# pasqualedem/LabelAnything

Measured on AMD Instinct MI355X. Metric: episodes/sec (query+support fwd) ViT-B 1024px 1-shot, higher is better.
Workload: dtype f16; 1 GPU; BASELINE cfg2: SAM ViT-B 1024px encoder + LabelAnything decoder, 1-way 1-shot episodes (2 images each), random-init weights, full-resolution logits; parallelism=episode-sharded x1, no collective, launch=hipGraph replay

## Files before the change

include/la_hip.h:

```cpp
#ifndef LA_HIP_H
#define LA_HIP_H
#ifdef __cplusplus
extern "C" {
#endif

enum { LA_F16 = 0, LA_BF16 = 1, LA_F32 = 2, LA_F16X2 = 3 };
enum { LA_ACT_NONE = 0, LA_ACT_GELU = 1, LA_ACT_RELU = 2, LA_ACT_GELU_BWD = 3  };
enum { LA_MAP_NONE = 0, LA_MAP_GROUP = 1, LA_MAP_WINDOW_MERGE = 2, LA_MAP_CONVT2X2 = 3, LA_MAP_WINDOW_PART = 4, LA_MAP_CONV3X3 = 5  };
enum { LA_ATTN_PLAIN = 0, LA_ATTN_RELPOS = 1, LA_ATTN_RELPOS_WIN16 = 2 };

const char* la_last_error(void);
int la_version(void);

int la_gemm_variant(int v);

typedef struct LaGemmEpilogue {
  const float* bias;
  const float* res;
  int ldr;
  int res_mod;
  float* out32;
  int ld32;
  void* out16;
  int ld16;
  int act;
  int map;
  int p0, p1, p2, p3, p4;
  void* vt;
  int vt_col0, vt_T, vt_Tpad, vt_hd, vt_heads;
  int vt_ws;
  int amap;
  int a_kmod;
  int ksplit;
  void* aux16;
  int ldaux;
  float* nstat_out;
  const float* rvec;
  int rvec_rpg;
  const float* nstat_in;
  const float* ncol;
} LaGemmEpilogue;

int la_gemm_fused_act_ok(int M, int N, int K);

int la_gemm(const void* A, int lda, const void* W, int ldw, int M, int N, int K,
            const LaGemmEpilogue* epi, int dt, void* stream);

enum { LA_GEMM_NT = 0, LA_GEMM_DMA128, LA_GEMM_DMA256x128, LA_GEMM_T256, LA_GEMM_T256P, LA_GEMM_T256Q, LA_GEMM_T256W,
       LA_GEMM_F32_N32, LA_GEMM_F32_N128, LA_GEMM_F32_SMALL, LA_GEMM_SKINNY };
typedef struct LaGemmPlan {
  int kernel, epi, planes, direct, ragged, gm, ksplit, kchunk, grid, block, lds_bytes;
} LaGemmPlan;

int la_gemm_plan(const void* A, int lda, const void* W, int ldw, int M, int N, int K,
                 const LaGemmEpilogue* epi, int dt, int ncu, LaGemmPlan* out);

int la_conv3x3_f32(const float* in, int B, int H, int W, int Cin, const float* wt, const float* bias, int Cout, float* out32,
                   void* stream);

int la_conv3x3_split_ok(int Cin, int Cout);
int la_conv3x3_split(const float* in, int B, int H, int W, int Cin, const float* wt, const float* bias, int Cout, float* out32, void* stream);

int la_layernorm(const float* x, const float* x2, int ldx, int rows, int E, const float* gamma, const float* beta,
                 float eps, int gelu, float* out32, void* out16, void* out16_pe, const float* pe, int pe_mod,
                 int window, int H, int W, int dt, void* stream);

int la_im2col_patch(const float* img, int Bn, int S, int patch, void* out16, int dt, void* stream);

int la_im2col_3x3(const void* in16, int B, int H, int W, int C, void* out16, int dt, void* stream);

int la_relpos_terms(const void* qkv, int B, int heads, int G, int E, const void* tabh, const void* tabw,
                    float* relh, float* relw, int dt, void* stream);

int la_attn_fwd(const void* qkv, const void* vt, void* out16, const float* relh, const float* relw,
                const void* tabh, const void* tabw, int B, int heads, int T, int Tpad, int G, int E, float scale, int mode,
                int dt, void* stream);


int la_dense_pe(const float* gauss, int g, int D, float* out, void* stream);

int la_point_embed(const float* xy, const int* kind, const int* shift, int n, int D, int image_size, const float* gauss,
                   const float* type_emb, const float* not_a_point, const float* no_sparse, float* out32, void* stream);

int la_mask_embed(const float* masks, const int* flags, int P, int C, int Hm, int g, int D, const float* const* w,
                  const float* support, const float* class_enc, const float* pe, float* src32, void* src16, void* srcpe16,
                  int dt, void* stream);

int la_attn_small(const float* q, int ldq, const float* k, int ldk, const float* v, int ldv, int B, int Nq, int Nk, int heads,
                  int hd, void* out16, float* out32, int ldo, int dt, void* stream);

int la_colmean(const float* x, int P, int hw, int D, float* out, float* scratch, void* stream);

int la_class_mean(const float* emb, const unsigned char* flags, int B, int M, int C, int D, float* out, void* stream);

int la_region_mean(const float* x, int B, int M, int C, int g, int k, int D, float* out, void* stream);

int la_classify_max(const float* feat, const float* protos, const unsigned char* flags, int B, int Npix, int N, int C, int Cf, float* seg,
                    int* win, void* stream);

int la_classify(const float* feat, const float* protos, int B, int Npix, int C, int Cf, float* seg, void* stream);

int la_add_cast(const float* x, const float* y, int ymod, long rows, int D, float* out32, void* out16, int dt, void* stream);

int la_nchw_to_nhwc(const float* in, int N, int C, int HW, float* out32, void* out16, int dt, void* stream);
int la_nhwc_to_nchw(const float* in, int N, int C, int HW, float* out, void* stream);

int la_transpose_many(const long long* tile_table, int ntiles, void* stream);

int la_bilinear(const float* in, int N, int h, int w, int H, int W, float* out, void* stream);

int la_post_final(const float* big, int B, int C, int S, const int* sizes, const unsigned char* flag_gts, int Hmax, int Wmax,
                  float* logits, long long* argmax, void* stream);

int la_confmat_update(const long long* pred, const long long* gt, int B, long HW, const int* lut, int L, int K,
                      long long ignore_index, unsigned long long* confmat, unsigned long long* confbin,
                      unsigned long long* counters, void* stream);

int la_resample_u8(const unsigned char* in, long n_outer, int in_size, int inner, int out_size, const int* bounds, const int* kk,
                   int ksize, unsigned char* out, void* stream);
int la_u8_to_chw_norm(const unsigned char* in, int h, int w, int SH, int SW, const float* mean3, const float* std3, float* out,
                      void* stream);

int la_prompt_masks(const unsigned char* masks, const int* first, const int* count, const int* index, int P, int H, int W, int nh,
                    int nw, int S, int Mo, float* out, unsigned char* flags, void* stream);

int la_focal_loss(const float* logits, const long long* target, int B, int C, long HW, float gamma, int class_weighting, float scale,
                  long long ignore_index, float* loss, float* dlogits, float* class_weights, void* scratch, long scratch_bytes,
                  void* stream);

int la_logits_objective_workspace_bytes(int B, int C, long HW, long* bytes);
int la_logits_objective(const float* logits, const long long* target, int B, int C, long HW, long long ignore_index, int mask,
                        float w_focal, float gamma, float w_dice, float w_fp, int class_weighting, float* value, float* components,
                        float* dlogits, float* class_weights, void* workspace, long workspace_bytes, void* stream);

int la_prompt_contrastive_workspace_bytes(int B, int n, int D, long* bytes);
int la_prompt_contrastive(const float* emb, const unsigned char* flags, int B, int n, int C, int D, const float* t_prime, const float* bias,
                          float* loss, float* demb, float* dt_prime, float* dbias, void* workspace, long workspace_bytes, void* stream);

// ... 155 lines not shown
```

labelanything_amd/_lib.py:

```python
from __future__ import annotations

import ctypes as C
import os
from typing import Optional

import torch

_HERE = os.path.dirname(os.path.abspath(__file__))
LIB_PATH = os.path.join(_HERE, "libla_hip.so")

LA_F16, LA_BF16, LA_F32, LA_F16X2 = 0, 1, 2, 3
ACT_NONE, ACT_GELU, ACT_RELU, ACT_GELU_BWD = 0, 1, 2, 3
MAP_NONE, MAP_GROUP, MAP_WINDOW_MERGE, MAP_CONVT2X2, MAP_WINDOW_PART, MAP_CONV3X3 = 0, 1, 2, 3, 4, 5
ATTN_PLAIN, ATTN_RELPOS, ATTN_RELPOS_WIN16 = 0, 1, 2

_DT = {torch.float16: LA_F16, torch.bfloat16: LA_BF16, torch.float32: LA_F32}


class LaGemmEpilogue(C.Structure):
    _fields_ = [
        ("bias", C.c_void_p), ("res", C.c_void_p), ("ldr", C.c_int), ("res_mod", C.c_int),
        ("out32", C.c_void_p), ("ld32", C.c_int), ("out16", C.c_void_p), ("ld16", C.c_int),
        ("act", C.c_int), ("map", C.c_int),
        ("p0", C.c_int), ("p1", C.c_int), ("p2", C.c_int), ("p3", C.c_int), ("p4", C.c_int),
        ("vt", C.c_void_p), ("vt_col0", C.c_int), ("vt_T", C.c_int), ("vt_Tpad", C.c_int),
        ("vt_hd", C.c_int), ("vt_heads", C.c_int), ("vt_ws", C.c_int), ("amap", C.c_int), ("a_kmod", C.c_int), ("ksplit", C.c_int),
        ("aux16", C.c_void_p), ("ldaux", C.c_int),
        ("nstat_out", C.c_void_p), ("rvec", C.c_void_p), ("rvec_rpg", C.c_int), ("nstat_in", C.c_void_p), ("ncol", C.c_void_p),
    ]


_lib: Optional[C.CDLL] = None


def lib() -> C.CDLL:
    global _lib
    if _lib is None:
        if not os.path.exists(LIB_PATH):
            raise RuntimeError(
                f"labelanything_amd: HIP extension {LIB_PATH} is missing - build it with "
                "`python -c 'import __graft_entry__ as g; g.build()'` (there is no CPU/eager fallback)")
        l = C.CDLL(LIB_PATH)
        l.la_last_error.restype = C.c_char_p
        l.la_version.restype = C.c_int
        for name in EXPORTS:
            getattr(l, name).restype = C.c_int
        _lib = l
    return _lib


EXPORTS = [
    "la_gemm", "la_layernorm", "la_im2col_patch", "la_im2col_3x3", "la_relpos_terms", "la_attn_fwd",
    "la_dense_pe", "la_point_embed", "la_mask_embed", "la_attn_small", "la_colmean", "la_class_mean",
    "la_classify", "la_add_cast", "la_conv3x3_f32", "la_nchw_to_nhwc", "la_nhwc_to_nchw", "la_bilinear", "la_post_final",
    "la_confmat_update", "la_resample_u8", "la_u8_to_chw_norm", "la_prompt_masks", "la_focal_loss", "la_adamw_step",
    "la_gemm_tn", "la_gemm_tn16", "la_gemm_fused_act_ok", "la_gemm_plan", "la_colsum_acc", "la_layernorm_bwd", "la_layernorm_bwd_res", "la_transpose_many", "la_act_fwd", "la_act_bwd", "la_attn_small_lse", "la_attn_small_bwd", "la_bilinear_bwd", "la_bilinear_bwd_set", "la_bilinear_bwd_set_ok", "la_bilinear_rows", "la_bilinear_rows_bwd_set",
    "la_classify_bwd", "la_row_broadcast", "la_twoway_t2i", "la_twoway_i2t", "la_gemm_variant", "la_attn_fwd_lse", "la_head_transpose", "la_attn_bwd", "la_cast", "la_gelu_bwd16", "la_axpy", "la_transpose16", "la_qk_fp8", "la_attn_fwd_fp8", "la_colmean16", "la_layernorm_g", "la_add_rowvec", "la_add_rowvec_split", "la_attn_fwd_cs", "la_attn_fwd_rows", "la_colsum_fold", "la_gelu_fwd16", "la_gemm_tn_db",
    "la_attn_fwd_relpos_lse", "la_attn_bwd_relpos", "la_relpos_bwd", "la_twoway_pe_layout",
    "la_norm_finalize", "la_norm_stats", "la_conv3x3_split", "la_conv3x3_split_ok",
    "la_error_count", "la_error_points",
    "la_logits_objective_workspace_bytes", "la_logits_objective", "la_prompt_contrastive_workspace_bytes", "la_prompt_contrastive",
    "la_rle_scan", "la_rle_decode", "la_rle_prompt_masks", "la_rle_ground_truth", "la_rle_points",
    "la_region_mean", "la_classify_max", "la_region_mean_bwd", "la_classify_max_bwd",
    "la_classify_wide", "la_classify_wide_bwd", "la_level_reduce", "la_level_reduce_bwd",
    "la_proto_kernels", "la_proto_kernels_bwd", "la_classify_conv", "la_classify_conv_bwd",
    "la_extract_pool_plan", "la_extract_pool", "la_extract_fold", "la_extract_unfold",
]


def gemm_variant(v: int = -1) -> int:
    return int(lib().la_gemm_variant(int(v)))


def _check(rc: int, what: str) -> None:
    if rc != 0:
        msg = lib().la_last_error().decode()
        raise RuntimeError(f"{what} failed ({rc}): {msg}")


def _ptr(t: Optional[torch.Tensor]):
    return None if t is None else C.c_void_p(t.data_ptr())


def _stream() -> C.c_void_p:
    return C.c_void_p(torch.cuda.current_stream().cuda_stream)


def dt_of(t: torch.Tensor) -> int:
    return _DT[t.dtype]


def _dev(t: torch.Tensor) -> None:
    if not t.is_cuda:
        raise RuntimeError("labelanything_amd kernels need device tensors (no CPU fallback)")
    if t.device.index != torch.cuda.current_device():
        raise RuntimeError(f"tensor on {t.device} but the current device is cuda:{torch.cuda.current_device()}: "
                           "wrap the call in `with torch.cuda.device(tensor.device)`")


class LaGemmPlan(C.Structure):
    _fields_ = [(f, C.c_int) for f in ("kernel", "epi", "planes", "direct", "ragged", "gm", "ksplit", "kchunk", "grid", "block", "lds_bytes")]


GEMM_KERNELS = ("NT", "DMA128", "DMA256x128", "T256", "T256P", "T256Q", "T256W", "F32_N32", "F32_N128", "F32_SMALL", "SKINNY")


def _addr(x) -> Optional[int]:
    return x.data_ptr() if isinstance(x, torch.Tensor) else x


def _gemm_epilogue(m: int, n: int, *, bias=None, res=None, res_mod=0, out32=None, out16=None, act=ACT_NONE, map=MAP_NONE, p=(0, 0, 0, 0, 0), vt=None,
                   vt_col0=0, vt_T=0, vt_Tpad=0, vt_hd=64, vt_heads=0, vt_ws=0, amap=MAP_NONE, a_kmod=0, ksplit=0, aux16=None, nstat_out=None, rvec=None,
                   rvec_rpg=0, nstat_in=None, ncol=None, ldr=None, ld32=None, ld16=None, ldaux=None) -> LaGemmEpilogue:
    def ld(x, given):
        if x is None:
            return 0
        if given is not None:
            return given
        return n if not isinstance(x, torch.Tensor) else (x.stride(-2) if x.dim() >= 2 else 0)

    e = LaGemmEpilogue()
    e.bias, e.res, e.out32, e.out16, e.vt, e.aux16 = _addr(bias), _addr(res), _addr(out32), _addr(out16), _addr(vt), _addr(aux16)
    e.ldr, e.ld32, e.ld16, e.ldaux = ld(res, ldr), ld(out32, ld32), ld(out16, ld16), ld(aux16, ldaux)
    e.res_mod = res_mod
    e.act, e.map = act, map
    e.p0, e.p1, e.p2, e.p3, e.p4 = p
    e.vt_col0, e.vt_T, e.vt_Tpad, e.vt_hd, e.vt_heads = vt_col0, vt_T, vt_Tpad, vt_hd, vt_heads
    e.vt_ws = vt_ws
    e.amap = amap
    e.a_kmod = a_kmod
    e.ksplit = ksplit
    mpad = -(-m // 256) * 256
    if isinstance(nstat_out, torch.Tensor) and (nstat_out.dtype != torch.float32 or nstat_out.numel() < m * (n // 64) * 2):
        raise RuntimeError(f"gemm: nstat_out must be fp32 with at least M * (N / 64) * 2 = {m * (n // 64) * 2} entries")
    if isinstance(nstat_in, torch.Tensor) and (nstat_in.dtype != torch.float32 or nstat_in.numel() < mpad * 2 or ncol is None
                                               or ncol.dtype != torch.float32 or ncol.numel() < n):
        raise RuntimeError(f"gemm: nstat_in must be fp32 [ceil(M / 256) * 256, 2] (>= {mpad * 2} entries) and needs ncol fp32 [N]")
    if isinstance(rvec, torch.Tensor) and (rvec.dtype != torch.float32 or rvec_rpg <= 0 or rvec.numel() < -(-m // rvec_rpg) * n):
        raise RuntimeError("gemm: rvec must be fp32 [ceil(M / rvec_rpg), N] with rvec_rpg > 0")
    e.nstat_out, e.rvec, e.nstat_in, e.ncol = _addr(nstat_out), _addr(rvec), _addr(nstat_in), _addr(ncol)
    e.rvec_rpg = rvec_rpg
    return e


def gemm(a: torch.Tensor, w: torch.Tensor, *, M=None, lda=None, **epilogue) -> None:
    _dev(a)
    m = a.shape[0] if M is None else M
    k = w.shape[1]
    n = w.shape[0]
    e = _gemm_epilogue(m, n, **epilogue)
    rc = lib().la_gemm(_ptr(a), C.c_int(a.stride(0) if lda is None else lda), _ptr(w), C.c_int(w.stride(0)),
                       C.c_int(m), C.c_int(n), C.c_int(k), C.byref(e), C.c_int(dt_of(a)), _stream())
    _check(rc, "la_gemm")


def gemm_plan(a, lda: int, w, ldw: int, m: int, n: int, k: int, dt: int, ncu: int = 0, **epilogue) -> LaGemmPlan:
    plan = LaGemmPlan()
    e = _gemm_epilogue(m, n, **epilogue)
    rc = lib().la_gemm_plan(C.c_void_p(_addr(a)), C.c_int(lda), C.c_void_p(_addr(w)), C.c_int(ldw), C.c_int(m), C.c_int(n), C.c_int(k), C.byref(e),
                            C.c_int(dt), C.c_int(ncu), C.byref(plan))
    _check(rc, "la_gemm_plan")
    return plan


def norm_finalize(part: Optional[torch.Tensor], m: int, e: int, eps: float, mr: torch.Tensor, x16: Optional[torch.Tensor] = None, rpg: int = 0,
                  cs_part: Optional[torch.Tensor] = None) -> None:
    _dev(mr)
    mpad = -(-m // 256) * 256
    if mr.dtype != torch.float32 or mr.numel() < mpad * 2 or not mr.is_contiguous():
        raise RuntimeError(f"norm_finalize: mr must be contiguous fp32 with >= {mpad * 2} entries")
    if part is not None and (part.dtype != torch.float32 or part.numel() < m * (e // 64) * 2):
        raise RuntimeError("norm_finalize: part must be fp32 [m, e / 64, 2]")
    if cs_part is not None:
        if x16 is None or rpg <= 0 or m % rpg or x16.shape[0] < m or x16.shape[1] != e or x16.stride(1) != 1:
            raise RuntimeError("norm_finalize: column sums need x16 [m, e] and m % rpg == 0")
        if cs_part.dtype != torch.float32 or cs_part.numel() < (m // rpg) * norm_cs_chunks(rpg) * e:
            raise RuntimeError("norm_finalize: cs_part too small")
    _check(lib().la_norm_finalize(_ptr(part), C.c_int(m), C.c_int(e // 64), C.c_int(e), C.c_float(eps), _ptr(mr), _ptr(x16),
                                  C.c_int(x16.stride(0) if x16 is not None else 0), C.c_int(rpg), _ptr(cs_part),
                                  C.c_int(dt_of(x16) if x16 is not None else LA_F16), _stream()), "la_norm_finalize")


def norm_cs_chunks(rpg: int) -> int:
    return -(-rpg // 128)


def norm_stats(x: torch.Tensor, eps: float, x16: torch.Tensor, mr: torch.Tensor) -> None:
    _dev(x)
    m, e = x.shape
    mpad = -(-m // 256) * 256
    if x.dtype != torch.float32 or x.stride(1) != 1 or x16.shape != x.shape or not x16.is_contiguous() or mr.dtype != torch.float32 \
            or mr.numel() < mpad * 2:
        raise RuntimeError("norm_stats: x fp32 [m, e], x16 contiguous 16-bit [m, e], mr fp32 with >= ceil(m / 256) * 256 * 2 entries")
    _check(lib().la_norm_stats(_ptr(x), C.c_int(x.stride(0)), C.c_int(m), C.c_int(e), C.c_float(eps), _ptr(x16), _ptr(mr),
                               C.c_int(dt_of(x16)), _stream()), "la_norm_stats")


def gemm_fused_act_ok(m: int, n: int, k: int) -> bool:
    return bool(lib().la_gemm_fused_act_ok(C.c_int(m), C.c_int(n), C.c_int(k)))


def layernorm(x: torch.Tensor, gamma, beta, eps: float, *, x2=None, gelu=False, out32=None, out16=None,
              out16_pe=None, pe=None, pe_mod=0, window=0, H=0, W=0, dt=LA_F16) -> None:
    _dev(x)
    rows, e = x.shape[0], x.shape[1]
    if window < 0:
        o = out32 if out32 is not None else out16
        if window == -2:
            rows = o.shape[0]
            if x.shape[0] < (rows // (H * W)) * (H + 2) * (W + 2):
                raise RuntimeError("layernorm(window=-2): x must hold the padded maps [B * (H + 2) * (W + 2), E]")
        elif out16 is None or out16.shape[0] < (rows // (H * W)) * (H + 2) * (W + 2):
            raise RuntimeError("layernorm(window=-1): out16 must hold the padded maps [B * (H + 2) * (W + 2), ...]")
    rc = lib().la_layernorm(_ptr(x), _ptr(x2), C.c_int(x.stride(0)), C.c_int(rows), C.c_int(e), _ptr(gamma), _ptr(beta),
                            C.c_float(eps), C.c_int(int(gelu)), _ptr(out32), _ptr(out16), _ptr(out16_pe), _ptr(pe),
                            C.c_int(pe_mod), C.c_int(window), C.c_int(H), C.c_int(W), C.c_int(dt), _stream())
    _check(rc, "la_layernorm")


def im2col_patch(img: torch.Tensor, patch: int, out16: torch.Tensor, split: bool = False) -> None:
    _dev(img)
    bn, _, s, _ = img.shape
    dt = LA_F16X2 if split else dt_of(out16)
    if split and out16.dtype != torch.float16:
        raise RuntimeError("im2col_patch(split=True) writes fp16 plane pairs")
    _check(lib().la_im2col_patch(_ptr(img), C.c_int(bn), C.c_int(s), C.c_int(patch), _ptr(out16), C.c_int(dt),
                                 _stream()), "la_im2col_patch")


def im2col_3x3(x16: torch.Tensor, b: int, h: int, w: int, c: int, out16: torch.Tensor, split: bool = False) -> None:
    _dev(x16)
    _check(lib().la_im2col_3x3(_ptr(x16), C.c_int(b), C.c_int(h), C.c_int(w), C.c_int(c), _ptr(out16),
                               C.c_int(LA_F16X2 if split else dt_of(x16)), _stream()), "la_im2col_3x3")


def relpos_terms(qkv: torch.Tensor, b: int, heads: int, g: int, e: int, tabh, tabw, relh, relw) -> None:
    _check(lib().la_relpos_terms(_ptr(qkv), C.c_int(b), C.c_int(heads), C.c_int(g), C.c_int(e), _ptr(tabh), _ptr(tabw),
                                 _ptr(relh), _ptr(relw), C.c_int(dt_of(qkv)), _stream()), "la_relpos_terms")


def attn_fwd(qkv, vt, out16, relh, relw, b: int, heads: int, t: int, tpad: int, g: int, e: int, scale: float, mode: int,
             tabh=None, tabw=None) -> None:
    _check(lib().la_attn_fwd(_ptr(qkv), _ptr(vt), _ptr(out16), _ptr(relh), _ptr(relw), _ptr(tabh), _ptr(tabw), C.c_int(b),
                             C.c_int(heads), C.c_int(t),
                             C.c_int(tpad), C.c_int(g), C.c_int(e), C.c_float(scale), C.c_int(mode), C.c_int(dt_of(qkv)),
                             _stream()), "la_attn_fwd")

# ... 728 lines not shown
```

labelanything_amd/csrc/gemm.hip:

```cpp
#include <cstdlib>
#include <cstring>
#include <type_traits>
#include "la_common.h"
#include "../../include/la_hip.h"
#include "gemm_shared.h"
#include "gemm_plan.h"

namespace la {

constexpr int BM = 128, BN = 128, BK = 64;
constexpr int STAGE_BYTES = (BM + BN) * BK * 2;


template <typename T>
__global__ __launch_bounds__(256, 2) void gemm_nt_kernel(const T* __restrict__ A, int lda, const T* __restrict__ Wt, int ldw,
                                                          int M, int N, int K, LaGemmEpilogue e) {
  extern __shared__ __attribute__((aligned(16))) char smem[];
  const int tid = threadIdx.x, lane = tid & 63, wave = tid >> 6;
  const int wm = wave >> 1, wn = wave & 1;
  const int ntn = (N + BN - 1) / BN, ntm = (M + BM - 1) / BM;
  const int tile = xcd_remap(blockIdx.x, ntm * ntn);
  const int m0 = (tile / ntn) * BM, n0 = (tile % ntn) * BN;

  const int lc = tid & 7, lr = tid >> 3;
// ... 1469 lines not shown
        a[u] = *reinterpret_cast<const float4*>(ap + 8 * j);
        b[u] = *reinterpret_cast<const float4*>(wp + 8 * j);
      }
#pragma unroll
      for (int u = 0; u < 8; ++u) {
        if (j0 + u * KS < nchunk) {
          acc = __builtin_amdgcn_mfma_f32_32x32x2f32(a[u].x, b[u].x, acc, 0, 0, 0);
          acc = __builtin_amdgcn_mfma_f32_32x32x2f32(a[u].y, b[u].y, acc, 0, 0, 0);
          acc = __builtin_amdgcn_mfma_f32_32x32x2f32(a[u].z, b[u].z, acc, 0, 0, 0);
          acc = __builtin_amdgcn_mfma_f32_32x32x2f32(a[u].w, b[u].w, acc, 0, 0, 0);
        }
      }
    }
  }
  if (KS == 4) {
#pragma unroll
    for (int r = 0; r < 16; ++r) part[wave][r][lane] = acc[r];
    __syncthreads();
    if (wave != 0) return;
#pragma unroll
    for (int r = 0; r < 16; ++r) acc[r] = (part[0][r][lane] + part[1][r][lane]) + (part[2][r][lane] + part[3][r][lane]);
  }
  if (!active) return;
  const int col = tn * 32 + fr;
  if (col >= N) return;
  float* outT = reinterpret_cast<float*>(e.out16);
  const float bias = e.bias ? e.bias[col] : 0.f;
#pragma unroll
  for (int r = 0; r < 16; ++r) {
    const int m = tm * 32 + (r & 3) + 8 * (r >> 2) + 4 * fh;
    if (m >= M) continue;
    float v = acc[r] + bias;
    if (e.act == LA_ACT_GELU) v = gelu_erf(v);
    else if (e.act == LA_ACT_RELU) v = fmaxf(v, 0.f);
    if (e.res) v += e.res[(size_t)(e.res_mod ? m % e.res_mod : m) * e.ldr + col];
    if (e.out32) e.out32[(size_t)m * e.ld32 + col] = v;
    if (outT) outT[(size_t)m * e.ld16 + col] = v;
  }
}

static void launch_f32_small(const LaGemmPlan& p, const GemmArgs& g) {
  const dim2 d = f32_small_grid(g.M, g.N, g.K);
  with_int<1, 4>(g.K >= 1024 ? 4 : 1, [&](auto ks) { launch<float, gemm_f32_small_kernel<LA_V(ks)>>(dim3(d.x, d.y), p, g); });
}

template <typename T>
static void launch_plan(const LaGemmPlan& p, const GemmArgs& g, int stg) {
  const dim3 grid(p.grid);
  if constexpr (std::is_same<T, float>::value) {
    switch (p.kernel) {
      case LA_GEMM_F32_SMALL: return launch_f32_small(p, g);
      case LA_GEMM_SKINNY: return launch_skinny<float>(p, g);
      default: return launch_f32(p, g, ConvA{0, 0, 0, 0});
    }
  } else {
    switch (p.kernel) {
      case LA_GEMM_SKINNY: return launch_skinny<T>(p, g);
      case LA_GEMM_NT: return launch<T, gemm_nt_kernel<T>>(grid, p, g);
      case LA_GEMM_DMA128: return launch<T, gemm_dma_kernel<T, 128>>(grid, p, g, p.gm);
      case LA_GEMM_DMA256x128: return launch<T, gemm_dma4_kernel<T>>(grid, p, g, p.gm);
      case LA_GEMM_T256:
        return (void)with_int<1, 2>(p.planes, [&](auto npl) {
          with_int<0, 1, 2, 3>(p.epi, [&](auto e) { launch<T, gemm_t256_kernel<T, LA_V(npl), LA_V(e)>>(grid, p, g, p.gm); });
        });
      case LA_GEMM_T256P:
        return (void)with_int<1, 2>(p.planes, [&](auto npl) {
          with_int<1, 2, 3>(p.epi, [&](auto e) { launch<T, gemm_t256p_kernel<T, LA_V(npl), LA_V(e)>>(grid, p, g, p.gm); });
        });
      case LA_GEMM_T256Q:
        return (void)with_int<1, 2, 3, 4>(p.epi, [&](auto e) { launch<T, gemm_t256q_kernel<T, LA_V(e)>>(grid, p, g, p.gm, p.ksplit, p.kchunk); });
      default:
        with_int<1, 2, 3>(p.epi, [&](auto e) { launch_t256w<T, LA_V(e)>(p, g, stg); });
        with_int<5, 6>(p.epi, [&](auto e) { launch_t256w_fused<T, LA_V(e)>(p, g, stg); });
        if constexpr (std::is_same<T, f16_t>::value) with_int<7, 8, 9, 10, 11, 12>(p.epi, [&](auto e) { launch_t256w_fused<T, LA_V(e)>(p, g, stg); });
    }
  }
}

#ifdef LA_DEBUG
static void plan_debug_overrides(LaGemmPlan* p, uintptr_t A, int lda, uintptr_t W, int ldw, int M, int N, int K, const LaGemmEpilogue& e, int ncu,
                                 int variant, int* stg) {
  static const char *path = getenv("LA_GEMM_PATH"), *nop = getenv("LA_GEMM_NO_PERSISTENT"), *nosmall = getenv("LA_NO_F32_SMALL"),
                    *want = getenv("LA_KSPLIT_WANT"), *kgrid = getenv("LA_KSPLIT_GRID"), *gmenv = getenv("LA_GEMM_GROUP_M"),
                    *w4grid = getenv("LA_W4_GRID"), *stagger = getenv("LA_W4_STAGGER");
  const bool tiles16 = p->kernel <= LA_GEMM_T256P || (p->kernel == LA_GEMM_T256Q && p->epi != 4) || (p->kernel == LA_GEMM_T256W && p->epi <= 3);
  const int planes = p->planes;
  if (tiles16 && path && (path[0] == 'v' || p->kernel != LA_GEMM_NT)) {
    *p = plan_default(K);
    if (path[0] == 'v') plan_launch(p, LA_GEMM_NT, M, N, K, ncu, variant);
    else if (path[0] == '7' && (!e.vt || (e.vt_col0 % 256) == 0)) plan_t256(p, planes, M, N, K / planes, e, ncu, variant);
    else plan_launch(p, path[0] == '4' || (path[0] != '2' && K <= 1536 && tiles_of(M, N, 256, 128) >= 512) ? LA_GEMM_DMA256x128 : LA_GEMM_DMA128, M, N, K, ncu, variant);
  }
  if (tiles16 && nop && p->kernel >= LA_GEMM_T256P) {
    *p = plan_default(K);
    plan_t256(p, planes, M, N, K / planes, e, ncu, variant, false);
  }
  if (nosmall && p->kernel == LA_GEMM_F32_SMALL) plan_launch(p, LA_GEMM_SKINNY, M, N, K, ncu, variant);
  if (p->kernel == LA_GEMM_T256Q && p->epi == 4) {
    if (want) ksplit_chunks(K / 64, atoi(want), p), plan_launch(p, LA_GEMM_T256Q, M, N, K, ncu, variant);
    if (kgrid) p->grid = atoi(kgrid) > 0 ? atoi(kgrid) : (int)tiles_of(M, N, 256, 256) * p->ksplit;
  }
  if (gmenv && group_m(p->kernel, N)) p->gm = (p->gm & ~0xff) | atoi(gmenv);
  if (p->kernel == LA_GEMM_T256W) {
    if (w4grid && atoi(w4grid) > 0 && atoi(w4grid) < p->grid) p->grid = atoi(w4grid);
    if (stagger) *stg = (atoi(stagger) << 16) | (strchr(stagger, ',') ? atoi(strchr(stagger, ',') + 1) : 0);
  }
}
#endif

}

extern "C" int la_gemm_variant(int v) {
  const int prev = la::g_gemm_variant;
#ifdef LA_DEBUG
  if (v >= 0) la::g_gemm_variant = v;
#else
  if (v >= 0 && v <= 2) la::g_gemm_variant = v;
#endif
  return prev;
}

#ifdef LA_DEBUG
extern "C" int la_dbg_gemm_stamps(unsigned long long* host_out) {
  (void)hipDeviceSynchronize();
  return (int)hipMemcpyFromSymbol(host_out, HIP_SYMBOL(la::g_dbg_stamps), sizeof(unsigned long long) * 8 * la::LA_DBG_NSTAMP);
}
extern "C" int la_dbg_gemm_stamps_clear() {
  static unsigned long long z[8 * la::LA_DBG_NSTAMP] = {0};
  return (int)hipMemcpyToSymbol(HIP_SYMBOL(la::g_dbg_stamps), z, sizeof(z));
}
#endif

extern "C" int la_gemm_fused_act_ok(int M, int N, int K) { return la::fused_act_ok(M, N, K, la::cu_count(), la::g_gemm_variant); }

static int gemm_plan_checked(const void* A, int lda, const void* W, int ldw, int M, int N, int K, const LaGemmEpilogue* epi, int dt, int ncu,
                             LaGemmPlan* p, int* stg) {
  LA_CHECK_ARG(A && W && epi && p, "la_gemm: null pointer");
  if (ncu <= 0) ncu = la::cu_count();
  const uintptr_t a = reinterpret_cast<uintptr_t>(A), w = reinterpret_cast<uintptr_t>(W);
  char err[640];
  if (la::gemm_plan(a, lda, w, ldw, M, N, K, *epi, dt, ncu, la::g_gemm_variant, p, err, sizeof(err)) != 0) {
    la_set_error("%s", err);
    return -1;
  }
#ifdef LA_DEBUG
  la::plan_debug_overrides(p, a, lda, w, ldw, M, N, K, *epi, ncu, la::g_gemm_variant, stg);
#endif
  return 0;
}

extern "C" int la_gemm_plan(const void* A, int lda, const void* W, int ldw, int M, int N, int K, const LaGemmEpilogue* epi, int dt, int ncu,
                            LaGemmPlan* out) {
  int stg = 0;
  return gemm_plan_checked(A, lda, W, ldw, M, N, K, epi, dt, ncu, out, &stg);
}

extern "C" int la_gemm(const void* A, int lda, const void* W, int ldw, int M, int N, int K, const LaGemmEpilogue* epi, int dt,
                       void* stream) {
  LaGemmPlan p;
  int stg = 0;
  if (gemm_plan_checked(A, lda, W, ldw, M, N, K, epi, dt, 0, &p, &stg) != 0) return -1;
  const la::GemmArgs g{A, W, lda, ldw, M, N, K, *epi, reinterpret_cast<hipStream_t>(stream)};
  if (dt == LA_F32) la::launch_plan<float>(p, g, stg);
  else if (dt == LA_F16) la::launch_plan<la::f16_t>(p, g, stg);
  else la::launch_plan<la::bf16_t>(p, g, stg);
  LA_CHECK_LAUNCH("la_gemm");
  return 0;
}

extern "C" int la_conv3x3_f32(const float* in, int B, int H, int W, int Cin, const float* wt, const float* bias, int Cout, float* out32,
                              void* stream) {
  LA_CHECK_ARG(in && wt && out32, "la_conv3x3_f32: null pointer");
  LA_CHECK_ARG(B > 0 && H > 0 && W > 0 && Cin > 0 && (Cin % 32) == 0 && Cout > 0, "la_conv3x3_f32: Cin=%d must be a multiple of 32", Cin);
  LaGemmEpilogue e{};
  e.bias = bias;
  e.out32 = out32;
  e.ld32 = Cout;
  const int M = B * H * W, K = 9 * Cin;
  LaGemmPlan p = la::plan_default(K);
  la::plan_f32(&p, M, Cout, K, e);
  la::launch_f32(p, la::GemmArgs{in, wt, Cin, K, M, Cout, K, e, reinterpret_cast<hipStream_t>(stream)}, la::ConvA{1, H, W, Cin});
  LA_CHECK_LAUNCH("la_conv3x3_f32");
  return 0;
}
```

labelanything_amd/csrc/gemm_plan.h:

```cpp
#pragma once
#include <cstdint>
#include <cstdio>
#include "../../include/la_hip.h"

namespace la {

#define LA_PLAN_CHECK(cond, ...) \
  do { if (!(cond)) { snprintf(err, errsz, __VA_ARGS__); return -1; } } while (0)

template <typename P> static inline bool al16(P p) { return ((uintptr_t)p & 15) == 0; }
static inline long tiles_of(int M, int N, int bm, int bn) { return (long)((M + bm - 1) / bm) * ((N + bn - 1) / bn); }

static inline bool k64_ok(int K, int a_kmod) { return (K % 64) == 0 && K >= 128 && (a_kmod == 0 || (a_kmod % 64) == 0); }

static inline bool epi_vec_ok(int N, const LaGemmEpilogue& e, int elt_bytes) {
  return (N % 8) == 0 && (!e.bias || al16(e.bias)) && (!e.res || (al16(e.res) && (e.ldr % 4) == 0)) &&
         (!e.out32 || (al16(e.out32) && (e.ld32 % 4) == 0)) && (!e.out16 || (al16(e.out16) && (e.ld16 % (16 / elt_bytes)) == 0)) &&
         (e.map != LA_MAP_CONVT2X2 || (e.p2 % 8) == 0) && (!e.vt || ((e.vt_col0 % 128) == 0 && (e.vt_Tpad % 4) == 0 && al16(e.vt)));
}

static inline bool dma_operands_ok(uintptr_t A, int lda, uintptr_t W, int ldw, int M, int N) {
  return (size_t)M * lda * 2 < (1ull << 32) && (size_t)N * ldw * 2 < (1ull << 32) && al16(A) && al16(W);
}
static inline bool fast_ok(uintptr_t A, int lda, uintptr_t W, int ldw, int M, int N, int K, const LaGemmEpilogue& e) {
  return (K % 64) == 0 && dma_operands_ok(A, lda, W, ldw, M, N) && epi_vec_ok(N, e, 2);
}

static inline bool fused_act_ok(int M, int N, int K, int ncu, int variant) {
  return M > 0 && (N % 256) == 0 && k64_ok(K, 0) && tiles_of(M, N, 256, 256) >= ncu && (variant & 0xff) == 2;
}

static inline int group_m(int kernel, int N) {
  if (kernel == LA_GEMM_DMA128 || kernel == LA_GEMM_DMA256x128) return 8;
  if (kernel == LA_GEMM_T256Q || kernel == LA_GEMM_T256W) return N >= 2560 ? 8 : 2;
  return kernel == LA_GEMM_T256 || kernel == LA_GEMM_T256P ? 2 : 0;
}

static inline int persistent_grid(long ntiles, int ncu) { return ntiles < ncu ? (int)ntiles : ncu; }

static inline void ksplit_chunks(int nkt, int want, LaGemmPlan* p) {
  if (want > nkt / 2) want = nkt / 2;
  if (want < 1) want = 1;
  int c = (nkt + want - 1) / want;
  if (c < 2) c = 2;
  while (c < nkt && (nkt % c) == 1) ++c;
  if (c > nkt) c = nkt;
  p->kchunk = c * 64;
  p->ksplit = (nkt + c - 1) / c;
}

struct dim2 { int x, y; };
static inline dim2 f32_small_grid(int M, int N, int K) {
  return K >= 1024 ? dim2{(N + 31) / 32, (M + 31) / 32} : dim2{(N + 63) / 64, (M + 63) / 64};
}
static inline dim2 skinny_grid(int M, int N, int K) {
  const int groups = (N + 3) / 4;
  return dim2{K >= 1024 ? groups : (groups + 3) / 4, M > 32 ? (M + 31) / 32 : 1};
}

struct KernelShape { int bm, bn, block, lds, lds2; };
constexpr KernelShape KERNEL_SHAPE[] = {
    {128, 128, 256, 65536, 0},
    {128, 128, 256, 128 * 132 * 4, 0},
    {256, 128, 256, 3 * 24576, 0},
    {256, 256, 512, 136 * 1024, 3 * 49152},
    {256, 256, 512, 4 * 32768 + 8 * 512 + 8 * 2048, 3 * 49152 + 8 * 2048},
    {256, 256, 512, 2 * 65536 + 8 * 2048 + 8 * 512, 0},
    {256, 256, 256, 4 * 32768 + 4 * 8192, 0},
    {128, 32, 256, 2 * (128 + 32) * 128, 0},
    {128, 128, 256, 128 * 132 * 4, 0},
};

static inline void plan_launch(LaGemmPlan* p, int kernel, int M, int N, int K, int ncu, int variant) {
  p->kernel = kernel;
  p->gm = group_m(kernel, N);
  if (kernel == LA_GEMM_F32_SMALL || kernel == LA_GEMM_SKINNY) {
    const dim2 g = kernel == LA_GEMM_SKINNY ? skinny_grid(M, N, K) : f32_small_grid(M, N, K);
    p->grid = g.x * g.y, p->block = 256, p->lds_bytes = 0;
    return;
  }
  const KernelShape& s = KERNEL_SHAPE[kernel];
  const long tiles = tiles_of(M, N, s.bm, s.bn) * p->ksplit;
  p->grid = kernel >= LA_GEMM_T256P && kernel <= LA_GEMM_T256W ? persistent_grid(tiles, ncu) : (int)tiles;
  p->block = s.block, p->lds_bytes = p->planes == 2 ? s.lds2 : s.lds;
  if (kernel == LA_GEMM_T256Q) p->gm |= variant & 0x800500;
}

static inline void plan_t256(LaGemmPlan* p, int planes, int M, int N, int K, const LaGemmEpilogue& e, int ncu, int variant, bool persistent = true) {
  const int var = variant & 0xff;
  const bool plain = e.map == LA_MAP_NONE && e.res_mod == 0;
  const bool only16 = !e.res && !e.out32 && e.out16;
  const bool plain16 = plain && only16 && e.act == LA_ACT_NONE, gelu16 = plain && only16 && e.act == LA_ACT_GELU && !e.vt;
  const bool scatter = e.map == LA_MAP_WINDOW_PART && e.res_mod == 0 && e.amap == LA_MAP_NONE && only16 && e.act == LA_ACT_NONE &&
                       (planes == 1 || (e.vt && e.vt_col0 == 0)) &&
                       (!e.vt || (size_t)((M + e.vt_T - 1) / e.vt_T + 4096) * e.vt_heads * e.vt_hd * e.vt_Tpad < (1ull << 32));
  const bool w4_resmod = planes == 1 && e.map == LA_MAP_NONE && e.res_mod > 0 && (e.res_mod % 256) == 0 && (M % 256) == 0 && e.res && var == 2 &&
                         k64_ok(K, e.a_kmod) && !((variant >> 8) & 1);
  const bool f32 = (plain || w4_resmod) && e.act == LA_ACT_NONE && e.out32 && !e.vt && (e.ld32 % 4) == 0 && (!e.res || (e.ldr % 4) == 0);
  const int pepi = (plain16 || scatter) ? 1 : gelu16 ? 2 : f32 ? 3 : 0;
  p->planes = planes, p->epi = pepi;
  if (!(persistent && pepi && (N % 256) == 0 && K / 32 >= 8 && (e.ld16 % 8) == 0)) {
    p->epi = plain16 ? 1 : gelu16 ? 2 : (plain && e.act == LA_ACT_NONE && e.res && e.out32 && !e.vt) ? 3 : 0;
    return plan_launch(p, LA_GEMM_T256, M, N, K, ncu, variant);
  }
  const bool k64 = planes == 1 && k64_ok(K, e.a_kmod);
  plan_launch(p, k64 && var == 2 ? LA_GEMM_T256W : k64 && var >= 1 ? LA_GEMM_T256Q : LA_GEMM_T256P, M, N, K, ncu, variant);
  if (p->kernel == LA_GEMM_T256W) {
    p->gm |= variant & 0xf500;
    p->direct = e.map == LA_MAP_NONE && !e.vt && !((variant >> 8) & 1);
    p->ragged = p->direct && (M & 255) != 0;
  }
}

static inline void plan_w4_fused(LaGemmPlan* p, int epi, int M, int N, int K, int ncu, int variant) {
  p->epi = epi, p->direct = 1, p->ragged = (M & 255) != 0;
  plan_launch(p, LA_GEMM_T256W, M, N, K, ncu, variant);
}

static inline void plan_tiles16(LaGemmPlan* p, uintptr_t A, int lda, uintptr_t W, int ldw, int M, int N, int K, const LaGemmEpilogue& e, int ncu,
                                int variant) {
  if (!fast_ok(A, lda, W, ldw, M, N, K, e)) return plan_launch(p, LA_GEMM_NT, M, N, K, ncu, variant);
  const int planes = (e.a_kmod > 0 && K == 2 * e.a_kmod) ? 2 : 1;
  if (tiles_of(M, N, 256, 256) >= (planes == 2 ? 128 : 512) && (!e.vt || (e.vt_col0 % 256) == 0)) return plan_t256(p, planes, M, N, K / planes, e, ncu, variant);
  plan_launch(p, K <= 1536 && tiles_of(M, N, 256, 128) >= 512 ? LA_GEMM_DMA256x128 : LA_GEMM_DMA128, M, N, K, ncu, variant);
}

static inline void plan_f32(LaGemmPlan* p, int M, int N, int K, const LaGemmEpilogue& e) {
  p->epi = epi_vec_ok(N, e, 4) ? 1 : 0;
  plan_launch(p, N <= 32 ? LA_GEMM_F32_N32 : LA_GEMM_F32_N128, M, N, K, 0, 0);
}

static inline LaGemmPlan plan_default(int K) { return LaGemmPlan{LA_GEMM_NT, 0, 1, 0, 0, 0, 1, K, 0, 256, 0}; }

static inline int gemm_plan(uintptr_t A, int lda, uintptr_t W, int ldw, int M, int N, int K, const LaGemmEpilogue& e, int dt, int ncu, int variant,
                            LaGemmPlan* p, char* err, size_t errsz) {
  *p = plan_default(K);
  LA_PLAN_CHECK(A && W, "la_gemm: null pointer");
  LA_PLAN_CHECK(M > 0 && N > 0 && K > 0, "la_gemm: bad shape M=%d N=%d K=%d", M, N, K);
  LA_PLAN_CHECK(e.ld16 < (1 << 22) && e.ldaux < (1 << 22) && e.ld32 < (1 << 22) && e.ldr < (1 << 22) && N < (1 << 22),
                "la_gemm: output / residual leading dimensions must be below %d elements", 1 << 22);
  const int kq = (dt == LA_F32) ? 4 : 8;
  LA_PLAN_CHECK((K % kq) == 0 && (lda % kq) == 0 && (ldw % kq) == 0, "la_gemm: K, lda, ldw must be multiples of %d (K=%d lda=%d ldw=%d)", kq, K,
                lda, ldw);
  LA_PLAN_CHECK(e.out32 || e.out16 || e.vt, "la_gemm: no output");
  LA_PLAN_CHECK(e.a_kmod == 0 || (dt != LA_F32 && e.a_kmod > 0 && (e.a_kmod % 64) == 0 && e.a_kmod <= K && lda >= e.a_kmod && M > 32),
                "la_gemm: a_kmod=%d must be a multiple of 64, <= K=%d and <= lda=%d (16-bit operands, M > 32)", e.a_kmod, K, lda);
  LA_PLAN_CHECK(dt == LA_F16 || dt == LA_BF16 || dt == LA_F32, "la_gemm: bad dtype %d", dt);
  LA_PLAN_CHECK(e.amap == LA_MAP_NONE || (e.amap == LA_MAP_WINDOW_PART && e.map == LA_MAP_NONE && dt != LA_F32) ||
                    (e.amap == LA_MAP_CONV3X3 && e.map == LA_MAP_NONE && dt == LA_F16 && e.a_kmod == 0 && e.p1 > 0 && (e.p1 % 64) == 0 &&
                     K == 27 * e.p1 && e.p2 == lda && lda == 2 * e.p1 && e.p0 > 2 && (N % 256) == 0 && !e.vt && e.ksplit == 0 && M > 512),
                "la_gemm: amap must be LA_MAP_NONE, LA_MAP_WINDOW_PART (16-bit operands, no output map) or LA_MAP_CONV3X3 (fp16 plane pairs, p0 = padded "
                "width, p1 = C %% 64 == 0, p2 = lda = 2 C, K = 27 C, N %% 256 == 0), got amap=%d map=%d dt=%d", e.amap, e.map, dt);
  LA_PLAN_CHECK(e.act != LA_ACT_GELU_BWD || e.aux16, "la_gemm: LA_ACT_GELU_BWD needs aux16 (the saved pre-activation)");
  const bool rows16 = (e.ld16 % 8) == 0 && e.ld16 >= N && al16(e.out16);
  if (e.aux16 && !e.nstat_out) {
    LA_PLAN_CHECK(e.act == LA_ACT_GELU || e.act == LA_ACT_GELU_BWD, "la_gemm: aux16 goes with LA_ACT_GELU (written) or LA_ACT_GELU_BWD (read)");
    LA_PLAN_CHECK(dt != LA_F32 && fused_act_ok(M, N, K, ncu, variant) && fast_ok(A, lda, W, ldw, M, N, K, e),
                  "la_gemm: aux16 needs 16-bit operands and a shape la_gemm_fused_act_ok() accepts (M=%d N=%d K=%d)", M, N, K);
    LA_PLAN_CHECK(e.out16 && !e.out32 && !e.res && !e.vt && e.map == LA_MAP_NONE && e.amap == LA_MAP_NONE && e.a_kmod == 0 && e.ksplit == 0 && rows16 &&
                      (e.ldaux % 8) == 0 && e.ldaux >= N && al16(e.aux16),
                  "la_gemm: aux16 forms write out16 only (no residual / fp32 output / maps / V^T / planes), rows 16-byte aligned");
    LA_PLAN_CHECK(e.act == LA_ACT_GELU || !e.bias, "la_gemm: LA_ACT_GELU_BWD takes no bias");
    plan_w4_fused(p, e.act == LA_ACT_GELU ? 5 : 6, M, N, K, ncu, variant);
    return 0;
  }
  if (e.nstat_out || e.nstat_in || e.rvec) {
    LA_PLAN_CHECK(dt == LA_F16 && (N % 256) == 0 && k64_ok(K, e.a_kmod) && fast_ok(A, lda, W, ldw, M, N, K, e) && (variant & 0xff) == 2,
                  "la_gemm: nstat_out / nstat_in need fp16 operands, N %% 256 == 0, K %% 64 == 0, K >= 128, 16-byte aligned rows (M=%d N=%d K=%d)", M,
                  N, K);
    LA_PLAN_CHECK(!e.vt && e.map == LA_MAP_NONE && e.amap == LA_MAP_NONE && e.ksplit == 0 && !(e.nstat_out && e.nstat_in) &&
                      (!e.aux16 || (e.nstat_out && (e.ldaux % 8) == 0 && e.ldaux >= N && al16(e.aux16))),
                  "la_gemm: nstat_out / nstat_in take no row maps / V^T / ksplit, not both at once; aux16 only with nstat_out (the lo plane, 16-byte aligned rows)");
    const bool stat8 = (reinterpret_cast<uintptr_t>(e.nstat_out) & 7) == 0;
    const bool rvec_ok = !e.rvec || (e.rvec_rpg > 0 && al16(e.rvec) && ((e.rvec_rpg % 256) == 0 || e.rvec_rpg >= 128));
    const bool rvec_split = e.rvec && (e.rvec_rpg % 256) != 0;
    int epi;
    if (e.nstat_in) {
      LA_PLAN_CHECK(e.ncol && e.out16 && !e.out32 && !e.res && !e.rvec && (e.act == LA_ACT_NONE || e.act == LA_ACT_GELU) && rows16 && al16(e.nstat_in) &&
                        al16(e.ncol) && e.a_kmod == 0,
                    "la_gemm: nstat_in writes out16 only (act NONE / GELU), needs ncol, one weight plane");
      epi = e.act == LA_ACT_GELU ? 9 : 8;
    } else if (e.nstat_out && !e.out32 && e.res && e.aux16) {
      LA_PLAN_CHECK(e.out16 && e.act == LA_ACT_NONE && rows16 && (e.ldr % 4) == 0 && stat8 && !e.rvec,
                    "la_gemm: nstat_out with a residual and no out32 writes plane pairs only (out16 + aux16), no group vector");
      LA_PLAN_CHECK(e.res_mod == 0 || ((e.res_mod % 256) == 0 && (M % 256) == 0),
                    "la_gemm: nstat_out with a periodic residual needs res_mod %% 256 == 0 and M %% 256 == 0 (res_mod=%d M=%d)", e.res_mod, M);
      epi = 7;
    } else if (e.nstat_out && !e.out32 && !e.res) {
      LA_PLAN_CHECK(e.out16 && e.aux16 && e.act == LA_ACT_NONE && rows16 && (e.ldaux % 8) == 0 && e.ldaux >= N && al16(e.aux16) && stat8 && e.res_mod == 0,
                    "la_gemm: nstat_out without out32 / res updates a plane-pair stream in place: out16 (hi) and aux16 (lo), 16-byte aligned rows");
      LA_PLAN_CHECK(rvec_ok, "la_gemm: rvec needs a 16-byte aligned vector and groups of whole 256-row tiles or of at least 128 rows (rvec_rpg=%d)",
                    e.rvec_rpg);
      epi = rvec_split ? 12 : 11;
    } else {
      LA_PLAN_CHECK(e.nstat_out && e.out32 && e.out16 && e.act == LA_ACT_NONE && rows16 && (e.ld32 % 4) == 0 && e.ld32 >= N && al16(e.out32) &&
                        (!e.res || (e.ldr % 4) == 0) && stat8,
                    "la_gemm: nstat_out goes with out32 + out16 (no activation), 16-byte aligned rows");
      LA_PLAN_CHECK(e.res_mod == 0 || ((e.res_mod % 256) == 0 && (M % 256) == 0 && e.res),
// ... 36 lines not shown
```

labelanything_amd/csrc/gemm_w4.hip:

```cpp
#include <cstdlib>
#include <cstring>
#include <type_traits>
#include "gemm_shared.h"

namespace la {

typedef uint32_t u32x4 __attribute__((ext_vector_type(4)));
typedef float f32x4 __attribute__((ext_vector_type(4)));

__device__ __forceinline__ u32x4 lds_read16(unsigned addr) {
  return *reinterpret_cast<const __attribute__((address_space(3))) u32x4*>((uintptr_t)addr);
}

template <int IMM>
__device__ __forceinline__ void dma_piece(const void* gbase_uniform, unsigned voff, unsigned ldsbase_uniform) {
  asm volatile("s_add_u32 m0, %2, %3\n\ts_nop 0\n\tglobal_load_lds_dwordx4 %0, %1"
               :
               : "v"(voff), "s"(gbase_uniform), "s"(ldsbase_uniform), "n"(IMM)
               : "memory", "scc");
}

template <typename T> struct MfmaA;
template <> struct MfmaA<f16_t> {
  static __device__ __forceinline__ void go(f32x16& c, const u32x4& a, const u32x4& b) {
    asm volatile("v_mfma_f32_32x32x16_f16 %0, %1, %2, %0" : "+a"(c) : "v"(a), "v"(b));
  }
};
template <> struct MfmaA<bf16_t> {
  static __device__ __forceinline__ void go(f32x16& c, const u32x4& a, const u32x4& b) {
    asm volatile("v_mfma_f32_32x32x16_bf16 %0, %1, %2, %0" : "+a"(c) : "v"(a), "v"(b));
  }
};

__device__ __forceinline__ void acc_zero(f32x16& c) {
  const u32x4 z = {0u, 0u, 0u, 0u};
  asm volatile("s_nop 1\n\tv_mfma_f32_32x32x16_f16 %0, %1, %1, 0" : "=a"(c) : "v"(z));
}

#ifdef LA_DEBUG
constexpr int LA_W4_NSTAMP = 128;
__device__ unsigned long long g_w4_stamps[4 * LA_W4_NSTAMP];
#endif

template <int BYTES> struct GWords;
template <> struct GWords<16> { typedef unsigned type __attribute__((ext_vector_type(4))); };
template <> struct GWords<8> { typedef unsigned type __attribute__((ext_vector_type(2))); };
template <typename V> __device__ __forceinline__ V gld(uintptr_t a) {
  typedef typename GWords<sizeof(V)>::type W;
  return __builtin_bit_cast(V, *reinterpret_cast<const __attribute__((address_space(1))) W*>(a));
}
template <typename V> __device__ __forceinline__ void gst(uintptr_t a, const V& v) {
  typedef typename GWords<sizeof(V)>::type W;
  *reinterpret_cast<__attribute__((address_space(1))) W*>(a) = __builtin_bit_cast(W, v);
}

template <int N> __device__ __forceinline__ void wait_vm_lgkm0() { asm volatile("s_waitcnt vmcnt(%0) lgkmcnt(0)" ::"n"(N) : "memory"); }

#define LA_W4_SB __builtin_amdgcn_sched_barrier(0);
#define LA_W4_MF(IB, ii, j, PAR, KS)                                                                                            \
  if constexpr (!(ABL & 8)) MfmaA<T>::go(acc[(j) >> 1][(IB) + (ii)][(j) & 1], af[PAR][ii], wf[KS][j]); \
  LA_W4_SB
#define LA_W4_RW(KS, j) if constexpr (!(ABL & 2)) wf[KS][j] = lds_read16(waddr[KS] + (j) * 4096); LA_W4_SB
#define LA_W4_RA(PAR, ii, i, KS) if constexpr (!(ABL & 2)) af[PAR][ii] = lds_read16(aaddr[KS] + (i) * 4096); LA_W4_SB
#define LA_W4_PA0(src, i, bo) if constexpr (!(ABL & 1)) dma_piece<(i) * 1024>(src, soA0[i], dstA + (bo)); LA_W4_SB
#define LA_W4_PA1(src, i, bo) if constexpr (!(ABL & 1)) dma_piece<8192 + (i) * 1024>(src, soA1[i], dstA + (bo)); LA_W4_SB
#define LA_W4_PW(src, i, bo) if constexpr (!(ABL & 1)) dma_piece<(i) * 1024>(src, soW[i], dstW + (bo)); LA_W4_SB
#define LA_W4_QA0(src, i, bo) dma_piece<(i) * 1024>(src, soA0[i], dstA + (bo));
#define LA_W4_QA1(src, i, bo) dma_piece<8192 + (i) * 1024>(src, soA1[i], dstA + (bo));
#define LA_W4_QW(src, i, bo) dma_piece<(i) * 1024>(src, soW[i], dstW + (bo));
#define LA_W4_WAIT(N)                                                             \
  if constexpr (!(ABL & 4)) {                                                     \
    if (seam) wait_vm_lgkm0<((N) + SEAM > 63 ? 63 : (N) + SEAM)>();               \
    else wait_vm_lgkm0<(N)>();                                                    \
  }
#define LA_W4_BAR if constexpr (!(ABL & 4)) { __builtin_amdgcn_s_barrier(); asm volatile("" ::: "memory"); }
#ifndef LA_W4_GROUP
#define LA_W4_GROUP 1
#endif
#include "gemm_w4_ktile.inc"

template <typename T, int EPI, bool RAGGED>
__device__ __forceinline__ void epilogue_w4(char* slab, f32x16 (&acc)[2][4][2], int row0, int col0, const LaGemmEpilogue& e, int lane, int M, int N) {
  row0 = __builtin_amdgcn_readfirstlane(row0);
  col0 = __builtin_amdgcn_readfirstlane(col0);
  asm volatile("" : "+v"(lane));
  const int fr = lane & 31, fh = lane >> 5;
  const int rq = lane >> 3, cg = lane & 7;
  const unsigned sl = lds_addr_of(slab);
  const unsigned waddr = sl + (unsigned)((fh * 64 + (fr & ~7) + ((fr & 7) ^ (((fr >> 3) ^ fh) & 7))) << 4);
  unsigned raddr[8];
#pragma unroll
  for (int t = 0; t < 8; ++t) raddr[t] = sl + (unsigned)((rq * 64 + cg * 8 + (t ^ ((cg ^ rq) & 7))) << 4);
  constexpr bool RESP = EPI == 11 || EPI == 12;
  constexpr bool TWOG = EPI == 10 || EPI == 12;
  constexpr bool PROD = EPI == 7 || EPI == 10 || RESP;
  constexpr bool RES = EPI == 3 || PROD;
  constexpr bool NORM = EPI == 8 || EPI == 9;
  constexpr bool GELU = EPI == 2 || EPI == 5 || EPI == 9;
  float bias[2][8];
  float biasB[2][8];
  float ncol[2][8];
#pragma unroll
  for (int jp = 0; jp < 2; ++jp) {
    if (EPI == 6) continue;
    const float4 b0 = e.bias ? *reinterpret_cast<const float4*>(e.bias + col0 + jp * 64 + cg * 8) : make_float4(0.f, 0.f, 0.f, 0.f);
    const float4 b1 = e.bias ? *reinterpret_cast<const float4*>(e.bias + col0 + jp * 64 + cg * 8 + 4) : make_float4(0.f, 0.f, 0.f, 0.f);
    bias[jp][0] = b0.x; bias[jp][1] = b0.y; bias[jp][2] = b0.z; bias[jp][3] = b0.w;
    bias[jp][4] = b1.x; bias[jp][5] = b1.y; bias[jp][6] = b1.z; bias[jp][7] = b1.w;
    if (TWOG) {
#pragma unroll
      for (int t = 0; t < 8; ++t) biasB[jp][t] = bias[jp][t];
      const int gB = min(row0 / e.rvec_rpg + 1, (M - 1) / e.rvec_rpg);
      const float* rv = e.rvec + (size_t)gB * N + col0 + jp * 64 + cg * 8;
      const float4 r0 = *reinterpret_cast<const float4*>(rv), r1 = *reinterpret_cast<const float4*>(rv + 4);
      biasB[jp][0] += r0.x; biasB[jp][1] += r0.y; biasB[jp][2] += r0.z; biasB[jp][3] += r0.w;
      biasB[jp][4] += r1.x; biasB[jp][5] += r1.y; biasB[jp][6] += r1.z; biasB[jp][7] += r1.w;
    }
    if (PROD && e.rvec) {
      const float* rv = e.rvec + (size_t)min(row0 / e.rvec_rpg, (M - 1) / e.rvec_rpg) * N + col0 + jp * 64 + cg * 8;
      const float4 r0 = *reinterpret_cast<const float4*>(rv), r1 = *reinterpret_cast<const float4*>(rv + 4);
      bias[jp][0] += r0.x; bias[jp][1] += r0.y; bias[jp][2] += r0.z; bias[jp][3] += r0.w;
      bias[jp][4] += r1.x; bias[jp][5] += r1.y; bias[jp][6] += r1.z; bias[jp][7] += r1.w;
    }
    if (NORM) {
      const float4 c0 = *reinterpret_cast<const float4*>(e.ncol + col0 + jp * 64 + cg * 8);
      const float4 c1 = *reinterpret_cast<const float4*>(e.ncol + col0 + jp * 64 + cg * 8 + 4);
      ncol[jp][0] = c0.x; ncol[jp][1] = c0.y; ncol[jp][2] = c0.z; ncol[jp][3] = c0.w;
      ncol[jp][4] = c1.x; ncol[jp][5] = c1.y; ncol[jp][6] = c1.z; ncol[jp][7] = c1.w;
    }
  }
  float4 mrv[2][2];
  auto ldmr = [&](int i) {
#ifdef LA_W4_NO_MRLOAD
    mrv[i & 1][0] = mrv[i & 1][1] = make_float4(0.f, 1.f, 0.f, 1.f);
    return;
#endif
    const uintptr_t mp = reinterpret_cast<uintptr_t>(e.nstat_in + (size_t)(row0 + i * 32) * 2) + (size_t)(unsigned)(rq * 32);
    mrv[i & 1][0] = gld<float4>(mp);
    mrv[i & 1][1] = gld<float4>(mp + 16);
  };
  if (NORM) {
    ldmr(0);
    ldmr(1);
  }
  const int rowB = TWOG ? (row0 / e.rvec_rpg + 1) * e.rvec_rpg : 0;
  const int nslots = N >> 6;
  T* out16 = reinterpret_cast<T*>(e.out16);
  auto wr = [&](auto ic, auto jpc) {
    constexpr int i = decltype(ic)::value, jp = decltype(jpc)::value;
#pragma unroll
    for (int jj = 0; jj < 2; ++jj)
#pragma unroll
      for (int g = 0; g < 4; ++g) {
        const f32x4 v = {acc[jp][i][jj][4 * g], acc[jp][i][jj][4 * g + 1], acc[jp][i][jj][4 * g + 2], acc[jp][i][jj][4 * g + 3]};
        const unsigned a = (waddr ^ (unsigned)((((4 * jj) ^ (2 * g)) & 7) << 4)) + (unsigned)(g * 2048 + jj * 512);
        *reinterpret_cast<__attribute__((address_space(3))) f32x4*>((uintptr_t)a) = v;
      }
  };
  f32x4 rd0[8];
  auto rd = [&](f32x4 (&r)[8]) {
#pragma unroll
    for (int t = 0; t < 8; ++t) r[t] = *reinterpret_cast<const __attribute__((address_space(3))) f32x4*>((uintptr_t)raddr[t]);
  };
  const int rrow0 = e.res_mod > 0 ? row0 % e.res_mod : row0;
  auto tbase = [&](const void* p, int r0, int ld, int es) { return reinterpret_cast<uintptr_t>(p) + ((size_t)r0 * ld + col0) * es; };
  auto loff = [&](int ld, int es) { return (unsigned)((rq * 4 * ld + cg * 8) * es); };
  auto addr = [&](const void* p, uintptr_t base, unsigned lo, int r0, int r, int ld, int es, int cb) {
    if constexpr (RAGGED) return reinterpret_cast<uintptr_t>(p) + ((size_t)(r0 + rq * 4 + r) * ld + col0 + cg * 8) * es + cb;
    else return (base + (size_t)(unsigned)(r * ld * es)) + (size_t)lo + cb;
  };
  const uintptr_t b16 = tbase(e.out16, row0, e.ld16, 2), bax = tbase(e.aux16, row0, e.ldaux, 2), b32 = tbase(e.out32, row0, e.ld32, 4);
  const uintptr_t br16 = tbase(e.out16, rrow0, e.ld16, 2), brax = tbase(e.aux16, rrow0, e.ldaux, 2), brs = tbase(e.res, rrow0, e.ldr, 4);
  const unsigned l16 = loff(e.ld16, 2), lax = loff(e.ldaux, 2), l32 = loff(e.ld32, 4), lrs = loff(e.ldr, 4);
  const float4 zero4 = make_float4(0.f, 0.f, 0.f, 0.f);
  auto ldres = [&](int i, int jp, float4 (&res)[4][2]) {
    if constexpr (RESP) {
#pragma unroll
      for (int s_ = 0; s_ < 4; ++s_) {
        const uintptr_t ph = addr(e.out16, br16, l16, rrow0, i * 32 + s_, e.ld16, 2, jp * 128);
        const uintptr_t pl = addr(e.aux16, brax, lax, rrow0, i * 32 + s_, e.ldaux, 2, jp * 128);
        if constexpr (RAGGED) {
          const bool ok = row0 + i * 32 + rq * 4 + s_ < M;
          res[s_][0] = ok ? gld<float4>(ph) : zero4;
          res[s_][1] = ok ? gld<float4>(pl) : zero4;
        } else {
          res[s_][0] = gld<float4>(ph);
          res[s_][1] = gld<float4>(pl);
        }
      }
      return;
    }
    if (!e.res) {
#pragma unroll
      for (int s_ = 0; s_ < 4; ++s_) res[s_][0] = res[s_][1] = zero4;
      return;
    }
#pragma unroll
    for (int s_ = 0; s_ < 4; ++s_)
#pragma unroll
      for (int h = 0; h < 2; ++h) {
        const uintptr_t pr = addr(e.res, brs, lrs, rrow0, i * 32 + s_, e.ldr, 4, jp * 256 + 16 * h);
        if constexpr (RAGGED) res[s_][h] = row0 + i * 32 + rq * 4 + s_ < M ? gld<float4>(pr) : zero4;
        else res[s_][h] = gld<float4>(pr);
      }
  };
  T* aux16 = reinterpret_cast<T*>(e.aux16);
  auto ldaux = [&](int i, int jp, uint4 (&ax)[4]) {
    const int row = row0 + i * 32 + rq * 4;
#pragma unroll
    for (int s_ = 0; s_ < 4; ++s_) {
      const uintptr_t pa = addr(e.aux16, bax, lax, row0, i * 32 + s_, e.ldaux, 2, jp * 128);
      if constexpr (RAGGED) ax[s_] = row + s_ < M ? gld<uint4>(pa) : make_uint4(0u, 0u, 0u, 0u);
      else ax[s_] = gld<uint4>(pa);
    }
  };
  const uintptr_t bns = PROD ? reinterpret_cast<uintptr_t>(e.nstat_out) + ((size_t)row0 * nslots + (col0 >> 6)) * 8 : 0;
  const unsigned lns = (unsigned)(rq * 4 * nslots * 8);
  auto out = [&](int i, int jp, const f32x4 (&r)[8], const float4 (&res)[4][2], const uint4 (&ax)[4]) {
    const int row = row0 + i * 32 + rq * 4;
    if (RES) {
      if constexpr (RESP && !TWOG && !RAGGED) {
#pragma unroll
        for (int sp = 0; sp < 2; ++sp) {
          const int s0 = 2 * sp, s1 = 2 * sp + 1;
          const uint32_t h0[4] = {__builtin_bit_cast(uint32_t, res[s0][0].x), __builtin_bit_cast(uint32_t, res[s0][0].y),
                                  __builtin_bit_cast(uint32_t, res[s0][0].z), __builtin_bit_cast(uint32_t, res[s0][0].w)};
          const uint32_t h1[4] = {__builtin_bit_cast(uint32_t, res[s1][0].x), __builtin_bit_cast(uint32_t, res[s1][0].y),
                                  __builtin_bit_cast(uint32_t, res[s1][0].z), __builtin_bit_cast(uint32_t, res[s1][0].w)};
          const uint32_t l0[4] = {__builtin_bit_cast(uint32_t, res[s0][1].x), __builtin_bit_cast(uint32_t, res[s0][1].y),
                                  __builtin_bit_cast(uint32_t, res[s0][1].z), __builtin_bit_cast(uint32_t, res[s0][1].w)};
          const uint32_t l1[4] = {__builtin_bit_cast(uint32_t, res[s1][1].x), __builtin_bit_cast(uint32_t, res[s1][1].y),
                                  __builtin_bit_cast(uint32_t, res[s1][1].z), __builtin_bit_cast(uint32_t, res[s1][1].w)};
          f32x2 c[8];
#pragma unroll
          for (int t = 0; t < 8; ++t) {
            const f32x2 hv = (t & 1) ? f32x2{unpack_hi<T>(h0[t >> 1]), unpack_hi<T>(h1[t >> 1])} : f32x2{unpack_lo<T>(h0[t >> 1]), unpack_lo<T>(h1[t >> 1])};
            const f32x2 lv = (t & 1) ? f32x2{unpack_hi<T>(l0[t >> 1]), unpack_hi<T>(l1[t >> 1])} : f32x2{unpack_lo<T>(l0[t >> 1]), unpack_lo<T>(l1[t >> 1])};
            c[t] = f32x2{r[t][s0], r[t][s1]} + f32x2{bias[jp][t], bias[jp][t]} + (hv + lv);
          }
          const f32x2 a2 = ((c[0] + c[1]) + (c[2] + c[3])) + ((c[4] + c[5]) + (c[6] + c[7]));
// ... 197 lines not shown
      }
#pragma unroll
      for (int s_ = 0; s_ < 4; ++s_) {
        uint4 pk;
        pk.x = pack2<T>(v[0][s_ >> 1][s_ & 1], v[1][s_ >> 1][s_ & 1]);
        pk.y = pack2<T>(v[2][s_ >> 1][s_ & 1], v[3][s_ >> 1][s_ & 1]);
        pk.z = pack2<T>(v[4][s_ >> 1][s_ & 1], v[5][s_ >> 1][s_ & 1]);
        pk.w = pack2<T>(v[6][s_ >> 1][s_ & 1], v[7][s_ >> 1][s_ & 1]);
        if (!RAGGED || row + s_ < M) gst(addr(e.out16, b16, l16, row0, i * 32 + s_, e.ld16, 2, jp * 128), pk);
      }
    }
  };
  using I0 = std::integral_constant<int, 0>;
  using I1 = std::integral_constant<int, 1>;
  using I2 = std::integral_constant<int, 2>;
  using I3 = std::integral_constant<int, 3>;
  float4 res0[4][2], res1[4][2];
  uint4 aux0[4], aux1[4];
  if (RES) {
    ldres(0, 0, res0);
    ldres(0, 1, res1);
  }

  if (EPI == 6) {
    ldaux(0, 0, aux0);
    ldaux(0, 1, aux1);
  }
  wr(I0{}, I0{});
  rd(rd0);
  wr(I0{}, I1{});
  __builtin_amdgcn_sched_barrier(0);
  out(0, 0, rd0, res0, aux0);
  if (RES) ldres(1, 0, res0);
  if (EPI == 6) ldaux(1, 0, aux0);
  __builtin_amdgcn_sched_barrier(0);
  rd(rd0);
  wr(I1{}, I0{});
  __builtin_amdgcn_sched_barrier(0);
  out(0, 1, rd0, res1, aux1);
  if (NORM) ldmr(2);
  if (RES) ldres(1, 1, res1);
  if (EPI == 6) ldaux(1, 1, aux1);
  __builtin_amdgcn_sched_barrier(0);
  rd(rd0);
  wr(I1{}, I1{});
  __builtin_amdgcn_sched_barrier(0);
  out(1, 0, rd0, res0, aux0);
  if (RES) ldres(2, 0, res0);
  if (EPI == 6) ldaux(2, 0, aux0);
  __builtin_amdgcn_sched_barrier(0);
  rd(rd0);
  wr(I2{}, I0{});
  __builtin_amdgcn_sched_barrier(0);
  out(1, 1, rd0, res1, aux1);
  if (NORM) ldmr(3);
  if (RES) ldres(2, 1, res1);
  if (EPI == 6) ldaux(2, 1, aux1);
  __builtin_amdgcn_sched_barrier(0);
  rd(rd0);
  wr(I2{}, I1{});
  __builtin_amdgcn_sched_barrier(0);
  out(2, 0, rd0, res0, aux0);
  if (RES) ldres(3, 0, res0);
  if (EPI == 6) ldaux(3, 0, aux0);
  __builtin_amdgcn_sched_barrier(0);
  rd(rd0);
  wr(I3{}, I0{});
  __builtin_amdgcn_sched_barrier(0);
  out(2, 1, rd0, res1, aux1);
  if (RES) ldres(3, 1, res1);
  if (EPI == 6) ldaux(3, 1, aux1);
  __builtin_amdgcn_sched_barrier(0);
  rd(rd0);
  wr(I3{}, I1{});
  __builtin_amdgcn_sched_barrier(0);
  out(3, 0, rd0, res0, aux0);
  __builtin_amdgcn_sched_barrier(0);
  rd(rd0);
  __builtin_amdgcn_sched_barrier(0);
  out(3, 1, rd0, res1, aux1);
  __builtin_amdgcn_sched_barrier(0);
}

template <typename T, int EPI, int ABL, bool DIRECT, bool RAGGED = false>
__global__ __launch_bounds__(256, 1) void gemm_t256w_kernel(const T* __restrict__ A, int lda, const T* __restrict__ Wt, int ldw, int M, int N,
                                                             int K, LaGemmEpilogue e, int gm, int stg) {
  constexpr int BK_ = 64;
  constexpr unsigned REG = 32768;
  constexpr int SEAM = (EPI == 3 || EPI == 5 || EPI == 7 || EPI >= 10) ? 47 : 32;
  extern __shared__ __attribute__((aligned(16))) char smem[];
  const int tid = threadIdx.x, lane = tid & 63, wave = __builtin_amdgcn_readfirstlane(tid >> 6);
#ifdef LA_DEBUG
  const bool stamps = ((gm >> 10) & 1) && blockIdx.x == 0;
  int stamp_i = 0;
  auto stamp = [&](int tag) {
    if (stamps && stamp_i < LA_W4_NSTAMP) {
      unsigned long long t_;
      asm volatile("s_memtime %0\n\ts_waitcnt lgkmcnt(0)" : "=s"(t_)::"memory");
      if (lane == 0) g_w4_stamps[wave * LA_W4_NSTAMP + stamp_i] = (t_ << 8) | (unsigned)tag;
      ++stamp_i;
    }
  };
#else
  auto stamp = [](int) {};
#endif
#ifdef LA_DEBUG
  const bool nostore = (gm >> 8) & 1;
#else
  constexpr bool nostore = false;
#endif
  gm &= 0xff;
  if ((stg >> 16) > 1) {
    const int cls = (blockIdx.x >> 3) % (stg >> 16);
    for (int i = 0; i < cls * (stg & 0xffff); ++i) __builtin_amdgcn_s_sleep(16);
  }
  const int wr = wave >> 1, wc = wave & 1;
  const int fr = lane & 31, fh = lane >> 5;
  const int ntn = N / 256, ntm = (M + 255) / 256, ntiles = ntm * ntn;
  const unsigned lds0 = lds_addr_of(smem);
  char* slab = smem + 4 * REG + wave * 8192;
  unsigned* rtab = nullptr;
  if (EPI == 1 && e.map != LA_MAP_NONE) rtab = reinterpret_cast<unsigned*>(slab + 2048);

  unsigned aaddr[4], waddr[4];
#pragma unroll
  for (int ks = 0; ks < 4; ++ks) {
    const unsigned coff = (unsigned)(((ks * 2 + fh) ^ ((fr >> 1) & 7)) << 4);
    aaddr[ks] = lds0 + (wr * 128 + fr) * 128 + coff;
    waddr[ks] = lds0 + 2 * REG + (wc * 128 + fr) * 128 + coff;
  }
  const unsigned dstA = lds0 + (wave >> 1) * 16384 + (wave & 1) * 4096;
  const unsigned dstW = lds0 + 2 * REG + wave * 8192;
  unsigned soA0[4], soA1[4], soA1n[4], soW[8];
  int m0 = 0, n0 = 0, m0n = 0, n0n = 0;
  auto plan = [&](int tile, int& pm0, int& pn0, unsigned (&a0)[4], unsigned (&a1)[4], unsigned (&w)[8]) {
    int tm_, tn_;
    tile_coords(xcd_remap(tile, ntiles), ntm, ntn, gm, tm_, tn_);
    pm0 = tm_ * 256;
    pn0 = tn_ * 256;
    int lane_ = lane;
    if constexpr (EPI >= 7) asm volatile("" : "+v"(lane_));
    const int lane = lane_;
    const int lr = lane >> 3;
#pragma unroll
    for (int i = 0; i < 4; ++i) {
      const int r = (wave >> 1) * 128 + ((wave & 1) * 4 + i) * 8 + lr;
      const int ch = ((lane & 7) ^ ((r >> 1) & 7)) << 3;
      a0[i] = (unsigned)(((size_t)a_row(e, min(pm0 + r, M - 1)) * lda + ch) * sizeof(T));
      a1[i] = (unsigned)(((size_t)a_row(e, min(pm0 + r + 64, M - 1)) * lda + ch) * sizeof(T));
    }
#pragma unroll
    for (int i = 0; i < 8; ++i) {
      const int r = (wave * 8 + i) * 8 + lr;
      const int ch = ((lane & 7) ^ ((r >> 1) & 7)) << 3;
      w[i] = (unsigned)(((size_t)(pn0 + r) * ldw + ch) * sizeof(T));
    }
  };

  f32x16 acc[2][4][2];
#pragma unroll
  for (int h = 0; h < 2; ++h)
#pragma unroll
    for (int i = 0; i < 4; ++i)
#pragma unroll
      for (int j = 0; j < 2; ++j)
        acc_zero(acc[h][i][j]);
  u32x4 wf[4][4], af[2][2];

  int tile = blockIdx.x;
  plan(tile, m0, n0, soA0, soA1, soW);
  const int nk = K / BK_;
  unsigned bofs = 0;
  {
    const T* sa = A + a_koff(e, 0);
    const T* sw = Wt;
    LA_W4_QA0(sa, 0, 0) LA_W4_QA0(sa, 1, 0) LA_W4_QA0(sa, 2, 0) LA_W4_QA0(sa, 3, 0)
    LA_W4_QW(sw, 0, 0) LA_W4_QW(sw, 1, 0) LA_W4_QW(sw, 2, 0) LA_W4_QW(sw, 3, 0)
    LA_W4_QW(sw, 4, 0) LA_W4_QW(sw, 5, 0) LA_W4_QW(sw, 6, 0) LA_W4_QW(sw, 7, 0)
    LA_W4_QA1(sa, 0, 0) LA_W4_QA1(sa, 1, 0) LA_W4_QA1(sa, 2, 0) LA_W4_QA1(sa, 3, 0)
    sa = A + a_koff(e, BK_);
    sw = Wt + BK_;
    LA_W4_QA0(sa, 0, REG) LA_W4_QA0(sa, 1, REG) LA_W4_QA0(sa, 2, REG) LA_W4_QA0(sa, 3, REG)
    LA_W4_QW(sw, 0, REG) LA_W4_QW(sw, 1, REG) LA_W4_QW(sw, 2, REG) LA_W4_QW(sw, 3, REG)
    LA_W4_QW(sw, 4, REG) LA_W4_QW(sw, 5, REG) LA_W4_QW(sw, 6, REG) LA_W4_QW(sw, 7, REG)
  }
  wait_vm_lgkm0<16>();
  __builtin_amdgcn_s_barrier();
  asm volatile("" ::: "memory");
#pragma unroll
  for (int j = 0; j < 4; ++j) wf[0][j] = lds_read16(waddr[0] + j * 4096);
#pragma unroll
  for (int ii = 0; ii < 2; ++ii) af[0][ii] = lds_read16(aaddr[0] + ii * 4096);
  waddr[0] ^= REG;

  int kt = 0;
  stamp(1);
  bool seam = false;
  for (;;) {
    const int next = tile + gridDim.x;
    const bool more = next < ntiles;
    const bool last = kt + 1 == nk, prelast = kt + 2 == nk;
    const int kA1 = last ? 0 : kt + 1;
    const int kAW = kt + 2 < nk ? kt + 2 : kt + 2 - nk;
    if (last && more) {
#pragma unroll
      for (int i = 0; i < 4; ++i) soA1[i] = soA1n[i];
    }
    const T* sa1 = A + a_koff(e, kA1 * BK_);
    const unsigned bo1 = bofs ^ REG;
    LA_W4_BLOCK_0
    LA_W4_BLOCK_1
    LA_W4_BLOCK_2
    if (prelast && more) plan(next, m0n, n0n, soA0, soA1n, soW);
    const T* saw = A + a_koff(e, kAW * BK_);
    const T* sww = Wt + kAW * BK_;
#pragma unroll
    for (int ks = 1; ks < 4; ++ks) waddr[ks] ^= REG;
    LA_W4_BLOCK_3
    aaddr[0] ^= REG;
    LA_W4_BLOCK_4
    LA_W4_BLOCK_5
    LA_W4_BLOCK_6
#pragma unroll
    for (int ks = 1; ks < 4; ++ks) aaddr[ks] ^= REG;
    LA_W4_BLOCK_7
    waddr[0] ^= REG;
    bofs ^= REG;
    seam = false;
    ++kt;
    if (!last) continue;
    stamp(2);
    asm volatile("s_nop 15" ::: "memory");
    const bool vtile = !DIRECT && EPI == 1 && e.vt != nullptr && n0 >= e.vt_col0;
#pragma unroll
    for (int i = 0; i < 4; ++i)
#pragma unroll
      for (int j = 0; j < 2; ++j) asm volatile("" : "+a"(acc[0][i][j]));
    constexpr bool STASH = DIRECT && EPI >= 7;
    const unsigned stash = dstA + 8192 + (bofs ^ REG) + (unsigned)lane * 64;
    if constexpr (STASH) {
      const u32x4 q0 = {soA0[0], soA0[1], soA0[2], soA0[3]}, q1 = {soA1[0], soA1[1], soA1[2], soA1[3]};
      const u32x4 q2 = {soW[0], soW[1], soW[2], soW[3]}, q3 = {soW[4], soW[5], soW[6], soW[7]};
      asm volatile("ds_write_b128 %0, %1\n\tds_write_b128 %0, %2 offset:16\n\tds_write_b128 %0, %3 offset:32\n\tds_write_b128 %0, %4 offset:48"
                   :
                   : "v"(stash), "v"(q0), "v"(q1), "v"(q2), "v"(q3)
                   : "memory");
    }
    if constexpr (DIRECT) {
#pragma unroll
      for (int i = 0; i < 4; ++i)
#pragma unroll
        for (int j = 0; j < 2; ++j) asm volatile("" : "+a"(acc[1][i][j]));
      epilogue_w4<T, EPI, RAGGED>(slab, acc, m0 + wr * 128, n0 + wc * 128, e, lane, M, N);
    } else {
      epilogue_wave<T, EPI>(slab, rtab, acc[0], m0 + wr * 128, n0 + wc * 128, n0, M, e, lane, nostore);
#pragma unroll
      for (int i = 0; i < 4; ++i)
#pragma unroll
        for (int j = 0; j < 2; ++j) asm volatile("" : "+a"(acc[1][i][j]));
      epilogue_wave<T, EPI>(slab, rtab, acc[1], m0 + wr * 128, n0 + wc * 128 + 64, n0, M, e, lane, nostore);
    }
    seam = (m0 + 256 <= M) && !vtile;
    stamp(3);
    if (!more) break;
    if constexpr (STASH) {
      u32x4 q0, q1, q2, q3;
      asm volatile("ds_read_b128 %0, %4\n\tds_read_b128 %1, %4 offset:16\n\tds_read_b128 %2, %4 offset:32\n\tds_read_b128 %3, %4 offset:48\n\t"
                   "s_waitcnt lgkmcnt(0)"
                   : "=&v"(q0), "=&v"(q1), "=&v"(q2), "=&v"(q3)
                   : "v"(stash)
                   : "memory");
#pragma unroll
      for (int i = 0; i < 4; ++i) {
        soA0[i] = q0[i];
        soA1[i] = q1[i];
        soW[i] = q2[i];
        soW[4 + i] = q3[i];
      }
    }
#pragma unroll
    for (int h = 0; h < 2; ++h)
#pragma unroll
      for (int i = 0; i < 4; ++i)
#pragma unroll
        for (int j = 0; j < 2; ++j)
          acc_zero(acc[h][i][j]);
    m0 = m0n;
    n0 = n0n;
    tile = next;
    kt = 0;
    if constexpr (DIRECT) {
#pragma unroll
      for (int j = 0; j < 4; ++j) wf[0][j] = lds_read16((waddr[0] ^ REG) + j * 4096);
#pragma unroll
      for (int ii = 0; ii < 2; ++ii) af[0][ii] = lds_read16((aaddr[0]) + ii * 4096);
    }
    stamp(1);
  }
  asm volatile("s_waitcnt vmcnt(0)" ::: "memory");
}

template <typename T, int EPI, int ABL, bool DIRECT, bool RAGGED = false>
static void launch_t256w_abl(const LaGemmPlan& p, const GemmArgs& g, int stg) {
  launch<T, gemm_t256w_kernel<T, EPI, ABL, DIRECT, RAGGED>>(dim3(p.grid), p, g, p.gm & 0x5ff, stg);
}

template <typename T, int EPI>
void launch_t256w(const LaGemmPlan& p, const GemmArgs& g, int stg) {
#ifdef LA_DEBUG
  if (EPI == 1 && with_int<1, 2, 3, 4, 5, 7, 8, 14>((p.gm >> 12) & 15, [&](auto abl) { launch_t256w_abl<T, 1, LA_V(abl), false>(p, g, stg); })) return;
#endif
  if (p.direct && !p.ragged) launch_t256w_abl<T, EPI, 0, true>(p, g, stg);
  else if (p.direct) launch_t256w_abl<T, EPI, 0, true, true>(p, g, stg);
  else launch_t256w_abl<T, EPI, 0, false>(p, g, stg);
}

template <typename T, int EPI>
void launch_t256w_fused(const LaGemmPlan& p, const GemmArgs& g, int stg) {
  if (!p.ragged) launch_t256w_abl<T, EPI, 0, true>(p, g, stg);
  else launch_t256w_abl<T, EPI, 0, true, true>(p, g, stg);
}
#define LA_W4_FUSED(T, EPI) template void launch_t256w_fused<T, EPI>(const LaGemmPlan&, const GemmArgs&, int);
LA_W4_FUSED(f16_t, 5) LA_W4_FUSED(f16_t, 6) LA_W4_FUSED(bf16_t, 5) LA_W4_FUSED(bf16_t, 6)
LA_W4_FUSED(f16_t, 7) LA_W4_FUSED(f16_t, 10) LA_W4_FUSED(f16_t, 8) LA_W4_FUSED(f16_t, 9) LA_W4_FUSED(f16_t, 11) LA_W4_FUSED(f16_t, 12)

#define LA_W4_INST(T, EPI) template void launch_t256w<T, EPI>(const LaGemmPlan&, const GemmArgs&, int);
LA_W4_INST(f16_t, 1) LA_W4_INST(f16_t, 2) LA_W4_INST(f16_t, 3)
LA_W4_INST(bf16_t, 1) LA_W4_INST(bf16_t, 2) LA_W4_INST(bf16_t, 3)

}

#ifdef LA_DEBUG
extern "C" int la_dbg_w4_stamps(unsigned long long* host_out) {
  (void)hipDeviceSynchronize();
  return (int)hipMemcpyFromSymbol(host_out, HIP_SYMBOL(la::g_w4_stamps), sizeof(unsigned long long) * 4 * la::LA_W4_NSTAMP);
}
extern "C" int la_dbg_w4_stamps_clear() {
  static unsigned long long z[4 * la::LA_W4_NSTAMP] = {0};
  return (int)hipMemcpyToSymbol(HIP_SYMBOL(la::g_w4_stamps), z, sizeof(z));
}
#endif
```

labelanything_amd/csrc/gemm_w4_ktile.inc:

```
#if LA_W4_GROUP == 1
#define LA_W4_BLOCK_0 LA_W4_MF(0, 0, 0, 0, 0) LA_W4_RA(1, 0, 0, 1) LA_W4_MF(0, 0, 1, 0, 0) LA_W4_RW(1, 0) LA_W4_MF(0, 0, 2, 0, 0) LA_W4_RW(1, 1) LA_W4_MF(0, 0, 3, 0, 0) LA_W4_RW(1, 2) LA_W4_MF(0, 1, 0, 0, 0) LA_W4_RW(1, 3) LA_W4_MF(0, 1, 1, 0, 0) LA_W4_RA(1, 1, 1, 1) LA_W4_MF(0, 1, 2, 0, 0) LA_W4_PA1(sa1, 0, bo1) LA_W4_MF(0, 1, 3, 0, 0) LA_W4_PA1(sa1, 1, bo1)
#define LA_W4_BLOCK_1 LA_W4_MF(0, 0, 0, 1, 1) LA_W4_RA(0, 0, 0, 2) LA_W4_MF(0, 0, 1, 1, 1) LA_W4_RW(2, 0) LA_W4_MF(0, 0, 2, 1, 1) LA_W4_RW(2, 1) LA_W4_MF(0, 0, 3, 1, 1) LA_W4_RW(2, 2) LA_W4_MF(0, 1, 0, 1, 1) LA_W4_RW(2, 3) LA_W4_MF(0, 1, 1, 1, 1) LA_W4_RA(0, 1, 1, 2) LA_W4_MF(0, 1, 2, 1, 1) LA_W4_PA1(sa1, 2, bo1) LA_W4_MF(0, 1, 3, 1, 1)
#define LA_W4_BLOCK_2 LA_W4_MF(0, 0, 0, 0, 2) LA_W4_RA(1, 0, 0, 3) LA_W4_MF(0, 0, 1, 0, 2) LA_W4_RW(3, 0) LA_W4_MF(0, 0, 2, 0, 2) LA_W4_RW(3, 1) LA_W4_MF(0, 0, 3, 0, 2) LA_W4_RW(3, 2) LA_W4_MF(0, 1, 0, 0, 2) LA_W4_RW(3, 3) LA_W4_MF(0, 1, 1, 0, 2) LA_W4_RA(1, 1, 1, 3) LA_W4_MF(0, 1, 2, 0, 2) LA_W4_PA1(sa1, 3, bo1) LA_W4_WAIT(16) LA_W4_SB LA_W4_MF(0, 1, 3, 0, 2) LA_W4_BAR LA_W4_SB
#define LA_W4_BLOCK_3 LA_W4_MF(0, 0, 0, 1, 3) LA_W4_RA(0, 0, 2, 0) LA_W4_MF(0, 0, 1, 1, 3) LA_W4_RA(0, 1, 3, 0) LA_W4_MF(0, 0, 2, 1, 3) LA_W4_PA0(saw, 0, bofs) LA_W4_MF(0, 0, 3, 1, 3) LA_W4_PA0(saw, 1, bofs) LA_W4_MF(0, 1, 0, 1, 3) LA_W4_MF(0, 1, 1, 1, 3) LA_W4_MF(0, 1, 2, 1, 3) LA_W4_MF(0, 1, 3, 1, 3)
#define LA_W4_BLOCK_4 LA_W4_MF(2, 0, 0, 0, 0) LA_W4_RA(1, 0, 2, 1) LA_W4_MF(2, 0, 1, 0, 0) LA_W4_RA(1, 1, 3, 1) LA_W4_MF(2, 0, 2, 0, 0) LA_W4_PA0(saw, 2, bofs) LA_W4_MF(2, 0, 3, 0, 0) LA_W4_PA0(saw, 3, bofs) LA_W4_MF(2, 1, 0, 0, 0) LA_W4_PW(sww, 0, bofs) LA_W4_MF(2, 1, 1, 0, 0) LA_W4_MF(2, 1, 2, 0, 0) LA_W4_MF(2, 1, 3, 0, 0)
#define LA_W4_BLOCK_5 LA_W4_MF(2, 0, 0, 1, 1) LA_W4_RA(0, 0, 2, 2) LA_W4_MF(2, 0, 1, 1, 1) LA_W4_RA(0, 1, 3, 2) LA_W4_MF(2, 0, 2, 1, 1) LA_W4_PW(sww, 1, bofs) LA_W4_MF(2, 0, 3, 1, 1) LA_W4_PW(sww, 2, bofs) LA_W4_MF(2, 1, 0, 1, 1) LA_W4_PW(sww, 3, bofs) LA_W4_MF(2, 1, 1, 1, 1) LA_W4_MF(2, 1, 2, 1, 1) LA_W4_MF(2, 1, 3, 1, 1)
#define LA_W4_BLOCK_6 LA_W4_MF(2, 0, 0, 0, 2) LA_W4_RA(1, 0, 2, 3) LA_W4_MF(2, 0, 1, 0, 2) LA_W4_RA(1, 1, 3, 3) LA_W4_MF(2, 0, 2, 0, 2) LA_W4_PW(sww, 4, bofs) LA_W4_MF(2, 0, 3, 0, 2) LA_W4_PW(sww, 5, bofs) LA_W4_MF(2, 1, 0, 0, 2) LA_W4_PW(sww, 6, bofs) LA_W4_MF(2, 1, 1, 0, 2) LA_W4_MF(2, 1, 2, 0, 2) LA_W4_WAIT(15) LA_W4_SB LA_W4_MF(2, 1, 3, 0, 2) LA_W4_BAR LA_W4_SB
#define LA_W4_BLOCK_7 LA_W4_MF(2, 0, 0, 1, 3) LA_W4_RA(0, 0, 0, 0) LA_W4_MF(2, 0, 1, 1, 3) LA_W4_RW(0, 0) LA_W4_MF(2, 0, 2, 1, 3) LA_W4_RW(0, 1) LA_W4_MF(2, 0, 3, 1, 3) LA_W4_RW(0, 2) LA_W4_MF(2, 1, 0, 1, 3) LA_W4_RW(0, 3) LA_W4_MF(2, 1, 1, 1, 3) LA_W4_RA(0, 1, 1, 0) LA_W4_MF(2, 1, 2, 1, 3) LA_W4_PW(sww, 7, bofs) LA_W4_MF(2, 1, 3, 1, 3)
#elif LA_W4_GROUP == 2
#define LA_W4_BLOCK_0 LA_W4_MF(0, 0, 0, 0, 0) LA_W4_RA(1, 0, 0, 1) LA_W4_RW(1, 0) LA_W4_MF(0, 0, 1, 0, 0) LA_W4_MF(0, 0, 2, 0, 0) LA_W4_RW(1, 1) LA_W4_RW(1, 2) LA_W4_MF(0, 0, 3, 0, 0) LA_W4_MF(0, 1, 0, 0, 0) LA_W4_RW(1, 3) LA_W4_RA(1, 1, 1, 1) LA_W4_MF(0, 1, 1, 0, 0) LA_W4_MF(0, 1, 2, 0, 0) LA_W4_PA1(sa1, 0, bo1) LA_W4_PA1(sa1, 1, bo1) LA_W4_MF(0, 1, 3, 0, 0)
#define LA_W4_BLOCK_1 LA_W4_MF(0, 0, 0, 1, 1) LA_W4_RA(0, 0, 0, 2) LA_W4_RW(2, 0) LA_W4_MF(0, 0, 1, 1, 1) LA_W4_MF(0, 0, 2, 1, 1) LA_W4_RW(2, 1) LA_W4_RW(2, 2) LA_W4_MF(0, 0, 3, 1, 1) LA_W4_MF(0, 1, 0, 1, 1) LA_W4_RW(2, 3) LA_W4_RA(0, 1, 1, 2) LA_W4_MF(0, 1, 1, 1, 1) LA_W4_MF(0, 1, 2, 1, 1) LA_W4_PA1(sa1, 2, bo1) LA_W4_MF(0, 1, 3, 1, 1)
#define LA_W4_BLOCK_2 LA_W4_MF(0, 0, 0, 0, 2) LA_W4_RA(1, 0, 0, 3) LA_W4_RW(3, 0) LA_W4_MF(0, 0, 1, 0, 2) LA_W4_MF(0, 0, 2, 0, 2) LA_W4_RW(3, 1) LA_W4_RW(3, 2) LA_W4_MF(0, 0, 3, 0, 2) LA_W4_MF(0, 1, 0, 0, 2) LA_W4_RW(3, 3) LA_W4_RA(1, 1, 1, 3) LA_W4_MF(0, 1, 1, 0, 2) LA_W4_MF(0, 1, 2, 0, 2) LA_W4_PA1(sa1, 3, bo1) LA_W4_WAIT(16) LA_W4_SB LA_W4_MF(0, 1, 3, 0, 2) LA_W4_BAR LA_W4_SB
#define LA_W4_BLOCK_3 LA_W4_MF(0, 0, 0, 1, 3) LA_W4_RA(0, 0, 2, 0) LA_W4_RA(0, 1, 3, 0) LA_W4_MF(0, 0, 1, 1, 3) LA_W4_MF(0, 0, 2, 1, 3) LA_W4_MF(0, 0, 3, 1, 3) LA_W4_MF(0, 1, 0, 1, 3) LA_W4_MF(0, 1, 1, 1, 3) LA_W4_MF(0, 1, 2, 1, 3) LA_W4_PA0(saw, 0, bofs) LA_W4_PA0(saw, 1, bofs) LA_W4_MF(0, 1, 3, 1, 3)
#define LA_W4_BLOCK_4 LA_W4_MF(2, 0, 0, 0, 0) LA_W4_RA(1, 0, 2, 1) LA_W4_RA(1, 1, 3, 1) LA_W4_MF(2, 0, 1, 0, 0) LA_W4_MF(2, 0, 2, 0, 0) LA_W4_MF(2, 0, 3, 0, 0) LA_W4_PA0(saw, 2, bofs) LA_W4_PA0(saw, 3, bofs) LA_W4_MF(2, 1, 0, 0, 0) LA_W4_MF(2, 1, 1, 0, 0) LA_W4_MF(2, 1, 2, 0, 0) LA_W4_PW(sww, 0, bofs) LA_W4_MF(2, 1, 3, 0, 0)
#define LA_W4_BLOCK_5 LA_W4_MF(2, 0, 0, 1, 1) LA_W4_RA(0, 0, 2, 2) LA_W4_RA(0, 1, 3, 2) LA_W4_MF(2, 0, 1, 1, 1) LA_W4_MF(2, 0, 2, 1, 1) LA_W4_MF(2, 0, 3, 1, 1) LA_W4_PW(sww, 1, bofs) LA_W4_PW(sww, 2, bofs) LA_W4_MF(2, 1, 0, 1, 1) LA_W4_MF(2, 1, 1, 1, 1) LA_W4_MF(2, 1, 2, 1, 1) LA_W4_PW(sww, 3, bofs) LA_W4_MF(2, 1, 3, 1, 1)
#define LA_W4_BLOCK_6 LA_W4_MF(2, 0, 0, 0, 2) LA_W4_RA(1, 0, 2, 3) LA_W4_RA(1, 1, 3, 3) LA_W4_MF(2, 0, 1, 0, 2) LA_W4_MF(2, 0, 2, 0, 2) LA_W4_MF(2, 0, 3, 0, 2) LA_W4_PW(sww, 4, bofs) LA_W4_PW(sww, 5, bofs) LA_W4_MF(2, 1, 0, 0, 2) LA_W4_MF(2, 1, 1, 0, 2) LA_W4_MF(2, 1, 2, 0, 2) LA_W4_PW(sww, 6, bofs) LA_W4_WAIT(15) LA_W4_SB LA_W4_MF(2, 1, 3, 0, 2) LA_W4_BAR LA_W4_SB
#define LA_W4_BLOCK_7 LA_W4_MF(2, 0, 0, 1, 3) LA_W4_RA(0, 0, 0, 0) LA_W4_RW(0, 0) LA_W4_MF(2, 0, 1, 1, 3) LA_W4_MF(2, 0, 2, 1, 3) LA_W4_RW(0, 1) LA_W4_RW(0, 2) LA_W4_MF(2, 0, 3, 1, 3) LA_W4_MF(2, 1, 0, 1, 3) LA_W4_RW(0, 3) LA_W4_RA(0, 1, 1, 0) LA_W4_MF(2, 1, 1, 1, 3) LA_W4_MF(2, 1, 2, 1, 3) LA_W4_PW(sww, 7, bofs) LA_W4_MF(2, 1, 3, 1, 3)
#elif LA_W4_GROUP == 3
#define LA_W4_BLOCK_0 LA_W4_MF(0, 0, 0, 0, 0) LA_W4_RA(1, 0, 0, 1) LA_W4_RW(1, 0) LA_W4_RW(1, 1) LA_W4_MF(0, 0, 1, 0, 0) LA_W4_MF(0, 0, 2, 0, 0) LA_W4_MF(0, 0, 3, 0, 0) LA_W4_RW(1, 2) LA_W4_RW(1, 3) LA_W4_RA(1, 1, 1, 1) LA_W4_MF(0, 1, 0, 0, 0) LA_W4_MF(0, 1, 1, 0, 0) LA_W4_MF(0, 1, 2, 0, 0) LA_W4_PA1(sa1, 0, bo1) LA_W4_PA1(sa1, 1, bo1) LA_W4_MF(0, 1, 3, 0, 0)
#define LA_W4_BLOCK_1 LA_W4_MF(0, 0, 0, 1, 1) LA_W4_RA(0, 0, 0, 2) LA_W4_RW(2, 0) LA_W4_RW(2, 1) LA_W4_MF(0, 0, 1, 1, 1) LA_W4_MF(0, 0, 2, 1, 1) LA_W4_MF(0, 0, 3, 1, 1) LA_W4_RW(2, 2) LA_W4_RW(2, 3) LA_W4_RA(0, 1, 1, 2) LA_W4_MF(0, 1, 0, 1, 1) LA_W4_MF(0, 1, 1, 1, 1) LA_W4_MF(0, 1, 2, 1, 1) LA_W4_PA1(sa1, 2, bo1) LA_W4_MF(0, 1, 3, 1, 1)
#define LA_W4_BLOCK_2 LA_W4_MF(0, 0, 0, 0, 2) LA_W4_RA(1, 0, 0, 3) LA_W4_RW(3, 0) LA_W4_RW(3, 1) LA_W4_MF(0, 0, 1, 0, 2) LA_W4_MF(0, 0, 2, 0, 2) LA_W4_MF(0, 0, 3, 0, 2) LA_W4_RW(3, 2) LA_W4_RW(3, 3) LA_W4_RA(1, 1, 1, 3) LA_W4_MF(0, 1, 0, 0, 2) LA_W4_MF(0, 1, 1, 0, 2) LA_W4_MF(0, 1, 2, 0, 2) LA_W4_PA1(sa1, 3, bo1) LA_W4_WAIT(16) LA_W4_SB LA_W4_MF(0, 1, 3, 0, 2) LA_W4_BAR LA_W4_SB
#define LA_W4_BLOCK_3 LA_W4_MF(0, 0, 0, 1, 3) LA_W4_RA(0, 0, 2, 0) LA_W4_RA(0, 1, 3, 0) LA_W4_PA0(saw, 0, bofs) LA_W4_MF(0, 0, 1, 1, 3) LA_W4_MF(0, 0, 2, 1, 3) LA_W4_MF(0, 0, 3, 1, 3) LA_W4_MF(0, 1, 0, 1, 3) LA_W4_MF(0, 1, 1, 1, 3) LA_W4_MF(0, 1, 2, 1, 3) LA_W4_PA0(saw, 1, bofs) LA_W4_MF(0, 1, 3, 1, 3)
#define LA_W4_BLOCK_4 LA_W4_MF(2, 0, 0, 0, 0) LA_W4_RA(1, 0, 2, 1) LA_W4_RA(1, 1, 3, 1) LA_W4_PA0(saw, 2, bofs) LA_W4_MF(2, 0, 1, 0, 0) LA_W4_MF(2, 0, 2, 0, 0) LA_W4_MF(2, 0, 3, 0, 0) LA_W4_MF(2, 1, 0, 0, 0) LA_W4_MF(2, 1, 1, 0, 0) LA_W4_MF(2, 1, 2, 0, 0) LA_W4_PA0(saw, 3, bofs) LA_W4_PW(sww, 0, bofs) LA_W4_MF(2, 1, 3, 0, 0)
#define LA_W4_BLOCK_5 LA_W4_MF(2, 0, 0, 1, 1) LA_W4_RA(0, 0, 2, 2) LA_W4_RA(0, 1, 3, 2) LA_W4_PW(sww, 1, bofs) LA_W4_MF(2, 0, 1, 1, 1) LA_W4_MF(2, 0, 2, 1, 1) LA_W4_MF(2, 0, 3, 1, 1) LA_W4_MF(2, 1, 0, 1, 1) LA_W4_MF(2, 1, 1, 1, 1) LA_W4_MF(2, 1, 2, 1, 1) LA_W4_PW(sww, 2, bofs) LA_W4_PW(sww, 3, bofs) LA_W4_MF(2, 1, 3, 1, 1)
#define LA_W4_BLOCK_6 LA_W4_MF(2, 0, 0, 0, 2) LA_W4_RA(1, 0, 2, 3) LA_W4_RA(1, 1, 3, 3) LA_W4_PW(sww, 4, bofs) LA_W4_MF(2, 0, 1, 0, 2) LA_W4_MF(2, 0, 2, 0, 2) LA_W4_MF(2, 0, 3, 0, 2) LA_W4_MF(2, 1, 0, 0, 2) LA_W4_MF(2, 1, 1, 0, 2) LA_W4_MF(2, 1, 2, 0, 2) LA_W4_PW(sww, 5, bofs) LA_W4_PW(sww, 6, bofs) LA_W4_WAIT(15) LA_W4_SB LA_W4_MF(2, 1, 3, 0, 2) LA_W4_BAR LA_W4_SB
#define LA_W4_BLOCK_7 LA_W4_MF(2, 0, 0, 1, 3) LA_W4_RA(0, 0, 0, 0) LA_W4_RW(0, 0) LA_W4_RW(0, 1) LA_W4_MF(2, 0, 1, 1, 3) LA_W4_MF(2, 0, 2, 1, 3) LA_W4_MF(2, 0, 3, 1, 3) LA_W4_RW(0, 2) LA_W4_RW(0, 3) LA_W4_RA(0, 1, 1, 0) LA_W4_MF(2, 1, 0, 1, 3) LA_W4_MF(2, 1, 1, 1, 3) LA_W4_MF(2, 1, 2, 1, 3) LA_W4_PW(sww, 7, bofs) LA_W4_MF(2, 1, 3, 1, 3)
#elif LA_W4_GROUP == 4
#define LA_W4_BLOCK_0 LA_W4_MF(0, 0, 0, 0, 0) LA_W4_RA(1, 0, 0, 1) LA_W4_RW(1, 0) LA_W4_RW(1, 1) LA_W4_RW(1, 2) LA_W4_MF(0, 0, 1, 0, 0) LA_W4_MF(0, 0, 2, 0, 0) LA_W4_MF(0, 0, 3, 0, 0) LA_W4_MF(0, 1, 0, 0, 0) LA_W4_MF(0, 1, 1, 0, 0) LA_W4_MF(0, 1, 2, 0, 0) LA_W4_RW(1, 3) LA_W4_RA(1, 1, 1, 1) LA_W4_PA1(sa1, 0, bo1) LA_W4_PA1(sa1, 1, bo1) LA_W4_MF(0, 1, 3, 0, 0)
#define LA_W4_BLOCK_1 LA_W4_MF(0, 0, 0, 1, 1) LA_W4_RA(0, 0, 0, 2) LA_W4_RW(2, 0) LA_W4_RW(2, 1) LA_W4_RW(2, 2) LA_W4_MF(0, 0, 1, 1, 1) LA_W4_MF(0, 0, 2, 1, 1) LA_W4_MF(0, 0, 3, 1, 1) LA_W4_MF(0, 1, 0, 1, 1) LA_W4_MF(0, 1, 1, 1, 1) LA_W4_MF(0, 1, 2, 1, 1) LA_W4_RW(2, 3) LA_W4_RA(0, 1, 1, 2) LA_W4_PA1(sa1, 2, bo1) LA_W4_MF(0, 1, 3, 1, 1)
#define LA_W4_BLOCK_2 LA_W4_MF(0, 0, 0, 0, 2) LA_W4_RA(1, 0, 0, 3) LA_W4_RW(3, 0) LA_W4_RW(3, 1) LA_W4_RW(3, 2) LA_W4_MF(0, 0, 1, 0, 2) LA_W4_MF(0, 0, 2, 0, 2) LA_W4_MF(0, 0, 3, 0, 2) LA_W4_MF(0, 1, 0, 0, 2) LA_W4_MF(0, 1, 1, 0, 2) LA_W4_MF(0, 1, 2, 0, 2) LA_W4_RW(3, 3) LA_W4_RA(1, 1, 1, 3) LA_W4_PA1(sa1, 3, bo1) LA_W4_WAIT(16) LA_W4_SB LA_W4_MF(0, 1, 3, 0, 2) LA_W4_BAR LA_W4_SB
#define LA_W4_BLOCK_3 LA_W4_MF(0, 0, 0, 1, 3) LA_W4_RA(0, 0, 2, 0) LA_W4_RA(0, 1, 3, 0) LA_W4_PA0(saw, 0, bofs) LA_W4_PA0(saw, 1, bofs) LA_W4_MF(0, 0, 1, 1, 3) LA_W4_MF(0, 0, 2, 1, 3) LA_W4_MF(0, 0, 3, 1, 3) LA_W4_MF(0, 1, 0, 1, 3) LA_W4_MF(0, 1, 1, 1, 3) LA_W4_MF(0, 1, 2, 1, 3) LA_W4_MF(0, 1, 3, 1, 3)
#define LA_W4_BLOCK_4 LA_W4_MF(2, 0, 0, 0, 0) LA_W4_RA(1, 0, 2, 1) LA_W4_RA(1, 1, 3, 1) LA_W4_PA0(saw, 2, bofs) LA_W4_PA0(saw, 3, bofs) LA_W4_MF(2, 0, 1, 0, 0) LA_W4_MF(2, 0, 2, 0, 0) LA_W4_MF(2, 0, 3, 0, 0) LA_W4_MF(2, 1, 0, 0, 0) LA_W4_MF(2, 1, 1, 0, 0) LA_W4_MF(2, 1, 2, 0, 0) LA_W4_PW(sww, 0, bofs) LA_W4_MF(2, 1, 3, 0, 0)
#define LA_W4_BLOCK_5 LA_W4_MF(2, 0, 0, 1, 1) LA_W4_RA(0, 0, 2, 2) LA_W4_RA(0, 1, 3, 2) LA_W4_PW(sww, 1, bofs) LA_W4_PW(sww, 2, bofs) LA_W4_MF(2, 0, 1, 1, 1) LA_W4_MF(2, 0, 2, 1, 1) LA_W4_MF(2, 0, 3, 1, 1) LA_W4_MF(2, 1, 0, 1, 1) LA_W4_MF(2, 1, 1, 1, 1) LA_W4_MF(2, 1, 2, 1, 1) LA_W4_PW(sww, 3, bofs) LA_W4_MF(2, 1, 3, 1, 1)
#define LA_W4_BLOCK_6 LA_W4_MF(2, 0, 0, 0, 2) LA_W4_RA(1, 0, 2, 3) LA_W4_RA(1, 1, 3, 3) LA_W4_PW(sww, 4, bofs) LA_W4_PW(sww, 5, bofs) LA_W4_MF(2, 0, 1, 0, 2) LA_W4_MF(2, 0, 2, 0, 2) LA_W4_MF(2, 0, 3, 0, 2) LA_W4_MF(2, 1, 0, 0, 2) LA_W4_MF(2, 1, 1, 0, 2) LA_W4_MF(2, 1, 2, 0, 2) LA_W4_PW(sww, 6, bofs) LA_W4_WAIT(15) LA_W4_SB LA_W4_MF(2, 1, 3, 0, 2) LA_W4_BAR LA_W4_SB
#define LA_W4_BLOCK_7 LA_W4_MF(2, 0, 0, 1, 3) LA_W4_RA(0, 0, 0, 0) LA_W4_RW(0, 0) LA_W4_RW(0, 1) LA_W4_RW(0, 2) LA_W4_MF(2, 0, 1, 1, 3) LA_W4_MF(2, 0, 2, 1, 3) LA_W4_MF(2, 0, 3, 1, 3) LA_W4_MF(2, 1, 0, 1, 3) LA_W4_MF(2, 1, 1, 1, 3) LA_W4_MF(2, 1, 2, 1, 3) LA_W4_RW(0, 3) LA_W4_RA(0, 1, 1, 0) LA_W4_PW(sww, 7, bofs) LA_W4_MF(2, 1, 3, 1, 3)
#elif LA_W4_GROUP == 8
#define LA_W4_BLOCK_0 LA_W4_MF(0, 0, 0, 0, 0) LA_W4_RA(1, 0, 0, 1) LA_W4_RW(1, 0) LA_W4_RW(1, 1) LA_W4_RW(1, 2) LA_W4_RW(1, 3) LA_W4_RA(1, 1, 1, 1) LA_W4_PA1(sa1, 0, bo1) LA_W4_PA1(sa1, 1, bo1) LA_W4_MF(0, 0, 1, 0, 0) LA_W4_MF(0, 0, 2, 0, 0) LA_W4_MF(0, 0, 3, 0, 0) LA_W4_MF(0, 1, 0, 0, 0) LA_W4_MF(0, 1, 1, 0, 0) LA_W4_MF(0, 1, 2, 0, 0) LA_W4_MF(0, 1, 3, 0, 0)
#define LA_W4_BLOCK_1 LA_W4_MF(0, 0, 0, 1, 1) LA_W4_RA(0, 0, 0, 2) LA_W4_RW(2, 0) LA_W4_RW(2, 1) LA_W4_RW(2, 2) LA_W4_RW(2, 3) LA_W4_RA(0, 1, 1, 2) LA_W4_PA1(sa1, 2, bo1) LA_W4_MF(0, 0, 1, 1, 1) LA_W4_MF(0, 0, 2, 1, 1) LA_W4_MF(0, 0, 3, 1, 1) LA_W4_MF(0, 1, 0, 1, 1) LA_W4_MF(0, 1, 1, 1, 1) LA_W4_MF(0, 1, 2, 1, 1) LA_W4_MF(0, 1, 3, 1, 1)
#define LA_W4_BLOCK_2 LA_W4_MF(0, 0, 0, 0, 2) LA_W4_RA(1, 0, 0, 3) LA_W4_RW(3, 0) LA_W4_RW(3, 1) LA_W4_RW(3, 2) LA_W4_RW(3, 3) LA_W4_RA(1, 1, 1, 3) LA_W4_PA1(sa1, 3, bo1) LA_W4_MF(0, 0, 1, 0, 2) LA_W4_MF(0, 0, 2, 0, 2) LA_W4_MF(0, 0, 3, 0, 2) LA_W4_MF(0, 1, 0, 0, 2) LA_W4_MF(0, 1, 1, 0, 2) LA_W4_MF(0, 1, 2, 0, 2) LA_W4_WAIT(16) LA_W4_SB LA_W4_MF(0, 1, 3, 0, 2) LA_W4_BAR LA_W4_SB
#define LA_W4_BLOCK_3 LA_W4_MF(0, 0, 0, 1, 3) LA_W4_RA(0, 0, 2, 0) LA_W4_RA(0, 1, 3, 0) LA_W4_PA0(saw, 0, bofs) LA_W4_PA0(saw, 1, bofs) LA_W4_MF(0, 0, 1, 1, 3) LA_W4_MF(0, 0, 2, 1, 3) LA_W4_MF(0, 0, 3, 1, 3) LA_W4_MF(0, 1, 0, 1, 3) LA_W4_MF(0, 1, 1, 1, 3) LA_W4_MF(0, 1, 2, 1, 3) LA_W4_MF(0, 1, 3, 1, 3)
#define LA_W4_BLOCK_4 LA_W4_MF(2, 0, 0, 0, 0) LA_W4_RA(1, 0, 2, 1) LA_W4_RA(1, 1, 3, 1) LA_W4_PA0(saw, 2, bofs) LA_W4_PA0(saw, 3, bofs) LA_W4_PW(sww, 0, bofs) LA_W4_MF(2, 0, 1, 0, 0) LA_W4_MF(2, 0, 2, 0, 0) LA_W4_MF(2, 0, 3, 0, 0) LA_W4_MF(2, 1, 0, 0, 0) LA_W4_MF(2, 1, 1, 0, 0) LA_W4_MF(2, 1, 2, 0, 0) LA_W4_MF(2, 1, 3, 0, 0)
#define LA_W4_BLOCK_5 LA_W4_MF(2, 0, 0, 1, 1) LA_W4_RA(0, 0, 2, 2) LA_W4_RA(0, 1, 3, 2) LA_W4_PW(sww, 1, bofs) LA_W4_PW(sww, 2, bofs) LA_W4_PW(sww, 3, bofs) LA_W4_MF(2, 0, 1, 1, 1) LA_W4_MF(2, 0, 2, 1, 1) LA_W4_MF(2, 0, 3, 1, 1) LA_W4_MF(2, 1, 0, 1, 1) LA_W4_MF(2, 1, 1, 1, 1) LA_W4_MF(2, 1, 2, 1, 1) LA_W4_MF(2, 1, 3, 1, 1)
#define LA_W4_BLOCK_6 LA_W4_MF(2, 0, 0, 0, 2) LA_W4_RA(1, 0, 2, 3) LA_W4_RA(1, 1, 3, 3) LA_W4_PW(sww, 4, bofs) LA_W4_PW(sww, 5, bofs) LA_W4_PW(sww, 6, bofs) LA_W4_MF(2, 0, 1, 0, 2) LA_W4_MF(2, 0, 2, 0, 2) LA_W4_MF(2, 0, 3, 0, 2) LA_W4_MF(2, 1, 0, 0, 2) LA_W4_MF(2, 1, 1, 0, 2) LA_W4_MF(2, 1, 2, 0, 2) LA_W4_WAIT(15) LA_W4_SB LA_W4_MF(2, 1, 3, 0, 2) LA_W4_BAR LA_W4_SB
#define LA_W4_BLOCK_7 LA_W4_MF(2, 0, 0, 1, 3) LA_W4_RA(0, 0, 0, 0) LA_W4_RW(0, 0) LA_W4_RW(0, 1) LA_W4_RW(0, 2) LA_W4_RW(0, 3) LA_W4_RA(0, 1, 1, 0) LA_W4_PW(sww, 7, bofs) LA_W4_MF(2, 0, 1, 1, 3) LA_W4_MF(2, 0, 2, 1, 3) LA_W4_MF(2, 0, 3, 1, 3) LA_W4_MF(2, 1, 0, 1, 3) LA_W4_MF(2, 1, 1, 1, 3) LA_W4_MF(2, 1, 2, 1, 3) LA_W4_MF(2, 1, 3, 1, 3)
#else
#error "LA_W4_GROUP must be 1, 2, 3, 4 or 8"
#endif
```

Before: 391.2 episodes/s.

## Add 16x16x32 MFMA main loop variant for the T256W direct GEMM kernel

Adds a second main-loop variant of the T256W GEMM kernel that uses v_mfma_f32_16x16x32 instructions instead of 32x32x16, with a matching LDS fragment layout, accumulator arrays, k-tile schedule and epilogue write-out. The planner enables it by default for direct-epilogue tiles, except some residual, ragged and special epilogues, and a variant bit can force the 32x32 path back. The aim is better MFMA throughput or issue and latency characteristics on MI355X. It raises the number of accumulator registers and instructions per tile, and adds a small standalone probe kernel for checking layout correctness.

```diff
diff --git a/include/la_hip.h b/include/la_hip.h
--- a/include/la_hip.h
+++ b/include/la_hip.h
@@ -12,6 +12,7 @@
 const char* la_last_error(void);
 int la_version(void);
 
+enum { LA_GEMM_VARIANT_MFMA32 = 0x10000 };
 int la_gemm_variant(int v);
 
 typedef struct LaGemmEpilogue {
@@ -49,11 +50,13 @@
 enum { LA_GEMM_NT = 0, LA_GEMM_DMA128, LA_GEMM_DMA256x128, LA_GEMM_T256, LA_GEMM_T256P, LA_GEMM_T256Q, LA_GEMM_T256W,
        LA_GEMM_F32_N32, LA_GEMM_F32_N128, LA_GEMM_F32_SMALL, LA_GEMM_SKINNY };
 typedef struct LaGemmPlan {
-  int kernel, epi, planes, direct, ragged, gm, ksplit, kchunk, grid, block, lds_bytes;
+  int kernel, epi, planes, direct, ragged, gm, ksplit, kchunk, grid, block, lds_bytes, mfma;
 } LaGemmPlan;
 
 int la_gemm_plan(const void* A, int lda, const void* W, int ldw, int M, int N, int K,
                  const LaGemmEpilogue* epi, int dt, int ncu, LaGemmPlan* out);
+
+int la_mfma_shape_probe(const void* A, const void* W, float* out, int K, int dt, int shape, void* stream);
 
 int la_conv3x3_f32(const float* in, int B, int H, int W, int Cin, const float* wt, const float* bias, int Cout, float* out32,
                    void* stream);
diff --git a/labelanything_amd/_lib.py b/labelanything_amd/_lib.py
--- a/labelanything_amd/_lib.py
+++ b/labelanything_amd/_lib.py
@@ -65,7 +65,11 @@
     "la_classify_wide", "la_classify_wide_bwd", "la_level_reduce", "la_level_reduce_bwd",
     "la_proto_kernels", "la_proto_kernels_bwd", "la_classify_conv", "la_classify_conv_bwd",
     "la_extract_pool_plan", "la_extract_pool", "la_extract_fold", "la_extract_unfold",
+    "la_mfma_shape_probe",
 ]
+
+
+GEMM_VARIANT_MFMA32 = 0x10000
 
 
 def gemm_variant(v: int = -1) -> int:
@@ -99,7 +103,7 @@
 
 
 class LaGemmPlan(C.Structure):
-    _fields_ = [(f, C.c_int) for f in ("kernel", "epi", "planes", "direct", "ragged", "gm", "ksplit", "kchunk", "grid", "block", "lds_bytes")]
+    _fields_ = [(f, C.c_int) for f in ("kernel", "epi", "planes", "direct", "ragged", "gm", "ksplit", "kchunk", "grid", "block", "lds_bytes", "mfma")]
 
 
 GEMM_KERNELS = ("NT", "DMA128", "DMA256x128", "T256", "T256P", "T256Q", "T256W", "F32_N32", "F32_N128", "F32_SMALL", "SKINNY")
@@ -163,6 +167,16 @@
     return plan
 
 
+def mfma_shape_probe(a: torch.Tensor, w: torch.Tensor, shape: int) -> torch.Tensor:
+    _dev(a)
+    if a.dtype != w.dtype or a.shape != w.shape or a.shape[0] != 32 or not (a.is_contiguous() and w.is_contiguous()):
+        raise RuntimeError("mfma_shape_probe: a and w must be contiguous [32, K] of one 16-bit type")
+    out = torch.empty(32, 32, device=a.device, dtype=torch.float32)
+    rc = lib().la_mfma_shape_probe(_ptr(a), _ptr(w), _ptr(out), C.c_int(a.shape[1]), C.c_int(dt_of(a)), C.c_int(shape), _stream())
+    _check(rc, "la_mfma_shape_probe")
+    return out
+
+
 def norm_finalize(part: Optional[torch.Tensor], m: int, e: int, eps: float, mr: torch.Tensor, x16: Optional[torch.Tensor] = None, rpg: int = 0,
                   cs_part: Optional[torch.Tensor] = None) -> None:
     _dev(mr)
diff --git a/labelanything_amd/csrc/gemm.hip b/labelanything_amd/csrc/gemm.hip
--- a/labelanything_amd/csrc/gemm.hip
+++ b/labelanything_amd/csrc/gemm.hip
@@ -1575,7 +1575,7 @@
                                  int variant, int* stg) {
   static const char *path = getenv("LA_GEMM_PATH"), *nop = getenv("LA_GEMM_NO_PERSISTENT"), *nosmall = getenv("LA_NO_F32_SMALL"),
                     *want = getenv("LA_KSPLIT_WANT"), *kgrid = getenv("LA_KSPLIT_GRID"), *gmenv = getenv("LA_GEMM_GROUP_M"),
-                    *w4grid = getenv("LA_W4_GRID"), *stagger = getenv("LA_W4_STAGGER");
+                    *w4grid = getenv("LA_W4_GRID"), *stagger = getenv("LA_W4_STAGGER"), *w4mfma = getenv("LA_W4_MFMA");
   const bool tiles16 = p->kernel <= LA_GEMM_T256P || (p->kernel == LA_GEMM_T256Q && p->epi != 4) || (p->kernel == LA_GEMM_T256W && p->epi <= 3);
   const int planes = p->planes;
   if (tiles16 && path && (path[0] == 'v' || p->kernel != LA_GEMM_NT)) {
@@ -1597,6 +1597,7 @@
   if (p->kernel == LA_GEMM_T256W) {
     if (w4grid && atoi(w4grid) > 0 && atoi(w4grid) < p->grid) p->grid = atoi(w4grid);
     if (stagger) *stg = (atoi(stagger) << 16) | (strchr(stagger, ',') ? atoi(strchr(stagger, ',') + 1) : 0);
+    if (w4mfma && p->direct) p->mfma = atoi(w4mfma) == 16 ? w4_mfma_shape(1, p->epi, p->ragged, 1 << 20, 0) : 0;
   }
 }
 #endif
@@ -1608,7 +1609,7 @@
 #ifdef LA_DEBUG
   if (v >= 0) la::g_gemm_variant = v;
 #else
-  if (v >= 0 && v <= 2) la::g_gemm_variant = v;
+  if (v >= 0 && (v & ~LA_GEMM_VARIANT_MFMA32) <= 2) la::g_gemm_variant = v;
 #endif
   return prev;
 }
diff --git a/labelanything_amd/csrc/gemm_plan.h b/labelanything_amd/csrc/gemm_plan.h
--- a/labelanything_amd/csrc/gemm_plan.h
+++ b/labelanything_amd/csrc/gemm_plan.h
@@ -34,6 +34,11 @@
   if (kernel == LA_GEMM_DMA128 || kernel == LA_GEMM_DMA256x128) return 8;
   if (kernel == LA_GEMM_T256Q || kernel == LA_GEMM_T256W) return N >= 2560 ? 8 : 2;
   return kernel == LA_GEMM_T256 || kernel == LA_GEMM_T256P ? 2 : 0;
+}
+
+static inline int w4_mfma_shape(int direct, int epi, int ragged, int K, int variant) {
+  const bool res_epi = epi == 3 || epi == 7 || epi == 10 || epi == 11;
+  return direct && epi != 12 && !(epi == 9 && ragged) && !(res_epi && K < 1536) && !(variant & LA_GEMM_VARIANT_MFMA32) ? 1 : 0;
 }
 
 static inline int persistent_grid(long ntiles, int ncu) { return ntiles < ncu ? (int)ntiles : ncu; }
@@ -109,11 +114,13 @@
     p->gm |= variant & 0xf500;
     p->direct = e.map == LA_MAP_NONE && !e.vt && !((variant >> 8) & 1);
     p->ragged = p->direct && (M & 255) != 0;
+    p->mfma = w4_mfma_shape(p->direct, p->epi, p->ragged, K, variant);
   }
 }
 
 static inline void plan_w4_fused(LaGemmPlan* p, int epi, int M, int N, int K, int ncu, int variant) {
   p->epi = epi, p->direct = 1, p->ragged = (M & 255) != 0;
+  p->mfma = w4_mfma_shape(1, epi, p->ragged, K, variant);
   plan_launch(p, LA_GEMM_T256W, M, N, K, ncu, variant);
 }
 
diff --git a/labelanything_amd/csrc/gemm_w4.hip b/labelanything_amd/csrc/gemm_w4.hip
--- a/labelanything_amd/csrc/gemm_w4.hip
+++ b/labelanything_amd/csrc/gemm_w4.hip
@@ -32,14 +32,33 @@
   }
 };
 
+template <typename T> struct MfmaA16;
+template <> struct MfmaA16<f16_t> {
+  static __device__ __forceinline__ void go(f32x4& c, const u32x4& a, const u32x4& b) {
+    asm volatile("v_mfma_f32_16x16x32_f16 %0, %1, %2, %0" : "+a"(c) : "v"(a), "v"(b));
+  }
+};
+template <> struct MfmaA16<bf16_t> {
+  static __device__ __forceinline__ void go(f32x4& c, const u32x4& a, const u32x4& b) {
+    asm volatile("v_mfma_f32_16x16x32_bf16 %0, %1, %2, %0" : "+a"(c) : "v"(a), "v"(b));
+  }
+};
+
 __device__ __forceinline__ void acc_zero(f32x16& c) {
   const u32x4 z = {0u, 0u, 0u, 0u};
   asm volatile("s_nop 1\n\tv_mfma_f32_32x32x16_f16 %0, %1, %1, 0" : "=a"(c) : "v"(z));
 }
+__device__ __forceinline__ void acc_zero(f32x4& c) {
+  const u32x4 z = {0u, 0u, 0u, 0u};
+  asm volatile("s_nop 1\n\tv_mfma_f32_16x16x32_f16 %0, %1, %1, 0" : "=a"(c) : "v"(z));
+}
+template <int MS> struct W4Acc { typedef f32x16 type[2][4][2]; };
+template <> struct W4Acc<1> { typedef f32x4 type[8][8]; };
 
 #ifdef LA_DEBUG
 constexpr int LA_W4_NSTAMP = 128;
 __device__ unsigned long long g_w4_stamps[4 * LA_W4_NSTAMP];
+__device__ unsigned long long g_w4_rstamps[4 * LA_W4_NSTAMP];
 #endif
 
 template <int BYTES> struct GWords;
@@ -62,6 +81,11 @@
   LA_W4_SB
 #define LA_W4_RW(KS, j) if constexpr (!(ABL & 2)) wf[KS][j] = lds_read16(waddr[KS] + (j) * 4096); LA_W4_SB
 #define LA_W4_RA(PAR, ii, i, KS) if constexpr (!(ABL & 2)) af[PAR][ii] = lds_read16(aaddr[KS] + (i) * 4096); LA_W4_SB
+#define LA_W4_MF16(bi, bj, PAR, ii, KS)                                                      \
+  if constexpr (!(ABL & 8)) MfmaA16<T>::go(acc[bi][bj], af[PAR][ii], wf[KS][bj]); \
+  LA_W4_SB
+#define LA_W4_RW16(KS, j) if constexpr (!(ABL & 2)) wf[KS][j] = lds_read16(waddr[KS] + (j) * 2048); LA_W4_SB
+#define LA_W4_RA16(PAR, ii, bi, KS) if constexpr (!(ABL & 2)) af[PAR][ii] = lds_read16(aaddr[KS] + (bi) * 2048); LA_W4_SB
 #define LA_W4_PA0(src, i, bo) if constexpr (!(ABL & 1)) dma_piece<(i) * 1024>(src, soA0[i], dstA + (bo)); LA_W4_SB
 #define LA_W4_PA1(src, i, bo) if constexpr (!(ABL & 1)) dma_piece<8192 + (i) * 1024>(src, soA1[i], dstA + (bo)); LA_W4_SB
 #define LA_W4_PW(src, i, bo) if constexpr (!(ABL & 1)) dma_piece<(i) * 1024>(src, soW[i], dstW + (bo)); LA_W4_SB
@@ -79,15 +103,16 @@
 #endif
 #include "gemm_w4_ktile.inc"
 
-template <typename T, int EPI, bool RAGGED>
-__device__ __forceinline__ void epilogue_w4(char* slab, f32x16 (&acc)[2][4][2], int row0, int col0, const LaGemmEpilogue& e, int lane, int M, int N) {
+template <typename T, int EPI, bool RAGGED, int MS = 0>
+__device__ __forceinline__ void epilogue_w4(char* slab, typename W4Acc<MS>::type& acc, int row0, int col0, const LaGemmEpilogue& e, int lane, int M, int N) {
   row0 = __builtin_amdgcn_readfirstlane(row0);
   col0 = __builtin_amdgcn_readfirstlane(col0);
   asm volatile("" : "+v"(lane));
   const int fr = lane & 31, fh = lane >> 5;
   const int rq = lane >> 3, cg = lane & 7;
   const unsigned sl = lds_addr_of(slab);
-  const unsigned waddr = sl + (unsigned)((fh * 64 + (fr & ~7) + ((fr & 7) ^ (((fr >> 3) ^ fh) & 7))) << 4);
+  const unsigned waddr = MS ? sl + (unsigned)(((lane >> 4) * 64 + (lane & 8) + ((lane & 7) ^ ((((lane >> 3) & 1) ^ (lane >> 4)) & 7))) << 4)
+                            : sl + (unsigned)((fh * 64 + (fr & ~7) + ((fr & 7) ^ (((fr >> 3) ^ fh) & 7))) << 4);
   unsigned raddr[8];
 #pragma unroll
   for (int t = 0; t < 8; ++t) raddr[t] = sl + (unsigned)((rq * 64 + cg * 8 + (t ^ ((cg ^ rq) & 7))) << 4);
@@ -148,14 +173,24 @@
   T* out16 = reinterpret_cast<T*>(e.out16);
   auto wr = [&](auto ic, auto jpc) {
     constexpr int i = decltype(ic)::value, jp = decltype(jpc)::value;
-#pragma unroll
-    for (int jj = 0; jj < 2; ++jj)
-#pragma unroll
-      for (int g = 0; g < 4; ++g) {
-        const f32x4 v = {acc[jp][i][jj][4 * g], acc[jp][i][jj][4 * g + 1], acc[jp][i][jj][4 * g + 2], acc[jp][i][jj][4 * g + 3]};
-        const unsigned a = (waddr ^ (unsigned)((((4 * jj) ^ (2 * g)) & 7) << 4)) + (unsigned)(g * 2048 + jj * 512);
-        *reinterpret_cast<__attribute__((address_space(3))) f32x4*>((uintptr_t)a) = v;
-      }
+    if constexpr (MS == 1) {
+#pragma unroll
+      for (int bil = 0; bil < 2; ++bil)
+#pragma unroll
+        for (int bjl = 0; bjl < 4; ++bjl) {
+          const unsigned a = (waddr ^ (unsigned)((((2 * bjl) ^ (4 * bil)) & 7) << 4)) + (unsigned)(bil * 4096 + bjl * 256);
+          *reinterpret_cast<__attribute__((address_space(3))) f32x4*>((uintptr_t)a) = acc[2 * i + bil][4 * jp + bjl];
+        }
+    } else {
+#pragma unroll
+      for (int jj = 0; jj < 2; ++jj)
+#pragma unroll
+        for (int g = 0; g < 4; ++g) {
+          const f32x4 v = {acc[jp][i][jj][4 * g], acc[jp][i][jj][4 * g + 1], acc[jp][i][jj][4 * g + 2], acc[jp][i][jj][4 * g + 3]};
+          const unsigned a = (waddr ^ (unsigned)((((4 * jj) ^ (2 * g)) & 7) << 4)) + (unsigned)(g * 2048 + jj * 512);
+          *reinterpret_cast<__attribute__((address_space(3))) f32x4*>((uintptr_t)a) = v;
+        }
+    }
   };
   f32x4 rd0[8];
   auto rd = [&](f32x4 (&r)[8]) {
@@ -519,11 +554,14 @@
   __builtin_amdgcn_sched_barrier(0);
 }
 
-template <typename T, int EPI, int ABL, bool DIRECT, bool RAGGED = false>
+template <typename T, int EPI, int ABL, bool DIRECT, bool RAGGED = false, int MS = 0>
 __global__ __launch_bounds__(256, 1) void gemm_t256w_kernel(const T* __restrict__ A, int lda, const T* __restrict__ Wt, int ldw, int M, int N,
                                                              int K, LaGemmEpilogue e, int gm, int stg) {
+  static_assert(MS == 0 || (MS == 1 && DIRECT), "the 16x16x32 main loop exists with the direct epilogue only");
   constexpr int BK_ = 64;
   constexpr unsigned REG = 32768;
+  constexpr int NKS = MS ? 2 : 4, NWF = MS ? 8 : 4;
+  constexpr unsigned FRAG = MS ? 2048 : 4096;
   constexpr int SEAM = (EPI == 3 || EPI == 5 || EPI == 7 || EPI >= 10) ? 47 : 32;
   extern __shared__ __attribute__((aligned(16))) char smem[];
   const int tid = threadIdx.x, lane = tid & 63, wave = __builtin_amdgcn_readfirstlane(tid >> 6);
@@ -532,9 +570,10 @@
   int stamp_i = 0;
   auto stamp = [&](int tag) {
     if (stamps && stamp_i < LA_W4_NSTAMP) {
-      unsigned long long t_;
-      asm volatile("s_memtime %0\n\ts_waitcnt lgkmcnt(0)" : "=s"(t_)::"memory");
+      unsigned long long t_, r_;
+      asm volatile("s_memtime %0\n\ts_memrealtime %1\n\ts_waitcnt lgkmcnt(0)" : "=s"(t_), "=s"(r_)::"memory");
       if (lane == 0) g_w4_stamps[wave * LA_W4_NSTAMP + stamp_i] = (t_ << 8) | (unsigned)tag;
+      if (lane == 0) g_w4_rstamps[wave * LA_W4_NSTAMP + stamp_i] = r_;
       ++stamp_i;
     }
   };
@@ -559,12 +598,13 @@
   unsigned* rtab = nullptr;
   if (EPI == 1 && e.map != LA_MAP_NONE) rtab = reinterpret_cast<unsigned*>(slab + 2048);
 
-  unsigned aaddr[4], waddr[4];
-#pragma unroll
-  for (int ks = 0; ks < 4; ++ks) {
-    const unsigned coff = (unsigned)(((ks * 2 + fh) ^ ((fr >> 1) & 7)) << 4);
-    aaddr[ks] = lds0 + (wr * 128 + fr) * 128 + coff;
-    waddr[ks] = lds0 + 2 * REG + (wc * 128 + fr) * 128 + coff;
+  unsigned aaddr[NKS], waddr[NKS];
+#pragma unroll
+  for (int ks = 0; ks < NKS; ++ks) {
+    const int r_ = MS ? (lane & 15) : fr;
+    const unsigned coff = (unsigned)(((MS ? ks * 4 + (lane >> 4) : ks * 2 + fh) ^ ((r_ >> 1) & 7)) << 4);
+    aaddr[ks] = lds0 + (wr * 128 + r_) * 128 + coff;
+    waddr[ks] = lds0 + 2 * REG + (wc * 128 + r_) * 128 + coff;
   }
   const unsigned dstA = lds0 + (wave >> 1) * 16384 + (wave & 1) * 4096;
   const unsigned dstW = lds0 + 2 * REG + wave * 8192;
@@ -594,15 +634,26 @@
     }
   };
 
-  f32x16 acc[2][4][2];
-#pragma unroll
-  for (int h = 0; h < 2; ++h)
-#pragma unroll
-    for (int i = 0; i < 4; ++i)
-#pragma unroll
-      for (int j = 0; j < 2; ++j)
-        acc_zero(acc[h][i][j]);
-  u32x4 wf[4][4], af[2][2];
+  typename W4Acc<MS>::type acc;
+  auto acc_clear = [&]() {
+    if constexpr (MS == 1) {
+#pragma unroll
+      for (int i = 0; i < 8; ++i)
+#pragma unroll
+        for (int j = 0; j < 8; ++j)
+          acc_zero(acc[i][j]);
+    } else {
+#pragma unroll
+      for (int h = 0; h < 2; ++h)
+#pragma unroll
+        for (int i = 0; i < 4; ++i)
+#pragma unroll
+          for (int j = 0; j < 2; ++j)
+            acc_zero(acc[h][i][j]);
+    }
+  };
+  acc_clear();
+  u32x4 wf[NKS][NWF], af[2][2];
 
   int tile = blockIdx.x;
   plan(tile, m0, n0, soA0, soA1, soW);
@@ -625,9 +676,9 @@
   __builtin_amdgcn_s_barrier();
   asm volatile("" ::: "memory");
 #pragma unroll
-  for (int j = 0; j < 4; ++j) wf[0][j] = lds_read16(waddr[0] + j * 4096);
-#pragma unroll
-  for (int ii = 0; ii < 2; ++ii) af[0][ii] = lds_read16(aaddr[0] + ii * 4096);
+  for (int j = 0; j < NWF; ++j) wf[0][j] = lds_read16(waddr[0] + j * FRAG);
+#pragma unroll
+  for (int ii = 0; ii < 2; ++ii) af[0][ii] = lds_read16(aaddr[0] + ii * FRAG);
   waddr[0] ^= REG;
 
   int kt = 0;
@@ -645,22 +696,40 @@
     }
     const T* sa1 = A + a_koff(e, kA1 * BK_);
     const unsigned bo1 = bofs ^ REG;
-    LA_W4_BLOCK_0
-    LA_W4_BLOCK_1
-    LA_W4_BLOCK_2
+    if constexpr (MS == 1) {
+      LA_W4_BLOCK16_0
+      LA_W4_BLOCK16_1
+      LA_W4_BLOCK16_2
+    } else {
+      LA_W4_BLOCK_0
+      LA_W4_BLOCK_1
+      LA_W4_BLOCK_2
+    }
     if (prelast && more) plan(next, m0n, n0n, soA0, soA1n, soW);
     const T* saw = A + a_koff(e, kAW * BK_);
     const T* sww = Wt + kAW * BK_;
 #pragma unroll
-    for (int ks = 1; ks < 4; ++ks) waddr[ks] ^= REG;
-    LA_W4_BLOCK_3
-    aaddr[0] ^= REG;
-    LA_W4_BLOCK_4
-    LA_W4_BLOCK_5
-    LA_W4_BLOCK_6
-#pragma unroll
-    for (int ks = 1; ks < 4; ++ks) aaddr[ks] ^= REG;
-    LA_W4_BLOCK_7
+    for (int ks = 1; ks < NKS; ++ks) waddr[ks] ^= REG;
+    if constexpr (MS == 1) {
+      LA_W4_BLOCK16_3
+      LA_W4_BLOCK16_4
+      aaddr[0] ^= REG;
+      LA_W4_BLOCK16_5
+      LA_W4_BLOCK16_6
+    } else {
+      LA_W4_BLOCK_3
+      aaddr[0] ^= REG;
+      LA_W4_BLOCK_4
+      LA_W4_BLOCK_5
+      LA_W4_BLOCK_6
+    }
+#pragma unroll
+    for (int ks = 1; ks < NKS; ++ks) aaddr[ks] ^= REG;
+    if constexpr (MS == 1) {
+      LA_W4_BLOCK16_7
+    } else {
+      LA_W4_BLOCK_7
+    }
     waddr[0] ^= REG;
     bofs ^= REG;
     seam = false;
@@ -669,10 +738,17 @@
     stamp(2);
     asm volatile("s_nop 15" ::: "memory");
     const bool vtile = !DIRECT && EPI == 1 && e.vt != nullptr && n0 >= e.vt_col0;
-#pragma unroll
-    for (int i = 0; i < 4; ++i)
-#pragma unroll
-      for (int j = 0; j < 2; ++j) asm volatile("" : "+a"(acc[0][i][j]));
+    if constexpr (MS == 1) {
+#pragma unroll
+      for (int i = 0; i < 8; ++i)
+#pragma unroll
+        for (int j = 0; j < 8; ++j) asm volatile("" : "+a"(acc[i][j]));
+    } else {
+#pragma unroll
+      for (int i = 0; i < 4; ++i)
+#pragma unroll
+        for (int j = 0; j < 2; ++j) asm volatile("" : "+a"(acc[0][i][j]));
+    }
     constexpr bool STASH = DIRECT && EPI >= 7;
     const unsigned stash = dstA + 8192 + (bofs ^ REG) + (unsigned)lane * 64;
     if constexpr (STASH) {
@@ -683,7 +759,9 @@
                    : "v"(stash), "v"(q0), "v"(q1), "v"(q2), "v"(q3)
                    : "memory");
     }
-    if constexpr (DIRECT) {
+    if constexpr (MS == 1) {
+      epilogue_w4<T, EPI, RAGGED, 1>(slab, acc, m0 + wr * 128, n0 + wc * 128, e, lane, M, N);
+    } else if constexpr (DIRECT) {
 #pragma unroll
       for (int i = 0; i < 4; ++i)
 #pragma unroll
@@ -715,31 +793,36 @@
         soW[4 + i] = q3[i];
       }
     }
-#pragma unroll
-    for (int h = 0; h < 2; ++h)
-#pragma unroll
-      for (int i = 0; i < 4; ++i)
-#pragma unroll
-        for (int j = 0; j < 2; ++j)
-          acc_zero(acc[h][i][j]);
+    acc_clear();
     m0 = m0n;
     n0 = n0n;
     tile = next;
     kt = 0;
     if constexpr (DIRECT) {
 #pragma unroll
-      for (int j = 0; j < 4; ++j) wf[0][j] = lds_read16((waddr[0] ^ REG) + j * 4096);
-#pragma unroll
-      for (int ii = 0; ii < 2; ++ii) af[0][ii] = lds_read16((aaddr[0]) + ii * 4096);
+      for (int j = 0; j < NWF; ++j) wf[0][j] = lds_read16((waddr[0] ^ REG) + j * FRAG);
+#pragma unroll
+      for (int ii = 0; ii < 2; ++ii) af[0][ii] = lds_read16((aaddr[0]) + ii * FRAG);
     }
     stamp(1);
   }
   asm volatile("s_waitcnt vmcnt(0)" ::: "memory");
 }
 
-template <typename T, int EPI, int ABL, bool DIRECT, bool RAGGED = false>
+template <typename T, int EPI, int ABL, bool DIRECT, bool RAGGED = false, int MS = 0>
 static void launch_t256w_abl(const LaGemmPlan& p, const GemmArgs& g, int stg) {
-  launch<T, gemm_t256w_kernel<T, EPI, ABL, DIRECT, RAGGED>>(dim3(p.grid), p, g, p.gm & 0x5ff, stg);
+  launch<T, gemm_t256w_kernel<T, EPI, ABL, DIRECT, RAGGED, MS>>(dim3(p.grid), p, g, p.gm & 0x5ff, stg);
+}
+
+template <typename T, int EPI>
+static void launch_t256w_direct(const LaGemmPlan& p, const GemmArgs& g, int stg) {
+  if constexpr (EPI != 12) {
+    if (p.mfma == 1 && !p.ragged) return launch_t256w_abl<T, EPI, 0, true, false, 1>(p, g, stg);
+    if constexpr (EPI != 9)
+      if (p.mfma == 1) return launch_t256w_abl<T, EPI, 0, true, true, 1>(p, g, stg);
+  }
+  if (!p.ragged) launch_t256w_abl<T, EPI, 0, true>(p, g, stg);
+  else launch_t256w_abl<T, EPI, 0, true, true>(p, g, stg);
 }
 
 template <typename T, int EPI>
@@ -747,15 +830,13 @@
 #ifdef LA_DEBUG
   if (EPI == 1 && with_int<1, 2, 3, 4, 5, 7, 8, 14>((p.gm >> 12) & 15, [&](auto abl) { launch_t256w_abl<T, 1, LA_V(abl), false>(p, g, stg); })) return;
 #endif
-  if (p.direct && !p.ragged) launch_t256w_abl<T, EPI, 0, true>(p, g, stg);
-  else if (p.direct) launch_t256w_abl<T, EPI, 0, true, true>(p, g, stg);
+  if (p.direct) launch_t256w_direct<T, EPI>(p, g, stg);
   else launch_t256w_abl<T, EPI, 0, false>(p, g, stg);
 }
 
 template <typename T, int EPI>
 void launch_t256w_fused(const LaGemmPlan& p, const GemmArgs& g, int stg) {
-  if (!p.ragged) launch_t256w_abl<T, EPI, 0, true>(p, g, stg);
-  else launch_t256w_abl<T, EPI, 0, true, true>(p, g, stg);
+  launch_t256w_direct<T, EPI>(p, g, stg);
 }
 #define LA_W4_FUSED(T, EPI) template void launch_t256w_fused<T, EPI>(const LaGemmPlan&, const GemmArgs&, int);
 LA_W4_FUSED(f16_t, 5) LA_W4_FUSED(f16_t, 6) LA_W4_FUSED(bf16_t, 5) LA_W4_FUSED(bf16_t, 6)
@@ -772,8 +853,13 @@
   (void)hipDeviceSynchronize();
   return (int)hipMemcpyFromSymbol(host_out, HIP_SYMBOL(la::g_w4_stamps), sizeof(unsigned long long) * 4 * la::LA_W4_NSTAMP);
 }
+extern "C" int la_dbg_w4_rstamps(unsigned long long* host_out) {
+  (void)hipDeviceSynchronize();
+  return (int)hipMemcpyFromSymbol(host_out, HIP_SYMBOL(la::g_w4_rstamps), sizeof(unsigned long long) * 4 * la::LA_W4_NSTAMP);
+}
 extern "C" int la_dbg_w4_stamps_clear() {
   static unsigned long long z[4 * la::LA_W4_NSTAMP] = {0};
-  return (int)hipMemcpyToSymbol(HIP_SYMBOL(la::g_w4_stamps), z, sizeof(z));
+  const int rc = (int)hipMemcpyToSymbol(HIP_SYMBOL(la::g_w4_stamps), z, sizeof(z));
+  return rc ? rc : (int)hipMemcpyToSymbol(HIP_SYMBOL(la::g_w4_rstamps), z, sizeof(z));
 }
 #endif
diff --git a/labelanything_amd/csrc/gemm_w4_ktile.inc b/labelanything_amd/csrc/gemm_w4_ktile.inc
--- a/labelanything_amd/csrc/gemm_w4_ktile.inc
+++ b/labelanything_amd/csrc/gemm_w4_ktile.inc
@@ -46,3 +46,49 @@
 #else
 #error "LA_W4_GROUP must be 1, 2, 3, 4 or 8"
 #endif
+#if LA_W4_GROUP == 1
+#define LA_W4_BLOCK16_0 LA_W4_MF16(0, 0, 0, 0, 0) LA_W4_RA16(1, 0, 2, 0) LA_W4_MF16(0, 1, 0, 0, 0) LA_W4_RA16(1, 1, 3, 0) LA_W4_MF16(0, 2, 0, 0, 0) LA_W4_RW16(1, 0) LA_W4_MF16(0, 3, 0, 0, 0) LA_W4_RW16(1, 1) LA_W4_MF16(0, 4, 0, 0, 0) LA_W4_RW16(1, 2) LA_W4_MF16(0, 5, 0, 0, 0) LA_W4_RW16(1, 3) LA_W4_MF16(0, 6, 0, 0, 0) LA_W4_PA1(sa1, 0, bo1) LA_W4_MF16(0, 7, 0, 0, 0) LA_W4_PA1(sa1, 1, bo1) LA_W4_MF16(1, 0, 0, 1, 0) LA_W4_MF16(1, 1, 0, 1, 0) LA_W4_MF16(1, 2, 0, 1, 0) LA_W4_MF16(1, 3, 0, 1, 0) LA_W4_MF16(1, 4, 0, 1, 0) LA_W4_MF16(1, 5, 0, 1, 0) LA_W4_MF16(1, 6, 0, 1, 0) LA_W4_MF16(1, 7, 0, 1, 0)
+#define LA_W4_BLOCK16_1 LA_W4_MF16(2, 0, 1, 0, 0) LA_W4_RA16(0, 0, 0, 1) LA_W4_MF16(2, 1, 1, 0, 0) LA_W4_RW16(1, 4) LA_W4_MF16(2, 2, 1, 0, 0) LA_W4_RW16(1, 5) LA_W4_MF16(2, 3, 1, 0, 0) LA_W4_RW16(1, 6) LA_W4_MF16(2, 4, 1, 0, 0) LA_W4_RW16(1, 7) LA_W4_MF16(2, 5, 1, 0, 0) LA_W4_RA16(0, 1, 1, 1) LA_W4_MF16(2, 6, 1, 0, 0) LA_W4_PA1(sa1, 2, bo1) LA_W4_MF16(2, 7, 1, 0, 0) LA_W4_MF16(3, 0, 1, 1, 0) LA_W4_MF16(3, 1, 1, 1, 0) LA_W4_MF16(3, 2, 1, 1, 0) LA_W4_MF16(3, 3, 1, 1, 0) LA_W4_MF16(3, 4, 1, 1, 0) LA_W4_MF16(3, 5, 1, 1, 0) LA_W4_MF16(3, 6, 1, 1, 0) LA_W4_MF16(3, 7, 1, 1, 0)
+#define LA_W4_BLOCK16_2 LA_W4_MF16(0, 0, 0, 0, 1) LA_W4_RA16(1, 0, 2, 1) LA_W4_MF16(0, 1, 0, 0, 1) LA_W4_RA16(1, 1, 3, 1) LA_W4_MF16(0, 2, 0, 0, 1) LA_W4_PA1(sa1, 3, bo1) LA_W4_MF16(0, 3, 0, 0, 1) LA_W4_MF16(0, 4, 0, 0, 1) LA_W4_MF16(0, 5, 0, 0, 1) LA_W4_MF16(0, 6, 0, 0, 1) LA_W4_MF16(0, 7, 0, 0, 1) LA_W4_MF16(1, 0, 0, 1, 1) LA_W4_MF16(1, 1, 0, 1, 1) LA_W4_MF16(1, 2, 0, 1, 1) LA_W4_MF16(1, 3, 0, 1, 1) LA_W4_MF16(1, 4, 0, 1, 1) LA_W4_MF16(1, 5, 0, 1, 1) LA_W4_MF16(1, 6, 0, 1, 1) LA_W4_WAIT(16) LA_W4_SB LA_W4_MF16(1, 7, 0, 1, 1) LA_W4_BAR LA_W4_SB
+#define LA_W4_BLOCK16_3 LA_W4_MF16(2, 0, 1, 0, 1) LA_W4_RA16(0, 0, 4, 0) LA_W4_MF16(2, 1, 1, 0, 1) LA_W4_RA16(0, 1, 5, 0) LA_W4_MF16(2, 2, 1, 0, 1) LA_W4_PA0(saw, 0, bofs) LA_W4_MF16(2, 3, 1, 0, 1) LA_W4_PA0(saw, 1, bofs) LA_W4_MF16(2, 4, 1, 0, 1) LA_W4_MF16(2, 5, 1, 0, 1) LA_W4_MF16(2, 6, 1, 0, 1) LA_W4_MF16(2, 7, 1, 0, 1) LA_W4_MF16(3, 0, 1, 1, 1) LA_W4_MF16(3, 1, 1, 1, 1) LA_W4_MF16(3, 2, 1, 1, 1) LA_W4_MF16(3, 3, 1, 1, 1) LA_W4_MF16(3, 4, 1, 1, 1) LA_W4_MF16(3, 5, 1, 1, 1) LA_W4_MF16(3, 6, 1, 1, 1) LA_W4_MF16(3, 7, 1, 1, 1)
+#define LA_W4_BLOCK16_4 LA_W4_MF16(4, 0, 0, 0, 0) LA_W4_RA16(1, 0, 6, 0) LA_W4_MF16(4, 1, 0, 0, 0) LA_W4_RA16(1, 1, 7, 0) LA_W4_MF16(4, 2, 0, 0, 0) LA_W4_PA0(saw, 2, bofs) LA_W4_MF16(4, 3, 0, 0, 0) LA_W4_PA0(saw, 3, bofs) LA_W4_MF16(4, 4, 0, 0, 0) LA_W4_PW(sww, 0, bofs) LA_W4_MF16(4, 5, 0, 0, 0) LA_W4_MF16(4, 6, 0, 0, 0) LA_W4_MF16(4, 7, 0, 0, 0) LA_W4_MF16(5, 0, 0, 1, 0) LA_W4_MF16(5, 1, 0, 1, 0) LA_W4_MF16(5, 2, 0, 1, 0) LA_W4_MF16(5, 3, 0, 1, 0) LA_W4_MF16(5, 4, 0, 1, 0) LA_W4_MF16(5, 5, 0, 1, 0) LA_W4_MF16(5, 6, 0, 1, 0) LA_W4_MF16(5, 7, 0, 1, 0)
+#define LA_W4_BLOCK16_5 LA_W4_MF16(6, 0, 1, 0, 0) LA_W4_RA16(0, 0, 4, 1) LA_W4_MF16(6, 1, 1, 0, 0) LA_W4_RA16(0, 1, 5, 1) LA_W4_MF16(6, 2, 1, 0, 0) LA_W4_PW(sww, 1, bofs) LA_W4_MF16(6, 3, 1, 0, 0) LA_W4_PW(sww, 2, bofs) LA_W4_MF16(6, 4, 1, 0, 0) LA_W4_PW(sww, 3, bofs) LA_W4_MF16(6, 5, 1, 0, 0) LA_W4_MF16(6, 6, 1, 0, 0) LA_W4_MF16(6, 7, 1, 0, 0) LA_W4_MF16(7, 0, 1, 1, 0) LA_W4_MF16(7, 1, 1, 1, 0) LA_W4_MF16(7, 2, 1, 1, 0) LA_W4_MF16(7, 3, 1, 1, 0) LA_W4_MF16(7, 4, 1, 1, 0) LA_W4_MF16(7, 5, 1, 1, 0) LA_W4_MF16(7, 6, 1, 1, 0) LA_W4_MF16(7, 7, 1, 1, 0)
+#define LA_W4_BLOCK16_6 LA_W4_MF16(4, 0, 0, 0, 1) LA_W4_RA16(1, 0, 6, 1) LA_W4_MF16(4, 1, 0, 0, 1) LA_W4_RA16(1, 1, 7, 1) LA_W4_MF16(4, 2, 0, 0, 1) LA_W4_PW(sww, 4, bofs) LA_W4_MF16(4, 3, 0, 0, 1) LA_W4_PW(sww, 5, bofs) LA_W4_MF16(4, 4, 0, 0, 1) LA_W4_PW(sww, 6, bofs) LA_W4_MF16(4, 5, 0, 0, 1) LA_W4_MF16(4, 6, 0, 0, 1) LA_W4_MF16(4, 7, 0, 0, 1) LA_W4_MF16(5, 0, 0, 1, 1) LA_W4_MF16(5, 1, 0, 1, 1) LA_W4_MF16(5, 2, 0, 1, 1) LA_W4_MF16(5, 3, 0, 1, 1) LA_W4_MF16(5, 4, 0, 1, 1) LA_W4_MF16(5, 5, 0, 1, 1) LA_W4_MF16(5, 6, 0, 1, 1) LA_W4_WAIT(15) LA_W4_SB LA_W4_MF16(5, 7, 0, 1, 1) LA_W4_BAR LA_W4_SB
+#define LA_W4_BLOCK16_7 LA_W4_MF16(6, 0, 1, 0, 1) LA_W4_RA16(0, 0, 0, 0) LA_W4_MF16(6, 1, 1, 0, 1) LA_W4_RW16(0, 0) LA_W4_MF16(6, 2, 1, 0, 1) LA_W4_RW16(0, 1) LA_W4_MF16(6, 3, 1, 0, 1) LA_W4_RW16(0, 2) LA_W4_MF16(6, 4, 1, 0, 1) LA_W4_RW16(0, 3) LA_W4_MF16(6, 5, 1, 0, 1) LA_W4_RW16(0, 4) LA_W4_MF16(6, 6, 1, 0, 1) LA_W4_RW16(0, 5) LA_W4_MF16(6, 7, 1, 0, 1) LA_W4_RW16(0, 6) LA_W4_MF16(7, 0, 1, 1, 1) LA_W4_RW16(0, 7) LA_W4_MF16(7, 1, 1, 1, 1) LA_W4_RA16(0, 1, 1, 0) LA_W4_MF16(7, 2, 1, 1, 1) LA_W4_PW(sww, 7, bofs) LA_W4_MF16(7, 3, 1, 1, 1) LA_W4_MF16(7, 4, 1, 1, 1) LA_W4_MF16(7, 5, 1, 1, 1) LA_W4_MF16(7, 6, 1, 1, 1) LA_W4_MF16(7, 7, 1, 1, 1)
+#elif LA_W4_GROUP == 2
+#define LA_W4_BLOCK16_0 LA_W4_MF16(0, 0, 0, 0, 0) LA_W4_RA16(1, 0, 2, 0) LA_W4_RA16(1, 1, 3, 0) LA_W4_MF16(0, 1, 0, 0, 0) LA_W4_MF16(0, 2, 0, 0, 0) LA_W4_MF16(0, 3, 0, 0, 0) LA_W4_MF16(0, 4, 0, 0, 0) LA_W4_RW16(1, 0) LA_W4_RW16(1, 1) LA_W4_MF16(0, 5, 0, 0, 0) LA_W4_MF16(0, 6, 0, 0, 0) LA_W4_MF16(0, 7, 0, 0, 0) LA_W4_MF16(1, 0, 0, 1, 0) LA_W4_MF16(1, 1, 0, 1, 0) LA_W4_RW16(1, 2) LA_W4_RW16(1, 3) LA_W4_MF16(1, 2, 0, 1, 0) LA_W4_MF16(1, 3, 0, 1, 0) LA_W4_MF16(1, 4, 0, 1, 0) LA_W4_MF16(1, 5, 0, 1, 0) LA_W4_MF16(1, 6, 0, 1, 0) LA_W4_PA1(sa1, 0, bo1) LA_W4_PA1(sa1, 1, bo1) LA_W4_MF16(1, 7, 0, 1, 0)
+#define LA_W4_BLOCK16_1 LA_W4_MF16(2, 0, 1, 0, 0) LA_W4_RA16(0, 0, 0, 1) LA_W4_RW16(1, 4) LA_W4_MF16(2, 1, 1, 0, 0) LA_W4_MF16(2, 2, 1, 0, 0) LA_W4_MF16(2, 3, 1, 0, 0) LA_W4_MF16(2, 4, 1, 0, 0) LA_W4_RW16(1, 5) LA_W4_RW16(1, 6) LA_W4_MF16(2, 5, 1, 0, 0) LA_W4_MF16(2, 6, 1, 0, 0) LA_W4_MF16(2, 7, 1, 0, 0) LA_W4_MF16(3, 0, 1, 1, 0) LA_W4_MF16(3, 1, 1, 1, 0) LA_W4_RW16(1, 7) LA_W4_RA16(0, 1, 1, 1) LA_W4_MF16(3, 2, 1, 1, 0) LA_W4_MF16(3, 3, 1, 1, 0) LA_W4_MF16(3, 4, 1, 1, 0) LA_W4_MF16(3, 5, 1, 1, 0) LA_W4_MF16(3, 6, 1, 1, 0) LA_W4_PA1(sa1, 2, bo1) LA_W4_MF16(3, 7, 1, 1, 0)
+#define LA_W4_BLOCK16_2 LA_W4_MF16(0, 0, 0, 0, 1) LA_W4_RA16(1, 0, 2, 1) LA_W4_RA16(1, 1, 3, 1) LA_W4_MF16(0, 1, 0, 0, 1) LA_W4_MF16(0, 2, 0, 0, 1) LA_W4_MF16(0, 3, 0, 0, 1) LA_W4_MF16(0, 4, 0, 0, 1) LA_W4_MF16(0, 5, 0, 0, 1) LA_W4_MF16(0, 6, 0, 0, 1) LA_W4_MF16(0, 7, 0, 0, 1) LA_W4_MF16(1, 0, 0, 1, 1) LA_W4_MF16(1, 1, 0, 1, 1) LA_W4_MF16(1, 2, 0, 1, 1) LA_W4_MF16(1, 3, 0, 1, 1) LA_W4_MF16(1, 4, 0, 1, 1) LA_W4_MF16(1, 5, 0, 1, 1) LA_W4_MF16(1, 6, 0, 1, 1) LA_W4_PA1(sa1, 3, bo1) LA_W4_WAIT(16) LA_W4_SB LA_W4_MF16(1, 7, 0, 1, 1) LA_W4_BAR LA_W4_SB
+#define LA_W4_BLOCK16_3 LA_W4_MF16(2, 0, 1, 0, 1) LA_W4_RA16(0, 0, 4, 0) LA_W4_RA16(0, 1, 5, 0) LA_W4_MF16(2, 1, 1, 0, 1) LA_W4_MF16(2, 2, 1, 0, 1) LA_W4_MF16(2, 3, 1, 0, 1) LA_W4_MF16(2, 4, 1, 0, 1) LA_W4_MF16(2, 5, 1, 0, 1) LA_W4_MF16(2, 6, 1, 0, 1) LA_W4_MF16(2, 7, 1, 0, 1) LA_W4_MF16(3, 0, 1, 1, 1) LA_W4_MF16(3, 1, 1, 1, 1) LA_W4_MF16(3, 2, 1, 1, 1) LA_W4_MF16(3, 3, 1, 1, 1) LA_W4_MF16(3, 4, 1, 1, 1) LA_W4_MF16(3, 5, 1, 1, 1) LA_W4_MF16(3, 6, 1, 1, 1) LA_W4_PA0(saw, 0, bofs) LA_W4_PA0(saw, 1, bofs) LA_W4_MF16(3, 7, 1, 1, 1)
+#define LA_W4_BLOCK16_4 LA_W4_MF16(4, 0, 0, 0, 0) LA_W4_RA16(1, 0, 6, 0) LA_W4_RA16(1, 1, 7, 0) LA_W4_MF16(4, 1, 0, 0, 0) LA_W4_MF16(4, 2, 0, 0, 0) LA_W4_MF16(4, 3, 0, 0, 0) LA_W4_MF16(4, 4, 0, 0, 0) LA_W4_MF16(4, 5, 0, 0, 0) LA_W4_MF16(4, 6, 0, 0, 0) LA_W4_MF16(4, 7, 0, 0, 0) LA_W4_PA0(saw, 2, bofs) LA_W4_PA0(saw, 3, bofs) LA_W4_MF16(5, 0, 0, 1, 0) LA_W4_MF16(5, 1, 0, 1, 0) LA_W4_MF16(5, 2, 0, 1, 0) LA_W4_MF16(5, 3, 0, 1, 0) LA_W4_MF16(5, 4, 0, 1, 0) LA_W4_MF16(5, 5, 0, 1, 0) LA_W4_MF16(5, 6, 0, 1, 0) LA_W4_PW(sww, 0, bofs) LA_W4_MF16(5, 7, 0, 1, 0)
+#define LA_W4_BLOCK16_5 LA_W4_MF16(6, 0, 1, 0, 0) LA_W4_RA16(0, 0, 4, 1) LA_W4_RA16(0, 1, 5, 1) LA_W4_MF16(6, 1, 1, 0, 0) LA_W4_MF16(6, 2, 1, 0, 0) LA_W4_MF16(6, 3, 1, 0, 0) LA_W4_MF16(6, 4, 1, 0, 0) LA_W4_MF16(6, 5, 1, 0, 0) LA_W4_MF16(6, 6, 1, 0, 0) LA_W4_MF16(6, 7, 1, 0, 0) LA_W4_PW(sww, 1, bofs) LA_W4_PW(sww, 2, bofs) LA_W4_MF16(7, 0, 1, 1, 0) LA_W4_MF16(7, 1, 1, 1, 0) LA_W4_MF16(7, 2, 1, 1, 0) LA_W4_MF16(7, 3, 1, 1, 0) LA_W4_MF16(7, 4, 1, 1, 0) LA_W4_MF16(7, 5, 1, 1, 0) LA_W4_MF16(7, 6, 1, 1, 0) LA_W4_PW(sww, 3, bofs) LA_W4_MF16(7, 7, 1, 1, 0)
+#define LA_W4_BLOCK16_6 LA_W4_MF16(4, 0, 0, 0, 1) LA_W4_RA16(1, 0, 6, 1) LA_W4_RA16(1, 1, 7, 1) LA_W4_MF16(4, 1, 0, 0, 1) LA_W4_MF16(4, 2, 0, 0, 1) LA_W4_MF16(4, 3, 0, 0, 1) LA_W4_MF16(4, 4, 0, 0, 1) LA_W4_MF16(4, 5, 0, 0, 1) LA_W4_MF16(4, 6, 0, 0, 1) LA_W4_MF16(4, 7, 0, 0, 1) LA_W4_PW(sww, 4, bofs) LA_W4_PW(sww, 5, bofs) LA_W4_MF16(5, 0, 0, 1, 1) LA_W4_MF16(5, 1, 0, 1, 1) LA_W4_MF16(5, 2, 0, 1, 1) LA_W4_MF16(5, 3, 0, 1, 1) LA_W4_MF16(5, 4, 0, 1, 1) LA_W4_MF16(5, 5, 0, 1, 1) LA_W4_MF16(5, 6, 0, 1, 1) LA_W4_PW(sww, 6, bofs) LA_W4_WAIT(15) LA_W4_SB LA_W4_MF16(5, 7, 0, 1, 1) LA_W4_BAR LA_W4_SB
+#define LA_W4_BLOCK16_7 LA_W4_MF16(6, 0, 1, 0, 1) LA_W4_RA16(0, 0, 0, 0) LA_W4_RW16(0, 0) LA_W4_MF16(6, 1, 1, 0, 1) LA_W4_MF16(6, 2, 1, 0, 1) LA_W4_RW16(0, 1) LA_W4_RW16(0, 2) LA_W4_MF16(6, 3, 1, 0, 1) LA_W4_MF16(6, 4, 1, 0, 1) LA_W4_MF16(6, 5, 1, 0, 1) LA_W4_RW16(0, 3) LA_W4_RW16(0, 4) LA_W4_MF16(6, 6, 1, 0, 1) LA_W4_MF16(6, 7, 1, 0, 1) LA_W4_MF16(7, 0, 1, 1, 1) LA_W4_RW16(0, 5) LA_W4_RW16(0, 6) LA_W4_MF16(7, 1, 1, 1, 1) LA_W4_MF16(7, 2, 1, 1, 1) LA_W4_MF16(7, 3, 1, 1, 1) LA_W4_RW16(0, 7) LA_W4_RA16(0, 1, 1, 0) LA_W4_MF16(7, 4, 1, 1, 1) LA_W4_MF16(7, 5, 1, 1, 1) LA_W4_MF16(7, 6, 1, 1, 1) LA_W4_PW(sww, 7, bofs) LA_W4_MF16(7, 7, 1, 1, 1)
+#elif LA_W4_GROUP == 3
+#define LA_W4_BLOCK16_0 LA_W4_MF16(0, 0, 0, 0, 0) LA_W4_RA16(1, 0, 2, 0) LA_W4_RA16(1, 1, 3, 0) LA_W4_RW16(1, 0) LA_W4_MF16(0, 1, 0, 0, 0) LA_W4_MF16(0, 2, 0, 0, 0) LA_W4_MF16(0, 3, 0, 0, 0) LA_W4_MF16(0, 4, 0, 0, 0) LA_W4_MF16(0, 5, 0, 0, 0) LA_W4_MF16(0, 6, 0, 0, 0) LA_W4_MF16(0, 7, 0, 0, 0) LA_W4_RW16(1, 1) LA_W4_RW16(1, 2) LA_W4_RW16(1, 3) LA_W4_MF16(1, 0, 0, 1, 0) LA_W4_MF16(1, 1, 0, 1, 0) LA_W4_MF16(1, 2, 0, 1, 0) LA_W4_MF16(1, 3, 0, 1, 0) LA_W4_MF16(1, 4, 0, 1, 0) LA_W4_MF16(1, 5, 0, 1, 0) LA_W4_MF16(1, 6, 0, 1, 0) LA_W4_PA1(sa1, 0, bo1) LA_W4_PA1(sa1, 1, bo1) LA_W4_MF16(1, 7, 0, 1, 0)
+#define LA_W4_BLOCK16_1 LA_W4_MF16(2, 0, 1, 0, 0) LA_W4_RA16(0, 0, 0, 1) LA_W4_RW16(1, 4) LA_W4_RW16(1, 5) LA_W4_MF16(2, 1, 1, 0, 0) LA_W4_MF16(2, 2, 1, 0, 0) LA_W4_MF16(2, 3, 1, 0, 0) LA_W4_MF16(2, 4, 1, 0, 0) LA_W4_MF16(2, 5, 1, 0, 0) LA_W4_MF16(2, 6, 1, 0, 0) LA_W4_MF16(2, 7, 1, 0, 0) LA_W4_RW16(1, 6) LA_W4_RW16(1, 7) LA_W4_RA16(0, 1, 1, 1) LA_W4_MF16(3, 0, 1, 1, 0) LA_W4_MF16(3, 1, 1, 1, 0) LA_W4_MF16(3, 2, 1, 1, 0) LA_W4_MF16(3, 3, 1, 1, 0) LA_W4_MF16(3, 4, 1, 1, 0) LA_W4_MF16(3, 5, 1, 1, 0) LA_W4_MF16(3, 6, 1, 1, 0) LA_W4_PA1(sa1, 2, bo1) LA_W4_MF16(3, 7, 1, 1, 0)
+#define LA_W4_BLOCK16_2 LA_W4_MF16(0, 0, 0, 0, 1) LA_W4_RA16(1, 0, 2, 1) LA_W4_RA16(1, 1, 3, 1) LA_W4_PA1(sa1, 3, bo1) LA_W4_MF16(0, 1, 0, 0, 1) LA_W4_MF16(0, 2, 0, 0, 1) LA_W4_MF16(0, 3, 0, 0, 1) LA_W4_MF16(0, 4, 0, 0, 1) LA_W4_MF16(0, 5, 0, 0, 1) LA_W4_MF16(0, 6, 0, 0, 1) LA_W4_MF16(0, 7, 0, 0, 1) LA_W4_MF16(1, 0, 0, 1, 1) LA_W4_MF16(1, 1, 0, 1, 1) LA_W4_MF16(1, 2, 0, 1, 1) LA_W4_MF16(1, 3, 0, 1, 1) LA_W4_MF16(1, 4, 0, 1, 1) LA_W4_MF16(1, 5, 0, 1, 1) LA_W4_MF16(1, 6, 0, 1, 1) LA_W4_WAIT(16) LA_W4_SB LA_W4_MF16(1, 7, 0, 1, 1) LA_W4_BAR LA_W4_SB
+#define LA_W4_BLOCK16_3 LA_W4_MF16(2, 0, 1, 0, 1) LA_W4_RA16(0, 0, 4, 0) LA_W4_RA16(0, 1, 5, 0) LA_W4_PA0(saw, 0, bofs) LA_W4_MF16(2, 1, 1, 0, 1) LA_W4_MF16(2, 2, 1, 0, 1) LA_W4_MF16(2, 3, 1, 0, 1) LA_W4_MF16(2, 4, 1, 0, 1) LA_W4_MF16(2, 5, 1, 0, 1) LA_W4_MF16(2, 6, 1, 0, 1) LA_W4_MF16(2, 7, 1, 0, 1) LA_W4_MF16(3, 0, 1, 1, 1) LA_W4_MF16(3, 1, 1, 1, 1) LA_W4_MF16(3, 2, 1, 1, 1) LA_W4_MF16(3, 3, 1, 1, 1) LA_W4_MF16(3, 4, 1, 1, 1) LA_W4_MF16(3, 5, 1, 1, 1) LA_W4_MF16(3, 6, 1, 1, 1) LA_W4_PA0(saw, 1, bofs) LA_W4_MF16(3, 7, 1, 1, 1)
+#define LA_W4_BLOCK16_4 LA_W4_MF16(4, 0, 0, 0, 0) LA_W4_RA16(1, 0, 6, 0) LA_W4_RA16(1, 1, 7, 0) LA_W4_PA0(saw, 2, bofs) LA_W4_MF16(4, 1, 0, 0, 0) LA_W4_MF16(4, 2, 0, 0, 0) LA_W4_MF16(4, 3, 0, 0, 0) LA_W4_MF16(4, 4, 0, 0, 0) LA_W4_MF16(4, 5, 0, 0, 0) LA_W4_MF16(4, 6, 0, 0, 0) LA_W4_MF16(4, 7, 0, 0, 0) LA_W4_MF16(5, 0, 0, 1, 0) LA_W4_MF16(5, 1, 0, 1, 0) LA_W4_MF16(5, 2, 0, 1, 0) LA_W4_MF16(5, 3, 0, 1, 0) LA_W4_MF16(5, 4, 0, 1, 0) LA_W4_MF16(5, 5, 0, 1, 0) LA_W4_MF16(5, 6, 0, 1, 0) LA_W4_PA0(saw, 3, bofs) LA_W4_PW(sww, 0, bofs) LA_W4_MF16(5, 7, 0, 1, 0)
+#define LA_W4_BLOCK16_5 LA_W4_MF16(6, 0, 1, 0, 0) LA_W4_RA16(0, 0, 4, 1) LA_W4_RA16(0, 1, 5, 1) LA_W4_PW(sww, 1, bofs) LA_W4_MF16(6, 1, 1, 0, 0) LA_W4_MF16(6, 2, 1, 0, 0) LA_W4_MF16(6, 3, 1, 0, 0) LA_W4_MF16(6, 4, 1, 0, 0) LA_W4_MF16(6, 5, 1, 0, 0) LA_W4_MF16(6, 6, 1, 0, 0) LA_W4_MF16(6, 7, 1, 0, 0) LA_W4_MF16(7, 0, 1, 1, 0) LA_W4_MF16(7, 1, 1, 1, 0) LA_W4_MF16(7, 2, 1, 1, 0) LA_W4_MF16(7, 3, 1, 1, 0) LA_W4_MF16(7, 4, 1, 1, 0) LA_W4_MF16(7, 5, 1, 1, 0) LA_W4_MF16(7, 6, 1, 1, 0) LA_W4_PW(sww, 2, bofs) LA_W4_PW(sww, 3, bofs) LA_W4_MF16(7, 7, 1, 1, 0)
+#define LA_W4_BLOCK16_6 LA_W4_MF16(4, 0, 0, 0, 1) LA_W4_RA16(1, 0, 6, 1) LA_W4_RA16(1, 1, 7, 1) LA_W4_PW(sww, 4, bofs) LA_W4_MF16(4, 1, 0, 0, 1) LA_W4_MF16(4, 2, 0, 0, 1) LA_W4_MF16(4, 3, 0, 0, 1) LA_W4_MF16(4, 4, 0, 0, 1) LA_W4_MF16(4, 5, 0, 0, 1) LA_W4_MF16(4, 6, 0, 0, 1) LA_W4_MF16(4, 7, 0, 0, 1) LA_W4_MF16(5, 0, 0, 1, 1) LA_W4_MF16(5, 1, 0, 1, 1) LA_W4_MF16(5, 2, 0, 1, 1) LA_W4_MF16(5, 3, 0, 1, 1) LA_W4_MF16(5, 4, 0, 1, 1) LA_W4_MF16(5, 5, 0, 1, 1) LA_W4_MF16(5, 6, 0, 1, 1) LA_W4_PW(sww, 5, bofs) LA_W4_PW(sww, 6, bofs) LA_W4_WAIT(15) LA_W4_SB LA_W4_MF16(5, 7, 0, 1, 1) LA_W4_BAR LA_W4_SB
+#define LA_W4_BLOCK16_7 LA_W4_MF16(6, 0, 1, 0, 1) LA_W4_RA16(0, 0, 0, 0) LA_W4_RW16(0, 0) LA_W4_RW16(0, 1) LA_W4_MF16(6, 1, 1, 0, 1) LA_W4_MF16(6, 2, 1, 0, 1) LA_W4_MF16(6, 3, 1, 0, 1) LA_W4_MF16(6, 4, 1, 0, 1) LA_W4_RW16(0, 2) LA_W4_RW16(0, 3) LA_W4_RW16(0, 4) LA_W4_MF16(6, 5, 1, 0, 1) LA_W4_MF16(6, 6, 1, 0, 1) LA_W4_MF16(6, 7, 1, 0, 1) LA_W4_MF16(7, 0, 1, 1, 1) LA_W4_MF16(7, 1, 1, 1, 1) LA_W4_RW16(0, 5) LA_W4_RW16(0, 6) LA_W4_RW16(0, 7) LA_W4_MF16(7, 2, 1, 1, 1) LA_W4_MF16(7, 3, 1, 1, 1) LA_W4_MF16(7, 4, 1, 1, 1) LA_W4_MF16(7, 5, 1, 1, 1) LA_W4_MF16(7, 6, 1, 1, 1) LA_W4_RA16(0, 1, 1, 0) LA_W4_PW(sww, 7, bofs) LA_W4_MF16(7, 7, 1, 1, 1)
+#elif LA_W4_GROUP == 4
+#define LA_W4_BLOCK16_0 LA_W4_MF16(0, 0, 0, 0, 0) LA_W4_RA16(1, 0, 2, 0) LA_W4_RA16(1, 1, 3, 0) LA_W4_RW16(1, 0) LA_W4_RW16(1, 1) LA_W4_MF16(0, 1, 0, 0, 0) LA_W4_MF16(0, 2, 0, 0, 0) LA_W4_MF16(0, 3, 0, 0, 0) LA_W4_MF16(0, 4, 0, 0, 0) LA_W4_MF16(0, 5, 0, 0, 0) LA_W4_MF16(0, 6, 0, 0, 0) LA_W4_MF16(0, 7, 0, 0, 0) LA_W4_MF16(1, 0, 0, 1, 0) LA_W4_MF16(1, 1, 0, 1, 0) LA_W4_MF16(1, 2, 0, 1, 0) LA_W4_MF16(1, 3, 0, 1, 0) LA_W4_MF16(1, 4, 0, 1, 0) LA_W4_MF16(1, 5, 0, 1, 0) LA_W4_MF16(1, 6, 0, 1, 0) LA_W4_RW16(1, 2) LA_W4_RW16(1, 3) LA_W4_PA1(sa1, 0, bo1) LA_W4_PA1(sa1, 1, bo1) LA_W4_MF16(1, 7, 0, 1, 0)
+#define LA_W4_BLOCK16_1 LA_W4_MF16(2, 0, 1, 0, 0) LA_W4_RA16(0, 0, 0, 1) LA_W4_RW16(1, 4) LA_W4_RW16(1, 5) LA_W4_RW16(1, 6) LA_W4_MF16(2, 1, 1, 0, 0) LA_W4_MF16(2, 2, 1, 0, 0) LA_W4_MF16(2, 3, 1, 0, 0) LA_W4_MF16(2, 4, 1, 0, 0) LA_W4_MF16(2, 5, 1, 0, 0) LA_W4_MF16(2, 6, 1, 0, 0) LA_W4_MF16(2, 7, 1, 0, 0) LA_W4_MF16(3, 0, 1, 1, 0) LA_W4_MF16(3, 1, 1, 1, 0) LA_W4_MF16(3, 2, 1, 1, 0) LA_W4_MF16(3, 3, 1, 1, 0) LA_W4_MF16(3, 4, 1, 1, 0) LA_W4_MF16(3, 5, 1, 1, 0) LA_W4_MF16(3, 6, 1, 1, 0) LA_W4_RW16(1, 7) LA_W4_RA16(0, 1, 1, 1) LA_W4_PA1(sa1, 2, bo1) LA_W4_MF16(3, 7, 1, 1, 0)
+#define LA_W4_BLOCK16_2 LA_W4_MF16(0, 0, 0, 0, 1) LA_W4_RA16(1, 0, 2, 1) LA_W4_RA16(1, 1, 3, 1) LA_W4_PA1(sa1, 3, bo1) LA_W4_MF16(0, 1, 0, 0, 1) LA_W4_MF16(0, 2, 0, 0, 1) LA_W4_MF16(0, 3, 0, 0, 1) LA_W4_MF16(0, 4, 0, 0, 1) LA_W4_MF16(0, 5, 0, 0, 1) LA_W4_MF16(0, 6, 0, 0, 1) LA_W4_MF16(0, 7, 0, 0, 1) LA_W4_MF16(1, 0, 0, 1, 1) LA_W4_MF16(1, 1, 0, 1, 1) LA_W4_MF16(1, 2, 0, 1, 1) LA_W4_MF16(1, 3, 0, 1, 1) LA_W4_MF16(1, 4, 0, 1, 1) LA_W4_MF16(1, 5, 0, 1, 1) LA_W4_MF16(1, 6, 0, 1, 1) LA_W4_WAIT(16) LA_W4_SB LA_W4_MF16(1, 7, 0, 1, 1) LA_W4_BAR LA_W4_SB
+#define LA_W4_BLOCK16_3 LA_W4_MF16(2, 0, 1, 0, 1) LA_W4_RA16(0, 0, 4, 0) LA_W4_RA16(0, 1, 5, 0) LA_W4_PA0(saw, 0, bofs) LA_W4_PA0(saw, 1, bofs) LA_W4_MF16(2, 1, 1, 0, 1) LA_W4_MF16(2, 2, 1, 0, 1) LA_W4_MF16(2, 3, 1, 0, 1) LA_W4_MF16(2, 4, 1, 0, 1) LA_W4_MF16(2, 5, 1, 0, 1) LA_W4_MF16(2, 6, 1, 0, 1) LA_W4_MF16(2, 7, 1, 0, 1) LA_W4_MF16(3, 0, 1, 1, 1) LA_W4_MF16(3, 1, 1, 1, 1) LA_W4_MF16(3, 2, 1, 1, 1) LA_W4_MF16(3, 3, 1, 1, 1) LA_W4_MF16(3, 4, 1, 1, 1) LA_W4_MF16(3, 5, 1, 1, 1) LA_W4_MF16(3, 6, 1, 1, 1) LA_W4_MF16(3, 7, 1, 1, 1)
+#define LA_W4_BLOCK16_4 LA_W4_MF16(4, 0, 0, 0, 0) LA_W4_RA16(1, 0, 6, 0) LA_W4_RA16(1, 1, 7, 0) LA_W4_PA0(saw, 2, bofs) LA_W4_PA0(saw, 3, bofs) LA_W4_MF16(4, 1, 0, 0, 0) LA_W4_MF16(4, 2, 0, 0, 0) LA_W4_MF16(4, 3, 0, 0, 0) LA_W4_MF16(4, 4, 0, 0, 0) LA_W4_MF16(4, 5, 0, 0, 0) LA_W4_MF16(4, 6, 0, 0, 0) LA_W4_MF16(4, 7, 0, 0, 0) LA_W4_MF16(5, 0, 0, 1, 0) LA_W4_MF16(5, 1, 0, 1, 0) LA_W4_MF16(5, 2, 0, 1, 0) LA_W4_MF16(5, 3, 0, 1, 0) LA_W4_MF16(5, 4, 0, 1, 0) LA_W4_MF16(5, 5, 0, 1, 0) LA_W4_MF16(5, 6, 0, 1, 0) LA_W4_PW(sww, 0, bofs) LA_W4_MF16(5, 7, 0, 1, 0)
+#define LA_W4_BLOCK16_5 LA_W4_MF16(6, 0, 1, 0, 0) LA_W4_RA16(0, 0, 4, 1) LA_W4_RA16(0, 1, 5, 1) LA_W4_PW(sww, 1, bofs) LA_W4_PW(sww, 2, bofs) LA_W4_MF16(6, 1, 1, 0, 0) LA_W4_MF16(6, 2, 1, 0, 0) LA_W4_MF16(6, 3, 1, 0, 0) LA_W4_MF16(6, 4, 1, 0, 0) LA_W4_MF16(6, 5, 1, 0, 0) LA_W4_MF16(6, 6, 1, 0, 0) LA_W4_MF16(6, 7, 1, 0, 0) LA_W4_MF16(7, 0, 1, 1, 0) LA_W4_MF16(7, 1, 1, 1, 0) LA_W4_MF16(7, 2, 1, 1, 0) LA_W4_MF16(7, 3, 1, 1, 0) LA_W4_MF16(7, 4, 1, 1, 0) LA_W4_MF16(7, 5, 1, 1, 0) LA_W4_MF16(7, 6, 1, 1, 0) LA_W4_PW(sww, 3, bofs) LA_W4_MF16(7, 7, 1, 1, 0)
+#define LA_W4_BLOCK16_6 LA_W4_MF16(4, 0, 0, 0, 1) LA_W4_RA16(1, 0, 6, 1) LA_W4_RA16(1, 1, 7, 1) LA_W4_PW(sww, 4, bofs) LA_W4_PW(sww, 5, bofs) LA_W4_MF16(4, 1, 0, 0, 1) LA_W4_MF16(4, 2, 0, 0, 1) LA_W4_MF16(4, 3, 0, 0, 1) LA_W4_MF16(4, 4, 0, 0, 1) LA_W4_MF16(4, 5, 0, 0, 1) LA_W4_MF16(4, 6, 0, 0, 1) LA_W4_MF16(4, 7, 0, 0, 1) LA_W4_MF16(5, 0, 0, 1, 1) LA_W4_MF16(5, 1, 0, 1, 1) LA_W4_MF16(5, 2, 0, 1, 1) LA_W4_MF16(5, 3, 0, 1, 1) LA_W4_MF16(5, 4, 0, 1, 1) LA_W4_MF16(5, 5, 0, 1, 1) LA_W4_MF16(5, 6, 0, 1, 1) LA_W4_PW(sww, 6, bofs) LA_W4_WAIT(15) LA_W4_SB LA_W4_MF16(5, 7, 0, 1, 1) LA_W4_BAR LA_W4_SB
+#define LA_W4_BLOCK16_7 LA_W4_MF16(6, 0, 1, 0, 1) LA_W4_RA16(0, 0, 0, 0) LA_W4_RW16(0, 0) LA_W4_RW16(0, 1) LA_W4_RW16(0, 2) LA_W4_MF16(6, 1, 1, 0, 1) LA_W4_MF16(6, 2, 1, 0, 1) LA_W4_MF16(6, 3, 1, 0, 1) LA_W4_MF16(6, 4, 1, 0, 1) LA_W4_MF16(6, 5, 1, 0, 1) LA_W4_MF16(6, 6, 1, 0, 1) LA_W4_MF16(6, 7, 1, 0, 1) LA_W4_RW16(0, 3) LA_W4_RW16(0, 4) LA_W4_RW16(0, 5) LA_W4_RW16(0, 6) LA_W4_MF16(7, 0, 1, 1, 1) LA_W4_MF16(7, 1, 1, 1, 1) LA_W4_MF16(7, 2, 1, 1, 1) LA_W4_MF16(7, 3, 1, 1, 1) LA_W4_MF16(7, 4, 1, 1, 1) LA_W4_MF16(7, 5, 1, 1, 1) LA_W4_MF16(7, 6, 1, 1, 1) LA_W4_RW16(0, 7) LA_W4_RA16(0, 1, 1, 0) LA_W4_PW(sww, 7, bofs) LA_W4_MF16(7, 7, 1, 1, 1)
+#elif LA_W4_GROUP == 8
+#define LA_W4_BLOCK16_0 LA_W4_MF16(0, 0, 0, 0, 0) LA_W4_RA16(1, 0, 2, 0) LA_W4_RA16(1, 1, 3, 0) LA_W4_RW16(1, 0) LA_W4_RW16(1, 1) LA_W4_RW16(1, 2) LA_W4_RW16(1, 3) LA_W4_PA1(sa1, 0, bo1) LA_W4_PA1(sa1, 1, bo1) LA_W4_MF16(0, 1, 0, 0, 0) LA_W4_MF16(0, 2, 0, 0, 0) LA_W4_MF16(0, 3, 0, 0, 0) LA_W4_MF16(0, 4, 0, 0, 0) LA_W4_MF16(0, 5, 0, 0, 0) LA_W4_MF16(0, 6, 0, 0, 0) LA_W4_MF16(0, 7, 0, 0, 0) LA_W4_MF16(1, 0, 0, 1, 0) LA_W4_MF16(1, 1, 0, 1, 0) LA_W4_MF16(1, 2, 0, 1, 0) LA_W4_MF16(1, 3, 0, 1, 0) LA_W4_MF16(1, 4, 0, 1, 0) LA_W4_MF16(1, 5, 0, 1, 0) LA_W4_MF16(1, 6, 0, 1, 0) LA_W4_MF16(1, 7, 0, 1, 0)
+#define LA_W4_BLOCK16_1 LA_W4_MF16(2, 0, 1, 0, 0) LA_W4_RA16(0, 0, 0, 1) LA_W4_RW16(1, 4) LA_W4_RW16(1, 5) LA_W4_RW16(1, 6) LA_W4_RW16(1, 7) LA_W4_RA16(0, 1, 1, 1) LA_W4_PA1(sa1, 2, bo1) LA_W4_MF16(2, 1, 1, 0, 0) LA_W4_MF16(2, 2, 1, 0, 0) LA_W4_MF16(2, 3, 1, 0, 0) LA_W4_MF16(2, 4, 1, 0, 0) LA_W4_MF16(2, 5, 1, 0, 0) LA_W4_MF16(2, 6, 1, 0, 0) LA_W4_MF16(2, 7, 1, 0, 0) LA_W4_MF16(3, 0, 1, 1, 0) LA_W4_MF16(3, 1, 1, 1, 0) LA_W4_MF16(3, 2, 1, 1, 0) LA_W4_MF16(3, 3, 1, 1, 0) LA_W4_MF16(3, 4, 1, 1, 0) LA_W4_MF16(3, 5, 1, 1, 0) LA_W4_MF16(3, 6, 1, 1, 0) LA_W4_MF16(3, 7, 1, 1, 0)
+#define LA_W4_BLOCK16_2 LA_W4_MF16(0, 0, 0, 0, 1) LA_W4_RA16(1, 0, 2, 1) LA_W4_RA16(1, 1, 3, 1) LA_W4_PA1(sa1, 3, bo1) LA_W4_MF16(0, 1, 0, 0, 1) LA_W4_MF16(0, 2, 0, 0, 1) LA_W4_MF16(0, 3, 0, 0, 1) LA_W4_MF16(0, 4, 0, 0, 1) LA_W4_MF16(0, 5, 0, 0, 1) LA_W4_MF16(0, 6, 0, 0, 1) LA_W4_MF16(0, 7, 0, 0, 1) LA_W4_MF16(1, 0, 0, 1, 1) LA_W4_MF16(1, 1, 0, 1, 1) LA_W4_MF16(1, 2, 0, 1, 1) LA_W4_MF16(1, 3, 0, 1, 1) LA_W4_MF16(1, 4, 0, 1, 1) LA_W4_MF16(1, 5, 0, 1, 1) LA_W4_MF16(1, 6, 0, 1, 1) LA_W4_WAIT(16) LA_W4_SB LA_W4_MF16(1, 7, 0, 1, 1) LA_W4_BAR LA_W4_SB
+#define LA_W4_BLOCK16_3 LA_W4_MF16(2, 0, 1, 0, 1) LA_W4_RA16(0, 0, 4, 0) LA_W4_RA16(0, 1, 5, 0) LA_W4_PA0(saw, 0, bofs) LA_W4_PA0(saw, 1, bofs) LA_W4_MF16(2, 1, 1, 0, 1) LA_W4_MF16(2, 2, 1, 0, 1) LA_W4_MF16(2, 3, 1, 0, 1) LA_W4_MF16(2, 4, 1, 0, 1) LA_W4_MF16(2, 5, 1, 0, 1) LA_W4_MF16(2, 6, 1, 0, 1) LA_W4_MF16(2, 7, 1, 0, 1) LA_W4_MF16(3, 0, 1, 1, 1) LA_W4_MF16(3, 1, 1, 1, 1) LA_W4_MF16(3, 2, 1, 1, 1) LA_W4_MF16(3, 3, 1, 1, 1) LA_W4_MF16(3, 4, 1, 1, 1) LA_W4_MF16(3, 5, 1, 1, 1) LA_W4_MF16(3, 6, 1, 1, 1) LA_W4_MF16(3, 7, 1, 1, 1)
+#define LA_W4_BLOCK16_4 LA_W4_MF16(4, 0, 0, 0, 0) LA_W4_RA16(1, 0, 6, 0) LA_W4_RA16(1, 1, 7, 0) LA_W4_PA0(saw, 2, bofs) LA_W4_PA0(saw, 3, bofs) LA_W4_PW(sww, 0, bofs) LA_W4_MF16(4, 1, 0, 0, 0) LA_W4_MF16(4, 2, 0, 0, 0) LA_W4_MF16(4, 3, 0, 0, 0) LA_W4_MF16(4, 4, 0, 0, 0) LA_W4_MF16(4, 5, 0, 0, 0) LA_W4_MF16(4, 6, 0, 0, 0) LA_W4_MF16(4, 7, 0, 0, 0) LA_W4_MF16(5, 0, 0, 1, 0) LA_W4_MF16(5, 1, 0, 1, 0) LA_W4_MF16(5, 2, 0, 1, 0) LA_W4_MF16(5, 3, 0, 1, 0) LA_W4_MF16(5, 4, 0, 1, 0) LA_W4_MF16(5, 5, 0, 1, 0) LA_W4_MF16(5, 6, 0, 1, 0) LA_W4_MF16(5, 7, 0, 1, 0)
+#define LA_W4_BLOCK16_5 LA_W4_MF16(6, 0, 1, 0, 0) LA_W4_RA16(0, 0, 4, 1) LA_W4_RA16(0, 1, 5, 1) LA_W4_PW(sww, 1, bofs) LA_W4_PW(sww, 2, bofs) LA_W4_PW(sww, 3, bofs) LA_W4_MF16(6, 1, 1, 0, 0) LA_W4_MF16(6, 2, 1, 0, 0) LA_W4_MF16(6, 3, 1, 0, 0) LA_W4_MF16(6, 4, 1, 0, 0) LA_W4_MF16(6, 5, 1, 0, 0) LA_W4_MF16(6, 6, 1, 0, 0) LA_W4_MF16(6, 7, 1, 0, 0) LA_W4_MF16(7, 0, 1, 1, 0) LA_W4_MF16(7, 1, 1, 1, 0) LA_W4_MF16(7, 2, 1, 1, 0) LA_W4_MF16(7, 3, 1, 1, 0) LA_W4_MF16(7, 4, 1, 1, 0) LA_W4_MF16(7, 5, 1, 1, 0) LA_W4_MF16(7, 6, 1, 1, 0) LA_W4_MF16(7, 7, 1, 1, 0)
+#define LA_W4_BLOCK16_6 LA_W4_MF16(4, 0, 0, 0, 1) LA_W4_RA16(1, 0, 6, 1) LA_W4_RA16(1, 1, 7, 1) LA_W4_PW(sww, 4, bofs) LA_W4_PW(sww, 5, bofs) LA_W4_PW(sww, 6, bofs) LA_W4_MF16(4, 1, 0, 0, 1) LA_W4_MF16(4, 2, 0, 0, 1) LA_W4_MF16(4, 3, 0, 0, 1) LA_W4_MF16(4, 4, 0, 0, 1) LA_W4_MF16(4, 5, 0, 0, 1) LA_W4_MF16(4, 6, 0, 0, 1) LA_W4_MF16(4, 7, 0, 0, 1) LA_W4_MF16(5, 0, 0, 1, 1) LA_W4_MF16(5, 1, 0, 1, 1) LA_W4_MF16(5, 2, 0, 1, 1) LA_W4_MF16(5, 3, 0, 1, 1) LA_W4_MF16(5, 4, 0, 1, 1) LA_W4_MF16(5, 5, 0, 1, 1) LA_W4_MF16(5, 6, 0, 1, 1) LA_W4_WAIT(15) LA_W4_SB LA_W4_MF16(5, 7, 0, 1, 1) LA_W4_BAR LA_W4_SB
+#define LA_W4_BLOCK16_7 LA_W4_MF16(6, 0, 1, 0, 1) LA_W4_RA16(0, 0, 0, 0) LA_W4_RW16(0, 0) LA_W4_RW16(0, 1) LA_W4_RW16(0, 2) LA_W4_RW16(0, 3) LA_W4_RW16(0, 4) LA_W4_RW16(0, 5) LA_W4_RW16(0, 6) LA_W4_MF16(6, 1, 1, 0, 1) LA_W4_MF16(6, 2, 1, 0, 1) LA_W4_MF16(6, 3, 1, 0, 1) LA_W4_MF16(6, 4, 1, 0, 1) LA_W4_MF16(6, 5, 1, 0, 1) LA_W4_MF16(6, 6, 1, 0, 1) LA_W4_MF16(6, 7, 1, 0, 1) LA_W4_MF16(7, 0, 1, 1, 1) LA_W4_MF16(7, 1, 1, 1, 1) LA_W4_MF16(7, 2, 1, 1, 1) LA_W4_MF16(7, 3, 1, 1, 1) LA_W4_MF16(7, 4, 1, 1, 1) LA_W4_MF16(7, 5, 1, 1, 1) LA_W4_MF16(7, 6, 1, 1, 1) LA_W4_RW16(0, 7) LA_W4_RA16(0, 1, 1, 0) LA_W4_PW(sww, 7, bofs) LA_W4_MF16(7, 7, 1, 1, 1)
+#endif
diff --git a/labelanything_amd/csrc/mfma_shape.hip b/labelanything_amd/csrc/mfma_shape.hip
--- /dev/null
+++ b/labelanything_amd/csrc/mfma_shape.hip
@@ -0,0 +1,83 @@
+#include "la_common.h"
+#include "../../include/la_hip.h"
+
+namespace la {
+
+template <typename T> struct Mfma16;
+template <> struct Mfma16<f16_t> {
+  static __device__ __forceinline__ f32x4 go(uint4 a, uint4 b, f32x4 c) {
+    return __builtin_amdgcn_mfma_f32_16x16x32_f16(__builtin_bit_cast(h8_t, a), __builtin_bit_cast(h8_t, b), c, 0, 0, 0);
+  }
+};
+template <> struct Mfma16<bf16_t> {
+  static __device__ __forceinline__ f32x4 go(uint4 a, uint4 b, f32x4 c) {
+    return __builtin_amdgcn_mfma_f32_16x16x32_bf16(__builtin_bit_cast(b8_t, a), __builtin_bit_cast(b8_t, b), c, 0, 0, 0);
+  }
+};
+
+template <typename T, int SHAPE>
+__global__ __launch_bounds__(64) void mfma_shape_kernel(const T* __restrict__ A, const T* __restrict__ W, float* __restrict__ out, int K) {
+  const int lane = threadIdx.x;
+  if constexpr (SHAPE == 0) {
+    const int fr = lane & 31, fh = lane >> 5;
+    f32x16 acc;
+#pragma unroll
+    for (int r = 0; r < 16; ++r) acc[r] = 0.f;
+    for (int k0 = 0; k0 < K; k0 += 64)
+#pragma unroll
+      for (int ks = 0; ks < 4; ++ks) {
+        const size_t o = (size_t)fr * K + k0 + ks * 16 + fh * 8;
+        acc = Half16<T>::mfma32(*reinterpret_cast<const uint4*>(A + o), *reinterpret_cast<const uint4*>(W + o), acc);
+      }
+#pragma unroll
+    for (int r = 0; r < 16; ++r) out[((r & 3) + 8 * (r >> 2) + 4 * fh) * 32 + fr] = acc[r];
+  } else {
+    const int r16 = lane & 15, q = lane >> 4;
+    f32x4 acc[2][2];
+#pragma unroll
+    for (int i = 0; i < 2; ++i)
+#pragma unroll
+      for (int j = 0; j < 2; ++j) acc[i][j] = f32x4{0.f, 0.f, 0.f, 0.f};
+    for (int k0 = 0; k0 < K; k0 += 64)
+#pragma unroll
+      for (int ks = 0; ks < 2; ++ks) {
+        uint4 a[2], b[2];
+#pragma unroll
+        for (int i = 0; i < 2; ++i) {
+          const size_t o = (size_t)(16 * i + r16) * K + k0 + ks * 32 + q * 8;
+          a[i] = *reinterpret_cast<const uint4*>(A + o);
+          b[i] = *reinterpret_cast<const uint4*>(W + o);
+        }
+#pragma unroll
+        for (int i = 0; i < 2; ++i)
+#pragma unroll
+          for (int j = 0; j < 2; ++j) acc[i][j] = Mfma16<T>::go(a[i], b[j], acc[i][j]);
+      }
+#pragma unroll
+    for (int i = 0; i < 2; ++i)
+#pragma unroll
+      for (int j = 0; j < 2; ++j)
+#pragma unroll
+        for (int r = 0; r < 4; ++r) out[(16 * i + 4 * q + r) * 32 + 16 * j + r16] = acc[i][j][r];
+  }
+}
+
+}
+
+extern "C" int la_mfma_shape_probe(const void* A, const void* W, float* out, int K, int dt, int shape, void* stream) {
+  LA_CHECK_ARG(A && W && out, "la_mfma_shape_probe: null pointer");
+  LA_CHECK_ARG(K > 0 && (K % 64) == 0, "la_mfma_shape_probe: K=%d must be a positive multiple of 64", K);
+  LA_CHECK_ARG((dt == LA_F16 || dt == LA_BF16) && (shape == 0 || shape == 1), "la_mfma_shape_probe: dt=%d must be 16-bit, shape=%d 0 or 1", dt, shape);
+  LA_CHECK_ARG((((uintptr_t)A | (uintptr_t)W) & 15) == 0, "la_mfma_shape_probe: operands must be 16-byte aligned");
+  hipStream_t s = reinterpret_cast<hipStream_t>(stream);
+  using namespace la;
+  if (dt == LA_F16) {
+    if (shape == 0) mfma_shape_kernel<f16_t, 0><<<1, 64, 0, s>>>((const f16_t*)A, (const f16_t*)W, out, K);
+    else mfma_shape_kernel<f16_t, 1><<<1, 64, 0, s>>>((const f16_t*)A, (const f16_t*)W, out, K);
+  } else {
+    if (shape == 0) mfma_shape_kernel<bf16_t, 0><<<1, 64, 0, s>>>((const bf16_t*)A, (const bf16_t*)W, out, K);
+    else mfma_shape_kernel<bf16_t, 1><<<1, 64, 0, s>>>((const bf16_t*)A, (const bf16_t*)W, out, K);
+  }
+  LA_CHECK_LAUNCH("la_mfma_shape_probe");
+  return 0;
+}
```

Result: faster. 402.6 episodes/s (median of 6 runs) (+2.9%).
